# laprade117/interactive-unet

Hardware: AMD Instinct MI355X
Metric: voxels/sec (train step + full-volume predict) on 128^3 chunks (higher is better)
Workload: dtype bf16

## Files before the change

### include/iunet.h

```cpp
#ifndef IUNET_H
#define IUNET_H
#ifdef __cplusplus
extern "C" {
#endif

const char* iunet_last_error(void);
int iunet_abi_version(void);

long long iunet_pack_conv3_elems(int Cout, int Cin, int taps, int mode);
int iunet_pack_conv3(int dtype, const void* w, const void* scale, void* dst, int Cout, int Cin, int taps, int mode,
                     void* stream);
long long iunet_pack_first_conv_elems(int Cout, int Cin, int taps);
int iunet_pack_first_conv(int dtype, const void* w, const void* scale, void* dst, int Cout, int Cin, int taps,
                          void* stream);
int iunet_pack_convT(int dtype, const void* w, void* dst, int Cin, int Cout, int npos, void* stream);

int iunet_pack_desc_bytes(void);
int iunet_pack_batch(const void* descs, int n, int quant_max_cout, void* stream);

int iunet_conv3_fwd(int dtype, int nd, const void* x, long long x_sstride, void* y, long long y_sstride,
                    const void* wpk, const void* bias, void* stats, int N, int D, int H, int W, int Cin, int Cout,
                    int epi, int layout, void* stream);
int iunet_conv3_pick_layout(int nd, int N, int D, int H, int W, int Cin, int Cout);
int iunet_conv3_tile_pairs(int nd, int N, int D, int H, int W, int Cin, int Cout);
// ... 190 lines not shown
int iunet_bn_relu_bwd(int dtype, const void* dz, long long dz_ss, const void* z, long long z_ss, const void* y,
                      long long y_ss, void* dy, long long dy_ss, const void* mean, const void* invstd, const void* gamma,
                      const void* scale, const void* shift, void* dgamma, void* dbeta, void* slab, void* coef, int C, int N,
                      long long vox, void* stream);
int iunet_bn_relu_sum_bwd(int dtype, int nd, int K, const void* const* srcs, const long long* src_ss, const void* dpool,
                          long long dp_ss, const void* y, long long y_ss, void* dy, long long dy_ss, const void* mean,
                          const void* invstd, const void* gamma, const void* scale, const void* shift, void* dgamma, void* dbeta,
                          void* slab, void* coef, int C, int N, int D, int H, int W, void* stream);
int iunet_conv3_dgrad_bnstats(int dtype, int nd, const void* dy, long long dy_sstride, void* dz, long long dz_sstride,
                              const void* wpk, void* stats, const void* yp, long long yp_sstride, const void* mean,
                              const void* invstd, const void* scale, const void* shift, int N, int D, int H, int W, int Cin,
                              int Cout, void* stream);
int iunet_conv3_dgrad_bnstats_lay(int dtype, int nd, const void* dy, long long dy_sstride, void* dz, long long dz_sstride,
                                  const void* wpk, void* stats, const void* yp, long long yp_sstride, const void* mean,
                                  const void* invstd, const void* scale, const void* shift, int N, int D, int H, int W, int Cin,
                                  int Cout, int layout, void* stream);
int iunet_bn_relu_bwd_apply(int dtype, const void* dz, long long dz_ss, const void* y, long long y_ss, void* dy, long long dy_ss,
                            const void* mean, const void* invstd, const void* gamma, const void* scale, const void* shift,
                            void* dgamma, void* dbeta, const void* slab, int nparts, void* coef, int C, int N, long long vox,
                            void* stream);
int iunet_gn_num_parts(int N, long long vox);
int iunet_gn_relu_fwd(int dtype, const void* y, long long y_ss, void* z, long long z_ss, const void* gamma, const void* beta,
                      int groups, float eps, void* slab, void* scale, void* shift, void* mean, void* invstd, int C, int N,
                      long long vox, void* stream);
int iunet_gn_finalize(const void* stats, int nparts, int C, int groups, long long vox, const void* gamma, const void* beta, float eps,
                      void* scale, void* shift, void* mean, void* invstd, void* stream);
int iunet_gn_relu_bwd(int dtype, const void* dz, long long dz_ss, const void* y, long long y_ss, void* dy, long long dy_ss,
                      const void* gamma, int groups, const void* scale, const void* shift, const void* mean, const void* invstd,
                      void* dgamma, void* dbeta, void* slab, void* coef, int C, int N, long long vox, void* stream);
int iunet_gn_relu_pool_fwd(int dtype, int nd, const void* y, long long y_ss, void* z, long long z_ss, void* pooled, long long p_ss,
                           const void* gamma, const void* beta, int groups, float eps, void* slab, void* scale, void* shift, void* mean,
                           void* invstd, int C, int N, int Do, int Ho, int Wo, void* stream);
int iunet_conv3_sample_stats_rows(int dtype, int nd, int N, int D, int H, int W, int Cin, int Cout, int layout);
int iunet_conv3_fwd_sample_stats(int dtype, int nd, const void* x, long long x_sstride, void* y, long long y_sstride, const void* wpk,
                                 void* stats, int N, int D, int H, int W, int Cin, int Cout, int layout, void* stream);
int iunet_gn_relu_fwd_rows(int dtype, const void* y, long long y_ss, void* z, long long z_ss, const void* gamma, const void* beta,
                           int groups, float eps, void* slab, int rows, void* scale, void* shift, void* mean, void* invstd, int C, int N,
                           long long vox, void* stream);
int iunet_gn_relu_pool_fwd_rows(int dtype, int nd, const void* y, long long y_ss, void* z, long long z_ss, void* pooled, long long p_ss,
                                const void* gamma, const void* beta, int groups, float eps, void* slab, int rows, void* scale, void* shift,
                                void* mean, void* invstd, int C, int N, int Do, int Ho, int Wo, void* stream);
int iunet_conv3_dgrad_sample_bnstats(int dtype, int nd, const void* dy, long long dy_sstride, void* dz, long long dz_sstride, const void* wpk,
                                     void* stats, const void* yp, long long yp_sstride, const void* mean, const void* invstd, const void* scale,
                                     const void* shift, int N, int D, int H, int W, int Cin, int Cout, int layout, void* stream);
int iunet_gn_relu_bwd_rows(int dtype, const void* dz, long long dz_ss, const void* y, long long y_ss, void* dy, long long dy_ss,
                           const void* gamma, int groups, const void* scale, const void* shift, const void* mean, const void* invstd,
                           void* dgamma, void* dbeta, void* slab, int rows, void* coef, int C, int N, long long vox, void* stream);
int iunet_gn_relu_pool_bwd(int dtype, int nd, const void* dskip, long long ds_ss, const void* dpool, long long dp_ss, const void* y,
                           long long y_ss, void* dy, long long dy_ss, const void* gamma, int groups, const void* scale, const void* shift,
                           const void* mean, const void* invstd, void* dgamma, void* dbeta, void* slab, void* coef, int C, int N, int Do,
                           int Ho, int Wo, void* stream);
int iunet_bn_relu_pool_bwd(int dtype, int nd, const void* dskip, long long ds_ss, const void* dpool, long long dp_ss,
                           const void* y, long long y_ss, void* dy, long long dy_ss, const void* mean, const void* invstd,
                           const void* gamma, const void* scale, const void* shift, void* dgamma, void* dbeta, void* slab,
                           void* coef, int C, int N, int Do, int Ho, int Wo, void* stream);
int iunet_maxpool_bwd(int dtype, int nd, const void* z, long long z_ss, const void* dpool, long long dp_ss, void* dz,
                      long long dz_ss, int add_skip, int C, int N, int Do, int Ho, int Wo, void* stream);
int iunet_head_loss_num_parts(int N, long long vox);
int iunet_head_loss_fwd(int dtype, const void* x, long long x_ss, int C0, const void* w, const void* bias, int ncls,
                        const void* target, const void* weight, int tdtype, int kind, void* slab, void* out4, void* coef,
                        int N, long long vox, void* stream);
int iunet_head_loss_bwd_num_parts(int N, long long vox, int ncls, int C0);
int iunet_head_loss_bwd(int dtype, const void* x, long long x_ss, int C0, const void* w, const void* bias, int ncls,
                        const void* target, const void* weight, int tdtype, const void* coef, float loss_scale, void* dx,
                        long long dx_ss, void* dwslab, int N, long long vox, void* stream);
int iunet_head_loss_fwd_act(int dtype, const void* x, long long x_ss, int C0, const void* w, const void* bias, int ncls,
                            const void* target, const void* weight, int tdtype, int kind, void* slab, void* out4, void* coef,
                            const void* in_scale, const void* in_shift, int N, long long vox, void* stream);
int iunet_head_loss_bwd_act(int dtype, const void* x, long long x_ss, int C0, const void* w, const void* bias, int ncls,
                            const void* target, const void* weight, int tdtype, const void* coef, float loss_scale, void* dx,
                            long long dx_ss, void* dwslab, const void* in_scale, const void* in_shift, int N, long long vox,
                            void* stream);
int iunet_reduce_slab(void* slab, int nparts, long long n, void* out, float alpha, int accumulate, void* stream);
int iunet_conv3_wgrad_blocks(int nd, int N, int D, int H, int W, int Cin, int Cout);
long long iunet_conv3_wgrad_slab_floats(int nd, int N, int D, int H, int W, int Cin, int Cout);
int iunet_conv3_wgrad(int dtype, int nd, const void* x, long long x_ss, const void* dy, long long dy_ss, void* slab,
                      void* dW, float alpha, int N, int D, int H, int W, int Cin, int Cout, void* stream);
int iunet_conv3_wgrad_act(int dtype, int nd, const void* x, long long x_ss, const void* dy, long long dy_ss, void* slab,
                          void* dW, float alpha, const void* x_scale, const void* x_shift, int N, int D, int H, int W,
                          int Cin, int Cout, void* stream);
int iunet_pack_convT_dgrad(int dtype, const void* w, void* dst, int Cin, int Cout, int npos, void* stream);
int iunet_convT_dgrad(int dtype, int nd, const void* dy, long long dy_ss, void* dx, long long dx_ss, const void* wpk,
                      int N, int D, int H, int W, int Cin, int Cout, void* stream);
int iunet_convT_wgrad_blocks(int nd, int N, int D, int H, int W, int Cin, int Cout);
int iunet_convT_wgrad(int dtype, int nd, const void* x, long long x_ss, const void* dy, long long dy_ss, void* wslab,
                      void* bslab, void* dW, void* db, int N, int D, int H, int W, int Cin, int Cout, void* stream);
int iunet_first_conv_wgrad_blocks(int nd, int N, int D, int H, int W);
int iunet_first_conv_wgrad(int dtype, int nd, const void* x, int in_dtype, const long long* in_strides, const void* dy,
                           long long dy_ss, void* slab, void* dW, int N, int D, int H, int W, int Cin, int Cout,
                           void* stream);
int iunet_first_conv_wgrad_bn(int dtype, int nd, const void* x, int in_dtype, const long long* in_strides, const void* dz,
                              long long dz_ss, const void* y, long long y_ss, const void* mean, const void* invstd,
                              const void* coef, const void* scale, const void* shift, void* slab, void* dW, int N, int D, int H,
                              int W, int Cin, int Cout, void* stream);
int iunet_check_finite(const void* g, long long n, void* flag, void* stream);
int iunet_adamw_step(void* p, const void* g, void* m, void* v, long long n, float lr, float b1, float b2, float eps,
                     float wd, int step, float grad_scale_inv, const void* skip_flag, void* stream);

int iunet_train_state_init(void* state, float loss_scale, int dynamic, void* stream);
int iunet_head_loss_bwd_dev(int dtype, const void* x, long long x_ss, int C0, const void* w, const void* bias, int ncls,
                            const void* target, const void* weight, int tdtype, const void* coef, const void* state, void* dx,
                            long long dx_ss, void* dwslab, const void* in_scale, const void* in_shift, int N, long long vox,
                            void* stream);
int iunet_head_bn_bwd_ok(int C0, int ncls);
int iunet_head_bn_bwd(int dtype, const void* y, long long y_ss, int C0, const void* w, const void* bias, int ncls, const void* target,
                      const void* weight, int tdtype, const void* coef, float loss_scale, const void* state, const void* scale,
                      const void* shift, const void* mean, const void* invstd, const void* gamma, void* dgamma, void* dbeta, void* dy,
                      long long dy_ss, void* dwslab, void* bnslab, void* bncoef, void* dl_scratch, int N, long long vox, void* stream);
int iunet_head_gn_bwd(int dtype, const void* y, long long y_ss, int C0, const void* w, const void* bias, int ncls, const void* target,
                      const void* weight, int tdtype, const void* coef, float loss_scale, const void* state, const void* scale,
                      const void* shift, const void* mean, const void* invstd, const void* gamma, int groups, void* dgamma, void* dbeta, void* dy,
                      long long dy_ss, void* dwslab, void* bnslab, void* bncoef, void* dl_scratch, int N, long long vox, void* stream);
int iunet_head_loss_fwd_act_ps(int dtype, const void* x, long long x_ss, int C0, const void* w, const void* bias, int ncls,
                               const void* target, const void* weight, int tdtype, int kind, void* slab, void* out4, void* coef,
                               const void* in_scale, const void* in_shift, int per_sample, int N, long long vox, void* stream);
int iunet_head_grad_scatter(const void* row, void* dw, void* db, int ncls, int C0, void* stream);
int iunet_adamw_step_dev(void* p, const void* g, void* m, void* v, long long n, float lr, float b1, float b2, float eps, float wd,
                         void* state, int check, float world, void* stream);

typedef struct iunet_train iunet_train;
int iunet_train_create(int dim, int levels, int base, int cin, int ncls, int dtype, int loss_kind, iunet_train** out);
int iunet_train_create_ex(int dim, int levels, int base, int cin, int ncls, int dtype, int loss_kind, int norm, int groups, iunet_train** out);
int iunet_train_create_nested(int dim, int levels, int base, int cin, int ncls, int dtype, int loss_kind, iunet_train** out);
void iunet_train_destroy(iunet_train* t);
long long iunet_train_num_params(const iunet_train* t);
int iunet_train_num_tensors(const iunet_train* t);
int iunet_train_param(const iunet_train* t, int index, char* name, int name_cap, long long* offset, long long* numel);
int iunet_train_num_bn(const iunet_train* t);
long long iunet_train_packed_bytes(const iunet_train* t);
long long iunet_train_workspace_bytes(const iunet_train* t, int N, int D, int H, int W);
int iunet_train_bind(iunet_train* t, void* flat, void* grad, void* m, void* v, void* const* running, void* packed, void* state, void* stream);
int iunet_train_repack(iunet_train* t, void* stream);
int iunet_train_forward_backward(iunet_train* t, const void* x, int in_dtype, const long long* in_strides, const void* target,
                                 const void* weight, int tdtype, int N, int D, int H, int W, void* workspace, void* out4, void* stream);
typedef void (*iunet_train_hook)(void* ctx, int stage);
int iunet_train_forward_backward_hooks(iunet_train* t, const void* x, int in_dtype, const long long* in_strides, const void* target,
                                       const void* weight, int tdtype, int N, int D, int H, int W, void* workspace, void* out4,
                                       iunet_train_hook hook, void* hook_ctx, void* stream);
int iunet_train_update(iunet_train* t, float lr, float b1, float b2, float eps, float wd, float world, void* stream);
int iunet_train_step(iunet_train* t, const void* x, int in_dtype, const long long* in_strides, const void* target, const void* weight,
                     int tdtype, int N, int D, int H, int W, void* workspace, float lr, float b1, float b2, float eps, float wd, void* out4,
                     void* stream);

long long iunet_lk_pack_elems(int nd, int kind, int Cout, int Cin);
int iunet_lk_pack(int dtype, int nd, int kind, const void* w, const void* gamma, const void* beta, const void* mean, const void* var,
                  float eps, void* dst, void* bias_out, int Cout, int Cin, void* stream);
int iunet_lk_stats_parts(int nd, int kind, int N, int D, int H, int W, int Cout);
int iunet_lk_conv_fwd(int dtype, int nd, int kind, const void* x, long long x_ss, void* y, long long y_ss, const void* wpk,
                      const void* in_scale, const void* in_shift, const void* bias, const void* skip, long long skip_ss, void* stats, int epi,
                      int N, int D, int H, int W, int Cin, int Cout, void* stream);
long long iunet_lk_wgrad_slab_floats(int nd, int kind, int N, int D, int H, int W, int Cin, int Cout);
int iunet_lk_wgrad(int dtype, int nd, int kind, const void* x, long long x_ss, const void* dy, long long dy_ss, const void* x_scale,
                   const void* x_shift, void* slab, void* dW, float alpha, int N, int D, int H, int W, int Cin, int Cout, void* stream);
int iunet_lk_bn_relu_add(int dtype, const void* y, long long y_ss, const void* skip, long long skip_ss, void* out, long long out_ss,
                         const void* scale, const void* shift, int C, int N, long long vox, void* stream);
int iunet_lk_f32_conv_fwd(int nd, int kind, const void* x, long long x_ss, void* y, long long y_ss, const void* wpk, const void* bias,
                          const void* skip, long long skip_ss, int N, int D, int H, int W, int Cin, int Cout, void* stream);

int iunet_dl_num_taps(int nd, int rate, int D, int H, int W);
int iunet_dl_pack(int dtype, int nd, int mode, int ksz, const void* w, const void* gamma, const void* beta, const void* mean, const void* var,
                  float eps, void* dst, void* bias_out, int Cout, int Cin, int Cin_tot, int ci_off, int k_off, int ld, void* stream);
int iunet_dl_stats_parts(int N, int D, int H, int W, int Cout);
int iunet_dl_conv_fwd(int dtype, int nd, const void* x, long long x_ss, void* y, long long y_ss, const void* wpk, int Kw, int nbr,
                      const int* rates, const int* cbase, const int* colbase, const void* in_scale, const void* in_shift, const void* bias,
                      const void* psb, float psb_scale, void* stats, int epi, int N, int D, int H, int W, int Cin, int Cout, void* stream);
long long iunet_dl_wgrad_slab_floats(int nd, int rate, int N, int D, int H, int W, int Cin, int Cout);
// ... 45 lines not shown
```

### interactive-unet_amd/csrc/train_misc.hip

```cpp
#include "common.h"

namespace {


struct ConvTDgradParams {
  const void* dy; long long dy_ss;
  void* dx; long long dx_ss;
  const void* wpk;
  int N, D, H, W, Cin, Cout;
};

template <typename T, int ND>
__global__ __launch_bounds__(256) void convT_dgrad_kernel(ConvTDgradParams p) {
  using V8 = V8T<T>;
  constexpr int NPOS = ND == 3 ? 8 : 4;
  const int lane = threadIdx.x & 63, wave = threadIdx.x >> 6;
  const int l15 = lane & 15, q = lane >> 4;
  const int xg = (p.W + 15) / 16;
  const long long rows = (long long)p.D * p.H * xg;
  const long long wid = (long long)blockIdx.x * 4 + wave;
  if (wid >= rows * p.N) return;
  const int n = (int)(wid / rows);
  const long long r = wid - n * rows;
  const int xb = (int)(r % xg), y = (int)((r / xg) % p.H), z = (int)(r / ((long long)xg * p.H));
  const int cib = blockIdx.y;
  const int x = xb * 16 + l15;
  const bool ok = x < p.W;
  const int xc = ok ? x : p.W - 1;
  const int Do = ND == 3 ? p.D * 2 : 1, Ho = p.H * 2, Wo = p.W * 2;
  const long long out_plane = (long long)Do * Ho * Wo * 8;
  const T* dyin = (const T*)p.dy + n * p.dy_ss;
  const int nk = p.Cout >> 5;
  const V8* wp = (const V8*)p.wpk + (long long)cib * NPOS * nk * 2 * 64 + lane;
  f32x4 acc0 = f32x4{0, 0, 0, 0}, acc1 = f32x4{0, 0, 0, 0};
#pragma unroll
  for (int s = 0; s < NPOS; ++s) {
    const int a = ND == 3 ? (s >> 2) : 0, b = (s >> 1) & 1, c = s & 1;
    const int oz = ND == 3 ? z * 2 + a : 0;
    const long long voff = (((long long)oz * Ho + y * 2 + b) * Wo + xc * 2 + c) * 8;
    for (int kc = 0; kc < nk; ++kc) {
      const V8 bf = *(const V8*)(dyin + (long long)(kc * 4 + q) * out_plane + voff);
      const V8 a0 = wp[((s * nk + kc) * 2 + 0) * 64];
      const V8 a1 = wp[((s * nk + kc) * 2 + 1) * 64];
      acc0 = mfma16<T>(a0, bf, acc0);
      acc1 = mfma16<T>(a1, bf, acc1);
    }
  }
  const long long in_plane = (long long)p.D * p.H * p.W * 8;
  V8 o;
#pragma unroll
  for (int j = 0; j < 4; ++j) { o[j] = from_f32<T>(acc0[j]); o[4 + j] = from_f32<T>(acc1[j]); }
  if (ok)
    *(V8*)((T*)p.dx + n * p.dx_ss + (long long)(cib * 4 + q) * in_plane + (((long long)z * p.H + y) * p.W + x) * 8) = o;
}

template <typename T, int ND, int NK, int NCI>
__global__ __launch_bounds__(256, (NCI * NK * (ND == 3 ? 16 : 8) <= 64) ? 2 : 1) void convT_dgrad_lds_kernel(ConvTDgradParams p) {
  using V8 = V8T<T>;
  constexpr int NPOS = ND == 3 ? 8 : 4, G = 2;
  constexpr int WCI = NPOS * NK * 2 * 64;
  extern __shared__ __attribute__((aligned(256))) unsigned char smem[];
  const int lane = threadIdx.x & 63, wave = threadIdx.x >> 6;
  const int l15 = lane & 15, q = lane >> 4;
  const int cib0 = blockIdx.y * NCI;
  {
    const u32x4* wsrc = (const u32x4*)p.wpk + (long long)cib0 * WCI;
    stage_to_lds(smem, wsrc, NCI * WCI, threadIdx.x, 256);
  }
  __syncthreads();
  const int xg = (p.W + 15) / 16;
  const long long rows = (long long)p.D * p.H * xg, ngroups = rows * p.N;
  const int Do = ND == 3 ? p.D * 2 : 1, Ho = p.H * 2, Wo = p.W * 2;
  const long long out_plane = (long long)Do * Ho * Wo * 8, in_plane = (long long)p.D * p.H * p.W * 8;
  for (long long g0 = ((long long)blockIdx.x * 4 + wave) * G; g0 < ngroups; g0 += (long long)gridDim.x * 4 * G) {
    unsigned woff = lane * 16;
    asm volatile("" : "+v"(woff));
    const V8* wl = (const V8*)(smem + woff);
    f32x4 acc[NCI][G][2];
    const T* dyb[G];
    long long xoff[G];
    bool okg[G];
#pragma unroll
    for (int g = 0; g < G; ++g) {
      const long long wid = g0 + g < ngroups ? g0 + g : ngroups - 1;
      const int n = (int)(wid / rows);
      const long long r = wid - n * rows;
      const int xb = (int)(r % xg), y = (int)((r / xg) % p.H), z = (int)(r / ((long long)xg * p.H));
      const int x = xb * 16 + l15, xc = min(x, p.W - 1);
      okg[g] = x < p.W && g0 + g < ngroups;
      const int oz = ND == 3 ? z * 2 : 0;
      dyb[g] = (const T*)p.dy + n * p.dy_ss + (((long long)oz * Ho + y * 2) * Wo + xc * 2) * 8;
      xoff[g] = n * p.dx_ss + (long long)(cib0 * 4 + q) * in_plane + (((long long)z * p.H + y) * p.W + x) * 8;
#pragma unroll
      for (int c = 0; c < NCI; ++c) { acc[c][g][0] = f32x4{0, 0, 0, 0}; acc[c][g][1] = f32x4{0, 0, 0, 0}; }
    }
#pragma unroll
    for (int s = 0; s < NPOS; ++s) {
      const int a = ND == 3 ? (s >> 2) : 0, b = (s >> 1) & 1, c = s & 1;
      const long long voff = (((long long)a * Ho + b) * Wo + c) * 8;
#pragma unroll
      for (int kc = 0; kc < NK; ++kc) {
        V8 bf[G];
#pragma unroll
        for (int g = 0; g < G; ++g) bf[g] = *(const V8*)(dyb[g] + (long long)(kc * 4 + q) * out_plane + voff);
#pragma unroll
        for (int c = 0; c < NCI; ++c) {
          const V8 a0 = wl[c * WCI + ((s * NK + kc) * 2 + 0) * 64];
          const V8 a1 = wl[c * WCI + ((s * NK + kc) * 2 + 1) * 64];
#pragma unroll
          for (int g = 0; g < G; ++g) {
            acc[c][g][0] = mfma16<T>(a0, bf[g], acc[c][g][0]);
            acc[c][g][1] = mfma16<T>(a1, bf[g], acc[c][g][1]);
          }
        }
      }
    }
#pragma unroll
    for (int c = 0; c < NCI; ++c)
#pragma unroll
      for (int g = 0; g < G; ++g) {
        V8 o;
#pragma unroll
        for (int j = 0; j < 4; ++j) { o[j] = from_f32<T>(acc[c][g][0][j]); o[4 + j] = from_f32<T>(acc[c][g][1][j]); }
        if (okg[g]) *(V8*)((T*)p.dx + xoff[g] + (long long)c * 4 * in_plane) = o;
      }
  }
}

template <typename T>
__global__ void pack_convT_dgrad_kernel(const float* __restrict__ w, T* __restrict__ dst, int Cin, int Cout, int npos) {
  const long long total = (long long)Cin * Cout * npos;
  const int nk = Cout >> 5;
  for (long long i = blockIdx.x * (long long)blockDim.x + threadIdx.x; i < total; i += (long long)gridDim.x * blockDim.x) {
    long long r = i;
    const int j = r & 7; r >>= 3;
    const int lane = r & 63; r >>= 6;
    const int t = r & 1; r >>= 1;
    const int kc = r % nk; r /= nk;
    const int s = r % npos;
    const int cib = r / npos;
    const int row = lane & 15, qq = lane >> 4;
    const int ci = cib * 32 + 8 * (row >> 2) + 4 * t + (row & 3);
    const int co = kc * 32 + 8 * qq + j;
    dst[i] = from_f32<T>(w[((long long)ci * Cout + co) * npos + s]);
  }
}

typedef short s16x4w __attribute__((ext_vector_type(4)));
typedef short s16x8w __attribute__((ext_vector_type(8)));
typedef __attribute__((address_space(3))) s16x4w* lds_s4w_ptr;

template <typename T>
__device__ __forceinline__ typename Vec8<T>::type tr_frag2(unsigned addr, unsigned hi_off) {
  const s16x4w lo = __builtin_amdgcn_ds_read_tr16_b64_v4i16((lds_s4w_ptr)addr);
  const s16x4w hi = __builtin_amdgcn_ds_read_tr16_b64_v4i16((lds_s4w_ptr)(addr + hi_off));
  const s16x8w v = __builtin_shufflevector(lo, hi, 0, 1, 2, 3, 4, 5, 6, 7);
  return __builtin_bit_cast(typename Vec8<T>::type, v);
}

struct ConvTWgradParams {
  const void* x; long long x_ss;
  const void* dy; long long dy_ss;
  float* wslab;
  float* bslab;
  int N, D, H, W, Cin, Cout;
  int tilesZ, tilesY, tilesX;
};

template <typename T, int ND, int NCI>
__global__ __launch_bounds__(256, 2) void convT_wgrad_kernel(ConvTWgradParams p) {
  using V8 = V8T<T>;
  constexpr int NPOS = ND == 3 ? 8 : 4;
  constexpr int TZ = ND == 3 ? 2 : 1, TY = ND == 3 ? 4 : 8, TX = 16;
  constexpr int NVI = TZ * TY * TX;
  constexpr int OZ = ND == 3 ? 2 * TZ : 1, OY = 2 * TY, OX = 2 * TX;
  constexpr int NVO = OZ * OY * OX;
  constexpr int PLANE_X = NVI * 16 + 64, PLANE_Y = NVO * 16 + 64;
  constexpr int OFF_Y = 4 * PLANE_X;
  constexpr int NKS = NVI / 32;
  constexpr int PL = NPOS / 4;
  extern __shared__ __attribute__((aligned(256))) unsigned char smem[];
  const unsigned lds0 = (unsigned)(size_t)(__attribute__((address_space(3))) unsigned char*)smem;
  const int tid = threadIdx.x, lane = tid & 63;
  const int wave = __builtin_amdgcn_readfirstlane(tid >> 6);
  const int g = lane >> 4, i16 = lane & 15, q = i16 >> 2, pp = i16 & 3, gh = g >> 1, gl = g & 1;
  const int cib0 = blockIdx.y * NCI, cob = blockIdx.z;
  const unsigned laneX = lds0 + (pp >> 1) * PLANE_X + (pp & 1) * 8 + (gh * 16 + gl * 8 + q) * 16;
  const unsigned laneY = lds0 + OFF_Y + (pp >> 1) * PLANE_Y + (pp & 1) * 8 + (gh * 2 * OX + 2 * (gl * 8 + q)) * 16;
  unsigned pos_off[PL];
#pragma unroll
  for (int i = 0; i < PL; ++i) {
    const int s = wave * PL + i;
    const int a = ND == 3 ? (s >> 2) : 0, b = (s >> 1) & 1, c = s & 1;
    pos_off[i] = (unsigned)(((a * OY + b) * OX + c) * 16);
  }
  f32x4 acc[NCI][PL][2][2];
#pragma unroll
  for (int c = 0; c < NCI; ++c)
#pragma unroll
    for (int i = 0; i < PL; ++i)
#pragma unroll
      for (int t = 0; t < 2; ++t) { acc[c][i][t][0] = f32x4{0, 0, 0, 0}; acc[c][i][t][1] = f32x4{0, 0, 0, 0}; }
  float bacc[8] = {0.f, 0.f, 0.f, 0.f, 0.f, 0.f, 0.f, 0.f};

  const int tps = p.tilesZ * p.tilesY * p.tilesX, ntiles = tps * p.N;
  const int Do = ND == 3 ? p.D * 2 : 1, Ho = p.H * 2, Wo = p.W * 2;
  const long long in_plane = (long long)p.D * p.H * p.W * 8, out_plane = (long long)Do * Ho * Wo * 8;
  constexpr int XIT = NVI * 4 / 256, YIT = NVO * 4 / 256;
  u32x4 xr[NCI * XIT], xkeep[NCI > 1 ? XIT : 1];
  V8 yr[YIT];
  auto load_tile = [&](int tile) {
    const int n = tile / tps;
    int trem = tile - n * tps;
    const int tz_i = trem / (p.tilesY * p.tilesX);
    trem -= tz_i * p.tilesY * p.tilesX;
    const int ty_i = trem / p.tilesX, tx_i = trem - ty_i * p.tilesX;
    const int z0 = tz_i * TZ, y0 = ty_i * TY, x0 = tx_i * TX;
    const T* xin = (const T*)p.x + (long long)n * p.x_ss + (long long)cib0 * 4 * in_plane;
    const T* dyin = (const T*)p.dy + (long long)n * p.dy_ss + (long long)cob * 4 * out_plane;
#pragma unroll
    for (int k = 0; k < NCI * XIT; ++k) {
      const int it = tid + k * 256;
      const int pl = it / NVI, pix = it - pl * NVI;
      const int px = pix % TX, t2 = pix / TX, py = t2 % TY, pz = t2 / TY;
      const int gz = z0 + pz, gy = y0 + py, gx = x0 + px;
      u32x4 v = u32x4{0u, 0u, 0u, 0u};
      if (gz < p.D && gy < p.H && gx < p.W) v = *(const u32x4*)(xin + pl * in_plane + (((long long)gz * p.H + gy) * p.W + gx) * 8);
      xr[k] = v;
    }
#pragma unroll
    for (int k = 0; k < YIT; ++k) {
      const int it = tid + k * 256;
      const int pl = it & 3, pix = it >> 2;
      const int px = pix % OX, t2 = pix / OX, py = t2 % OY, pz = t2 / OY;
      const int gz = 2 * z0 + pz, gy = 2 * y0 + py, gx = 2 * x0 + px;
      V8 v;
#pragma unroll
      for (int j = 0; j < 8; ++j) v[j] = from_f32<T>(0.f);
      if (gz < Do && gy < Ho && gx < Wo) v = *(const V8*)(dyin + pl * out_plane + (((long long)gz * Ho + gy) * Wo + gx) * 8);
      yr[k] = v;
    }
  };
  auto commit_x = [&](const u32x4* src) {
#pragma unroll
    for (int k = 0; k < XIT; ++k) {
      const int it = tid + k * 256;
      const int pl = it / NVI, pix = it - pl * NVI;
      *(u32x4*)(smem + pl * PLANE_X + pix * 16) = src[k];
    }
  };
  auto commit_tile = [&]() {
    commit_x(xr);
    if (NCI > 1) {
#pragma unroll
      for (int k = 0; k < XIT; ++k) xkeep[k] = xr[XIT + k];
    }
#pragma unroll
    for (int k = 0; k < YIT; ++k) {
      const int it = tid + k * 256;
      const int pl = it & 3, pix = it >> 2;
      *(V8*)(smem + OFF_Y + pl * PLANE_Y + pix * 16) = yr[k];
#pragma unroll
      for (int j = 0; j < 8; ++j) bacc[j] += to_f32<T>(yr[k][j]);
    }
  };
  if ((int)blockIdx.x < ntiles) load_tile(blockIdx.x);
  for (int tile = blockIdx.x; tile < ntiles; tile += gridDim.x) {
    __syncthreads();
    commit_tile();
    __syncthreads();
    if (tile + (int)gridDim.x < ntiles) load_tile(tile + gridDim.x);
#pragma unroll
    for (int c = 0; c < NCI; ++c) {
      if (c > 0) {
        __syncthreads();
        commit_x(xkeep);
        __syncthreads();
      }
#pragma unroll
      for (int ks = 0; ks < NKS; ++ks) {
        const int r = 2 * ks, rz = r / TY, ry = r % TY;
        const unsigned offX = (unsigned)(r * TX * 16);
        const unsigned offY = (unsigned)(((2 * rz * OY + 2 * ry) * OX) * 16);
        const V8 a0 = tr_frag2<T>(laneX + offX, 64);
        const V8 a1 = tr_frag2<T>(laneX + offX + 2 * PLANE_X, 64);
#pragma unroll
        for (int i = 0; i < PL; ++i) {
          const V8 b0 = tr_frag2<T>(laneY + offY + pos_off[i], 128);
          const V8 b1 = tr_frag2<T>(laneY + offY + pos_off[i] + 2 * PLANE_Y, 128);
          acc[c][i][0][0] = mfma16<T>(a0, b0, acc[c][i][0][0]);
          acc[c][i][0][1] = mfma16<T>(a0, b1, acc[c][i][0][1]);
          acc[c][i][1][0] = mfma16<T>(a1, b0, acc[c][i][1][0]);
          acc[c][i][1][1] = mfma16<T>(a1, b1, acc[c][i][1][1]);
        }
      }
    }
  }
#pragma unroll
  for (int c = 0; c < NCI; ++c) {
    float* ws = p.wslab + ((((long long)blockIdx.x * (gridDim.y * NCI) + cib0 + c) * gridDim.z + cob) * NPOS) * 1024;
#pragma unroll
    for (int i = 0; i < PL; ++i) {
      const int s = wave * PL + i;
#pragma unroll
      for (int t = 0; t < 2; ++t)
#pragma unroll
        for (int u = 0; u < 2; ++u)
#pragma unroll
          for (int j = 0; j < 4; ++j) ws[s * 1024 + (t * 16 + 4 * g + j) * 32 + u * 16 + i16] = acc[c][i][t][u][j];
    }
  }
  if (blockIdx.y == 0) {
    __syncthreads();
    float* red = (float*)smem;
#pragma unroll
    for (int j = 0; j < 8; ++j) red[tid * 8 + j] = bacc[j];
    __syncthreads();
    if (tid < 32) {
      const int pl = tid >> 3, j = tid & 7;
      float sum = 0.f;
      for (int k = pl; k < 256; k += 4) sum += red[k * 8 + j];
      p.bslab[(long long)blockIdx.x * p.Cout + cob * 32 + pl * 8 + j] = sum;
    }
  }
}

__global__ __launch_bounds__(256) void convT_wgrad_reduce_kernel(const float* __restrict__ slab, int nb, int Cin, int Cout, int npos,
                                                                 float* __restrict__ dW) {
  __shared__ f32x4 red[16][16];
  const long long per_b4 = (long long)Cin * Cout * npos / 4;
  const int col4 = threadIdx.x & 15, grp = threadIdx.x >> 4;
  const long long j4 = (long long)blockIdx.x * 16 + col4;
  const f32x4* slab4 = (const f32x4*)slab;
  f32x4 s = f32x4{0.f, 0.f, 0.f, 0.f};
  for (int b = grp; b < nb; b += 16) s += slab4[b * per_b4 + j4];
  red[grp][col4] = s;
  __syncthreads();
  if (grp != 0) return;
#pragma unroll
  for (int g = 1; g < 16; ++g) s += red[g][col4];
  const int ncob = Cout / 32;
#pragma unroll
  for (int k = 0; k < 4; ++k) {
    const long long j = j4 * 4 + k;
    const int c = (int)(j & 31), r = (int)((j >> 5) & 31);
    long long t = j >> 10;
    const int pos = (int)(t % npos); t /= npos;
    const int cob = (int)(t % ncob), cib = (int)(t / ncob);
    dW[((long long)(cib * 32 + r) * Cout + cob * 32 + c) * npos + pos] = s[k];
  }
}

struct FirstWgradParams {
  const void* x; long long sN, sC, sD, sH, sW; int in_dtype;
  const void* dy; long long dy_ss;
  const void* yraw; long long y_ss;
  const float* mean; const float* invstd; const float* coef; const float* scale; const float* shift;
  float* slab;
  int N, D, H, W, Cin, Cout;
  int tilesZ, tilesY, tilesX;
};

__device__ __forceinline__ float load_in2(const void* p, long long off, int dt) {
  switch (dt) {
    case 0: return ((const float*)p)[off];
    case 1: return (float)((const f16*)p)[off];
    case 2: return (float)((const unsigned char*)p)[off] / 255.0f;
    default: return (float)((const bf16*)p)[off];
  }
}

template <typename T, int ND, int CIN>
__global__ __launch_bounds__(256, 2) void first_wgrad_kernel(FirstWgradParams p) {
  using V8 = V8T<T>;
  constexpr int TZ = ND == 3 ? 4 : 1, TY = ND == 3 ? 8 : 16, TX = ND == 3 ? 16 : 32, PADZ = ND == 3 ? 1 : 0;
  constexpr int PZ = TZ + 2 * PADZ, PY = TY + 2, PX = TX + 2, NPIX = PZ * PY * PX, NVOX = TZ * TY * TX;
  constexpr int TAPS = ND == 3 ? 27 : 9, KK = TAPS * CIN, NT = (KK + 15) / 16, KKP = NT * 16;
  constexpr int FX = TX / 16, NKS = NVOX / 32;
  constexpr int PLANE_Y = NVOX * 16 + 64;
  constexpr int XS_BYTES = ((CIN * NPIX * 2 + 255) / 256) * 256;
  extern __shared__ __attribute__((aligned(256))) unsigned char smem[];
  T* xs = (T*)smem;
  unsigned char* dys = smem + XS_BYTES;
  __shared__ __attribute__((aligned(16))) float par[7 * 32];
  if (p.yraw != nullptr && threadIdx.x < 7 * 32) {
    const int k = threadIdx.x >> 5, c = blockIdx.y * 32 + (threadIdx.x & 31);
    par[threadIdx.x] = k == 0 ? p.scale[c] : k == 1 ? p.shift[c] : k == 2 ? p.mean[c] : k == 3 ? p.invstd[c] : p.coef[c * 3 + (k - 4)];
  }
  const unsigned lds_y = (unsigned)(size_t)(__attribute__((address_space(3))) unsigned char*)dys;
  const int tid = threadIdx.x, lane = tid & 63;
  const int wave = __builtin_amdgcn_readfirstlane(tid >> 6);
  const int g = lane >> 4, i16 = lane & 15, q = i16 >> 2, pp = i16 & 3, gh = g >> 1, gl = g & 1;
  const int cob = blockIdx.y;
  const unsigned laneY = lds_y + (pp >> 1) * PLANE_Y + (pp & 1) * 8 + (gh * 16 + gl * 8 + q) * 16;
  int col_off[NT];
#pragma unroll
  for (int ct = 0; ct < NT; ++ct) {
    const int kk = ct * 16 + i16, kc = kk < KK ? kk : 0;
    const int tap = kc / CIN, c = kc % CIN;
    const int dz = ND == 3 ? tap / 9 : 0, dy_ = (tap / 3) % 3, dx = tap % 3;
    col_off[ct] = c * NPIX + (dz * PY + dy_) * PX + dx;
  }
  f32x4 acc[2][NT];
#pragma unroll
  for (int t = 0; t < 2; ++t)
#pragma unroll
// ... 82 lines not shown
    __syncthreads();
    if (tile + (int)gridDim.x < ntiles) load_tile(tile + gridDim.x);
    for (int ks = wave; ks < NKS; ks += 4) {
      const int f = 2 * ks + gh;
      const int xh = f % FX, row = f / FX, fy = row % TY, fz = row / TY;
      const int vbase = (fz * PY + fy) * PX + xh * 16 + gl * 8;
      const V8 a0 = tr_frag2<T>(laneY + (unsigned)(2 * ks * 256), 64);
      const V8 a1 = tr_frag2<T>(laneY + (unsigned)(2 * ks * 256) + 2 * PLANE_Y, 64);
#pragma unroll
      for (int ct = 0; ct < NT; ++ct) {
        V8 b;
#pragma unroll
        for (int j = 0; j < 8; ++j) b[j] = xs[vbase + j + col_off[ct]];
        acc[0][ct] = mfma16<T>(a0, b, acc[0][ct]);
        acc[1][ct] = mfma16<T>(a1, b, acc[1][ct]);
      }
    }
  }
  __syncthreads();
  float* red = (float*)smem;
#pragma unroll
  for (int t = 0; t < 2; ++t)
#pragma unroll
    for (int ct = 0; ct < NT; ++ct)
#pragma unroll
      for (int j = 0; j < 4; ++j) red[(wave * 32 + t * 16 + 4 * g + j) * KKP + ct * 16 + i16] = acc[t][ct][j];
  __syncthreads();
  float* slab = p.slab + ((long long)blockIdx.x * p.Cout + cob * 32) * KKP;
  for (int i = tid; i < 32 * KKP; i += 256)
    slab[i] = red[i] + red[32 * KKP + i] + red[2 * 32 * KKP + i] + red[3 * 32 * KKP + i];
}

__global__ __launch_bounds__(256) void first_wgrad_reduce_kernel(const float* __restrict__ slab, int nb, int Cout, int Cin, int taps,
                                                                 int KKP, float* __restrict__ dW) {
  __shared__ float red[8][32];
  const int total = Cout * Cin * taps;
  const int o = threadIdx.x & 31, grp = threadIdx.x >> 5;
  const int i = blockIdx.x * 32 + o;
  float s = 0.f;
  if (i < total) {
    const int tap = i % taps, c = (i / taps) % Cin, co = i / (taps * Cin);
    const float* src = slab + (long long)co * KKP + tap * Cin + c;
    const long long st = (long long)Cout * KKP;
    int b = grp;
    float s1 = 0.f, s2 = 0.f, s3 = 0.f;
    for (; b + 24 < nb; b += 32) {
      const float a0 = src[b * st], a1 = src[(b + 8) * st], a2 = src[(b + 16) * st], a3 = src[(b + 24) * st];
      s += a0; s1 += a1; s2 += a2; s3 += a3;
    }
    for (; b < nb; b += 8) s += src[b * st];
    s = (s + s1) + (s2 + s3);
  }
  red[grp][o] = s;
  __syncthreads();
  if (grp == 0 && i < total) {
    float a = red[0][o];
#pragma unroll
    for (int g = 1; g < 8; ++g) a += red[g][o];
    dW[i] = a;
  }
}

}

#define DT_OK(dt) IUNET_REQUIRE((dt) == 0 || (dt) == 1, "dtype must be 0 (f16) or 1 (bf16), got %d", (dt))

extern "C" int iunet_reduce_slab(void* slab, int nparts, long long n, void* out, float alpha, int accumulate, void* stream);

extern "C" {

int iunet_pack_convT_dgrad(int dtype, const void* w, void* dst, int Cin, int Cout, int npos, void* stream) {
  DT_OK(dtype);
  IUNET_REQUIRE(w && dst, "pack_convT_dgrad: null pointer");
  IUNET_REQUIRE(Cin >= 32 && Cout >= 32 && Cin % 32 == 0 && Cout % 32 == 0, "pack_convT_dgrad: channels must be positive multiples of 32");
  IUNET_REQUIRE(npos == 4 || npos == 8, "pack_convT_dgrad: npos must be 4 or 8");
  const long long total = (long long)Cin * Cout * npos;
  const int blocks = (int)((total + 255) / 256 < 4096 ? (total + 255) / 256 : 4096);
  if (dtype == 0) hipLaunchKernelGGL(pack_convT_dgrad_kernel<f16>, dim3(blocks), dim3(256), 0, (hipStream_t)stream, (const float*)w, (f16*)dst, Cin, Cout, npos);
  else hipLaunchKernelGGL(pack_convT_dgrad_kernel<bf16>, dim3(blocks), dim3(256), 0, (hipStream_t)stream, (const float*)w, (bf16*)dst, Cin, Cout, npos);
  IUNET_CHECK_HIP(hipGetLastError());
  return IUNET_OK;
}

int iunet_convT_dgrad(int dtype, int nd, const void* dy, long long dy_ss, void* dx, long long dx_ss, const void* wpk,
                      int N, int D, int H, int W, int Cin, int Cout, void* stream) {
  DT_OK(dtype);
  IUNET_REQUIRE(dy && dx && wpk, "convT_dgrad: null pointer");
  IUNET_REQUIRE(nd == 2 || nd == 3, "convT_dgrad: nd must be 2 or 3");
  IUNET_REQUIRE_GRID("convT_dgrad", N, D, H, W);
  IUNET_REQUIRE(Cin >= 32 && Cout >= 32 && Cin % 32 == 0 && Cout % 32 == 0, "convT_dgrad: channels must be positive multiples of 32 (%d, %d)", Cin, Cout);
  ConvTDgradParams p;
  p.dy = dy; p.dy_ss = dy_ss; p.dx = dx; p.dx_ss = dx_ss; p.wpk = wpk; p.N = N; p.D = D; p.H = H; p.W = W; p.Cin = Cin; p.Cout = Cout;
  const long long waves = (long long)N * D * H * ((W + 15) / 16);
  const int nk = Cout / 32;
  if (nk <= 4 && waves >= 256) {
    const int nci = (nk <= 2 && (Cin / 32) % 2 == 0 && (nd == 3 ? 8 : 4) * nk * 2 * 1024 * 2 <= 32768) ? 2 : 1;
    const int lds = (nd == 3 ? 8 : 4) * nk * 2 * 1024 * nci;
    int gx = (int)((waves + 7) / 8);
    const int cap = 1024 / (Cin / 32 / nci);
    if (gx > cap) gx = cap;
    dim3 g2(gx, Cin / 32 / nci);
#define CDL(TT, NDV, NKV) do { if (nci == 2) { IUNET_SET_MAX_LDS((convT_dgrad_lds_kernel<TT, NDV, NKV, 2>), lds); \
      hipLaunchKernelGGL((convT_dgrad_lds_kernel<TT, NDV, NKV, 2>), g2, dim3(256), lds, (hipStream_t)stream, p); } \
    else { IUNET_SET_MAX_LDS((convT_dgrad_lds_kernel<TT, NDV, NKV, 1>), lds); \
      hipLaunchKernelGGL((convT_dgrad_lds_kernel<TT, NDV, NKV, 1>), g2, dim3(256), lds, (hipStream_t)stream, p); } } while (0)
#define CDL_NK(TT, NDV) switch (nk) { case 1: CDL(TT, NDV, 1); break; case 2: CDL(TT, NDV, 2); break; case 3: CDL(TT, NDV, 3); break; default: CDL(TT, NDV, 4); break; }
    if (dtype == 0) { if (nd == 3) { CDL_NK(f16, 3) } else { CDL_NK(f16, 2) } }
    else            { if (nd == 3) { CDL_NK(bf16, 3) } else { CDL_NK(bf16, 2) } }
#undef CDL_NK
#undef CDL
    IUNET_CHECK_HIP(hipGetLastError());
    return IUNET_OK;
  }
  dim3 grid((unsigned)((waves + 3) / 4), Cin / 32);
  if (dtype == 0) { if (nd == 3) hipLaunchKernelGGL((convT_dgrad_kernel<f16, 3>), grid, dim3(256), 0, (hipStream_t)stream, p);
                    else hipLaunchKernelGGL((convT_dgrad_kernel<f16, 2>), grid, dim3(256), 0, (hipStream_t)stream, p); }
  else { if (nd == 3) hipLaunchKernelGGL((convT_dgrad_kernel<bf16, 3>), grid, dim3(256), 0, (hipStream_t)stream, p);
         else hipLaunchKernelGGL((convT_dgrad_kernel<bf16, 2>), grid, dim3(256), 0, (hipStream_t)stream, p); }
  IUNET_CHECK_HIP(hipGetLastError());
  return IUNET_OK;
}

int iunet_convT_wgrad_blocks(int nd, int N, int D, int H, int W, int Cin, int Cout) {
  if (N < 1 || D < 1 || H < 1 || W < 1 || Cin < 32 || Cout < 32) return 0;
  const int TZ = nd == 3 ? 2 : 1, TY = nd == 3 ? 4 : 8, TX = 16;
  const long long ntiles = (long long)N * ((D + TZ - 1) / TZ) * ((H + TY - 1) / TY) * ((W + TX - 1) / TX);
  const int nci = (Cin / 32) % 2 == 0 ? 2 : 1;
  const int pairs = (Cin / 32 / nci) * (Cout / 32);
  long long nb = (512 + pairs - 1) / pairs;
  if (nb > ntiles) nb = ntiles;
  return (int)(nb < 1 ? 1 : nb);
}

int iunet_convT_wgrad(int dtype, int nd, const void* x, long long x_ss, const void* dy, long long dy_ss, void* wslab,
                      void* bslab, void* dW, void* db, int N, int D, int H, int W, int Cin, int Cout, void* stream) {
  DT_OK(dtype);
  IUNET_REQUIRE(x && dy && wslab && bslab && dW && db, "convT_wgrad: null pointer");
  IUNET_REQUIRE(Cin >= 32 && Cout >= 32 && Cin % 32 == 0 && Cout % 32 == 0, "convT_wgrad: channels must be positive multiples of 32");
  IUNET_REQUIRE(nd == 2 || nd == 3, "convT_wgrad: nd must be 2 or 3");
  IUNET_REQUIRE_GRID("convT_wgrad", N, D, H, W);
  ConvTWgradParams p;
  p.x = x; p.x_ss = x_ss; p.dy = dy; p.dy_ss = dy_ss; p.wslab = (float*)wslab; p.bslab = (float*)bslab;
  p.N = N; p.D = D; p.H = H; p.W = W; p.Cin = Cin; p.Cout = Cout;
  const int TZ = nd == 3 ? 2 : 1, TY = nd == 3 ? 4 : 8, TX = 16;
  p.tilesZ = (D + TZ - 1) / TZ; p.tilesY = (H + TY - 1) / TY; p.tilesX = (W + TX - 1) / TX;
  const int nb = iunet_convT_wgrad_blocks(nd, N, D, H, W, Cin, Cout);
  const int npos = nd == 3 ? 8 : 4;
  const int nvi = 128, nvo = nd == 3 ? 1024 : 512;
  const int lds = 4 * (nvi * 16 + 64) + 4 * (nvo * 16 + 64);
  const int nci = (Cin / 32) % 2 == 0 ? 2 : 1;
  dim3 grid(nb, Cin / 32 / nci, Cout / 32);
#define CTW(TT, NDV) do { if (nci == 2) { IUNET_SET_MAX_LDS((convT_wgrad_kernel<TT, NDV, 2>), lds); \
      hipLaunchKernelGGL((convT_wgrad_kernel<TT, NDV, 2>), grid, dim3(256), lds, (hipStream_t)stream, p); } \
    else { IUNET_SET_MAX_LDS((convT_wgrad_kernel<TT, NDV, 1>), lds); \
      hipLaunchKernelGGL((convT_wgrad_kernel<TT, NDV, 1>), grid, dim3(256), lds, (hipStream_t)stream, p); } } while (0)
  if (dtype == 0) { if (nd == 3) CTW(f16, 3); else CTW(f16, 2); } else { if (nd == 3) CTW(bf16, 3); else CTW(bf16, 2); }
#undef CTW
  const long long total = (long long)Cin * Cout * npos;
  hipLaunchKernelGGL(convT_wgrad_reduce_kernel, dim3((unsigned)(total / 64)), dim3(256), 0, (hipStream_t)stream,
                     (const float*)wslab, nb, Cin, Cout, npos, (float*)dW);
  IUNET_CHECK_HIP(hipGetLastError());
  return iunet_reduce_slab(bslab, nb, Cout, db, 1.0f, 0, stream);
}

int iunet_first_conv_wgrad_blocks(int nd, int N, int D, int H, int W) {
  if (N < 1 || D < 1 || H < 1 || W < 1) return 0;
  const int TZ = nd == 3 ? 4 : 1, TY = nd == 3 ? 8 : 16, TX = nd == 3 ? 16 : 32;
  const long long ntiles = (long long)N * ((D + TZ - 1) / TZ) * ((H + TY - 1) / TY) * ((W + TX - 1) / TX);
  return (int)(ntiles < 512 ? ntiles : 512);
}

static int first_wgrad_impl(int dtype, int nd, const void* x, int in_dtype, const long long* in_strides, const void* dy,
                            long long dy_ss, void* slab, void* dW, int N, int D, int H, int W, int Cin, int Cout,
                            const void* yraw, long long y_ss, const float* mean, const float* invstd, const float* coef,
                            const float* scale, const float* shift, void* stream) {
  DT_OK(dtype);
  IUNET_REQUIRE(x && dy && slab && dW && in_strides, "first_conv_wgrad: null pointer");
  IUNET_REQUIRE(Cin >= 1 && Cin <= 4 && Cout >= 32 && Cout % 32 == 0, "first_conv_wgrad: Cin 1..4, Cout a positive multiple of 32");
  IUNET_REQUIRE(nd == 2 || nd == 3, "first_conv_wgrad: nd must be 2 or 3");
  IUNET_REQUIRE(in_dtype >= 0 && in_dtype <= 3, "first_conv_wgrad: bad input dtype %d", in_dtype);
  IUNET_REQUIRE_GRID("first_conv_wgrad", N, D, H, W);
  FirstWgradParams p;
  p.x = x; p.sN = in_strides[0]; p.sC = in_strides[1]; p.sD = in_strides[2]; p.sH = in_strides[3]; p.sW = in_strides[4];
  p.in_dtype = in_dtype; p.dy = dy; p.dy_ss = dy_ss; p.slab = (float*)slab;
  p.yraw = yraw; p.y_ss = y_ss; p.mean = mean; p.invstd = invstd; p.coef = coef; p.scale = scale; p.shift = shift;
  p.N = N; p.D = D; p.H = H; p.W = W; p.Cin = Cin; p.Cout = Cout;
  const int TZ = nd == 3 ? 4 : 1, TY = nd == 3 ? 8 : 16, TX = nd == 3 ? 16 : 32;
  p.tilesZ = (D + TZ - 1) / TZ; p.tilesY = (H + TY - 1) / TY; p.tilesX = (W + TX - 1) / TX;
  const int nb = iunet_first_conv_wgrad_blocks(nd, N, D, H, W);
  const int taps = nd == 3 ? 27 : 9, KKP = ((taps * Cin + 15) / 16) * 16;
  const int npix = (nd == 3 ? 6 : 1) * (TY + 2) * (TX + 2);
  const int xs_bytes = ((Cin * npix * 2 + 255) / 256) * 256;
  int lds = xs_bytes + 4 * (512 * 16 + 64);
  if (lds < 4 * 32 * KKP * 4) lds = 4 * 32 * KKP * 4;
  dim3 grid(nb, Cout / 32);
#define FW(TT, NDV, CI) do { IUNET_SET_MAX_LDS((first_wgrad_kernel<TT, NDV, CI>), lds); \
    hipLaunchKernelGGL((first_wgrad_kernel<TT, NDV, CI>), grid, dim3(256), lds, (hipStream_t)stream, p); } while (0)
#define FW_CIN(TT, NDV) switch (Cin) { case 1: FW(TT, NDV, 1); break; case 2: FW(TT, NDV, 2); break; case 3: FW(TT, NDV, 3); break; default: FW(TT, NDV, 4); break; }
  if (dtype == 0) { if (nd == 3) { FW_CIN(f16, 3) } else { FW_CIN(f16, 2) } }
  else            { if (nd == 3) { FW_CIN(bf16, 3) } else { FW_CIN(bf16, 2) } }
#undef FW_CIN
#undef FW
  const int total = Cout * Cin * taps;
  hipLaunchKernelGGL(first_wgrad_reduce_kernel, dim3((total + 31) / 32), dim3(256), 0, (hipStream_t)stream,
                     (const float*)slab, nb, Cout, Cin, taps, KKP, (float*)dW);
  IUNET_CHECK_HIP(hipGetLastError());
  return IUNET_OK;
}

int iunet_first_conv_wgrad(int dtype, int nd, const void* x, int in_dtype, const long long* in_strides, const void* dy,
                           long long dy_ss, void* slab, void* dW, int N, int D, int H, int W, int Cin, int Cout,
                           void* stream) {
  return first_wgrad_impl(dtype, nd, x, in_dtype, in_strides, dy, dy_ss, slab, dW, N, D, H, W, Cin, Cout, nullptr, 0, nullptr,
                          nullptr, nullptr, nullptr, nullptr, stream);
}

int iunet_first_conv_wgrad_bn(int dtype, int nd, const void* x, int in_dtype, const long long* in_strides, const void* dz,
                              long long dz_ss, const void* y, long long y_ss, const void* mean, const void* invstd,
                              const void* coef, const void* scale, const void* shift, void* slab, void* dW, int N, int D, int H,
                              int W, int Cin, int Cout, void* stream) {
  IUNET_REQUIRE(y && mean && invstd && coef && scale && shift, "first_conv_wgrad_bn: null pointer");
  return first_wgrad_impl(dtype, nd, x, in_dtype, in_strides, dz, dz_ss, slab, dW, N, D, H, W, Cin, Cout, y, y_ss,
                          (const float*)mean, (const float*)invstd, (const float*)coef, (const float*)scale,
                          (const float*)shift, stream);
}

}
```

### interactive-unet_amd/csrc/train_net.hip

```cpp
#include "common.h"
#include "pack_desc.h"
#include <algorithm>
#include <cstdio>
#include <cstdlib>
#include <string>
#include <vector>

extern "C" {
int iunet_pack_batch(const void*, int, int, void*);
int iunet_pack_desc_bytes(void);
long long iunet_pack_conv3_elems(int, int, int, int);
long long iunet_pack_first_conv_elems(int, int, int);
int iunet_conv3_packs_compact(int, int);
int iunet_conv3_plan(int, int, int, int, int, int, int, int, int, int, int*);
int iunet_conv3_num_tiles(int, int, int, int, int);
int iunet_conv3_stats_parts(int, int, int, int, int, int, int);
int iunet_first_conv_fwd(int, int, const void*, int, const long long*, void*, long long, const void*, const void*, void*, int, int, int,
                         int, int, int, int, void*);
int iunet_conv3_fwd(int, int, const void*, long long, void*, long long, const void*, const void*, void*, int, int, int, int, int, int,
                    int, int, void*);
int iunet_conv3_fwd_act(int, int, const void*, long long, void*, long long, const void*, const void*, void*, const void*, const void*,
                        int, int, int, int, int, int, int, int, void*);
int iunet_convT_fwd(int, int, const void*, long long, void*, long long, const void*, const void*, int, int, int, int, int, int, void*);
int iunet_bn_finalize(const void*, int, int, double, const void*, const void*, void*, void*, float, float, void*, void*, void*, void*, void*);
int iunet_bn_relu_fwd(int, const void*, long long, void*, long long, const void*, const void*, int, int, long long, void*);
int iunet_bn_relu_pool_fwd(int, int, const void*, long long, void*, long long, void*, long long, const void*, const void*, int, int, int,
                           int, int, void*);
int iunet_bn_bwd_num_parts(int, long long);
int iunet_bn_relu_bwd(int, const void*, long long, const void*, long long, const void*, long long, void*, long long, const void*,
                      const void*, const void*, const void*, const void*, void*, void*, void*, void*, int, int, long long, void*);
int iunet_conv3_dgrad_bnstats_lay(int, int, const void*, long long, void*, long long, const void*, void*, const void*, long long, const void*,
                                  const void*, const void*, const void*, int, int, int, int, int, int, int, void*);
int iunet_bn_relu_bwd_apply(int, const void*, long long, const void*, long long, void*, long long, const void*, const void*, const void*,
                            const void*, const void*, void*, void*, const void*, int, void*, int, int, long long, void*);
int iunet_bn_relu_pool_bwd(int, int, const void*, long long, const void*, long long, const void*, long long, void*, long long, const void*,
                           const void*, const void*, const void*, const void*, void*, void*, void*, void*, int, int, int, int, int, void*);
int iunet_head_loss_num_parts(int, long long);
int iunet_head_loss_fwd(int, const void*, long long, int, const void*, const void*, int, const void*, const void*, int, int, void*, void*,
                        void*, int, long long, void*);
int iunet_head_loss_fwd_act(int, const void*, long long, int, const void*, const void*, int, const void*, const void*, int, int, void*,
                            void*, void*, const void*, const void*, int, long long, void*);
int iunet_head_loss_bwd_num_parts(int, long long, int, int);
int iunet_head_loss_bwd_dev(int, const void*, long long, int, const void*, const void*, int, const void*, const void*, int, const void*,
                            const void*, void*, long long, void*, const void*, const void*, int, long long, void*);
int iunet_head_grad_scatter(const void*, void*, void*, int, int, void*);
int iunet_head_bn_bwd_ok(int, int);
int iunet_head_gn_bwd(int, const void*, long long, int, const void*, const void*, int, const void*, const void*, int, const void*, float, const void*, const void*,
                      const void*, const void*, const void*, const void*, int, void*, void*, void*, long long, void*, void*, void*, void*, int, long long, void*);
int iunet_head_loss_fwd_act_ps(int, const void*, long long, int, const void*, const void*, int, const void*, const void*, int, int, void*, void*, void*,
                               const void*, const void*, int, int, long long, void*);
int iunet_head_bn_bwd(int, const void*, long long, int, const void*, const void*, int, const void*, const void*, int, const void*, float, const void*, const void*,
                      const void*, const void*, const void*, const void*, void*, void*, void*, long long, void*, void*, void*, void*, int, long long, void*);
int iunet_reduce_slab(void*, int, long long, void*, float, int, void*);
long long iunet_conv3_wgrad_slab_floats(int, int, int, int, int, int, int);
int iunet_conv3_wgrad(int, int, const void*, long long, const void*, long long, void*, void*, float, int, int, int, int, int, int, void*);
int iunet_conv3_wgrad_act(int, int, const void*, long long, const void*, long long, void*, void*, float, const void*, const void*, int,
                          int, int, int, int, int, void*);
int iunet_convT_dgrad(int, int, const void*, long long, void*, long long, const void*, int, int, int, int, int, int, void*);
int iunet_convT_wgrad_blocks(int, int, int, int, int, int, int);
int iunet_convT_wgrad(int, int, const void*, long long, const void*, long long, void*, void*, void*, void*, int, int, int, int, int, int,
                      void*);
int iunet_first_conv_wgrad_blocks(int, int, int, int, int);
int iunet_first_conv_wgrad_bn(int, int, const void*, int, const long long*, const void*, long long, const void*, long long, const void*,
                              const void*, const void*, const void*, const void*, void*, void*, int, int, int, int, int, int, void*);
int iunet_adamw_step_dev(void*, const void*, void*, void*, long long, float, float, float, float, float, void*, int, float, void*);
int iunet_conv3_sample_stats_rows(int, int, int, int, int, int, int, int, int);
int iunet_conv3_fwd_sample_stats(int, int, const void*, long long, void*, long long, const void*, void*, int, int, int, int, int, int, int, void*);
int iunet_conv3_dgrad_sample_bnstats(int, int, const void*, long long, void*, long long, const void*, void*, const void*, long long, const void*, const void*,
                                     const void*, const void*, int, int, int, int, int, int, int, void*);
int iunet_gn_relu_bwd_rows(int, const void*, long long, const void*, long long, void*, long long, const void*, int, const void*, const void*, const void*,
                           const void*, void*, void*, void*, int, void*, int, int, long long, void*);
int iunet_gn_relu_fwd_rows(int, const void*, long long, void*, long long, const void*, const void*, int, float, void*, int, void*, void*, void*, void*, int, int,
                           long long, void*);
int iunet_gn_relu_pool_fwd_rows(int, int, const void*, long long, void*, long long, void*, long long, const void*, const void*, int, float, void*, int, void*,
                                void*, void*, void*, int, int, int, int, int, void*);
int iunet_gn_relu_fwd(int, const void*, long long, void*, long long, const void*, const void*, int, float, void*, void*, void*, void*, void*, int, int,
                      long long, void*);
int iunet_gn_relu_pool_fwd(int, int, const void*, long long, void*, long long, void*, long long, const void*, const void*, int, float, void*, void*,
                           void*, void*, void*, int, int, int, int, int, void*);
int iunet_gn_relu_bwd(int, const void*, long long, const void*, long long, void*, long long, const void*, int, const void*, const void*, const void*,
                      const void*, void*, void*, void*, void*, int, int, long long, void*);
int iunet_gn_relu_pool_bwd(int, int, const void*, long long, const void*, long long, const void*, long long, void*, long long, const void*, int,
                           const void*, const void*, const void*, const void*, void*, void*, void*, void*, int, int, int, int, int, void*);
int iunet_first_conv_wgrad(int, int, const void*, int, const long long*, const void*, long long, void*, void*, int, int, int, int, int, int, void*);
int iunet_bn_relu_sum_bwd(int, int, int, const void* const*, const long long*, const void*, long long, const void*, long long, void*, long long,
                          const void*, const void*, const void*, const void*, const void*, void*, void*, void*, void*, int, int, int, int, int, void*);
}

namespace {

long long align256(long long v) { return (v + 255) & ~255ll; }
bool env_on(const char* name) { const char* e = getenv(name); return e != nullptr && e[0] != 0; }

struct TParam { std::string name; long long off, numel; };

struct TPack {
  int cout = 0, cin = 0, dg = 0;
  long long buf[2] = {-1, -1};
  long long elems[2] = {0, 0};
};

struct TConv {
  std::string name;
  int ci, co, l, first;
  long long w, gamma, beta;
  int bn;
  TPack fwd, dgr;
  long long first_pk = -1, first_elems = 0;
};
struct TUp { int ci, co, l; long long w, b, fwd, dgr; };

struct TWs {
  std::vector<long long> y, z, dz, scale, shift, mean, invstd;
  std::vector<long long> cat, dcat, bslab, pin, dpin;
  std::vector<long long> up, ndcat, dT;
  long long dy, stats, wslab, bnslab, bncoef, lslab, hslab, htmp, out4, coef, bytes;
};

}

struct iunet_train {
  int norm = 0, groups = 8;
  int dim, levels, base, cin, ncls, dtype, kind;
  int taps, npos;
  bool fuse_act, fuse_bw, head_act, gn_conv_stats, gn_bw, head_bn, gn_head;
  std::vector<int> ch;
  std::vector<TParam> params;
  long long nparams = 0;
  std::vector<TConv> conv;
  std::vector<TUp> up;
  bool nested = false;
  std::vector<std::pair<int, int>> nodes;
  std::vector<int> node_at;
  long long head_w = 0, head_b = 0;
  long long packed_bytes = 0, table_off = 0;
  int ndesc = 0;
  float *flat = nullptr, *grad = nullptr, *m = nullptr, *v = nullptr, *state = nullptr;
  std::vector<float*> running;
  unsigned char* packed = nullptr;
};

namespace {

int stage_index(const iunet_train* n, bool dec, int l) { return dec ? n->levels + (n->levels - 2 - l) : l; }
const TConv& conv_of(const iunet_train* n, bool dec, int l, int j) { return n->conv[2 * stage_index(n, dec, l) + (j - 1)]; }

void pack_alloc(TPack& p, int cout, int cin, int taps, int dg, long long& pk) {
  p.cout = cout; p.cin = cin; p.dg = dg;
  auto take = [&](int k, int mode) { p.elems[k] = iunet_pack_conv3_elems(cout, cin, taps, mode | dg); p.buf[k] = pk; pk = align256(pk + p.elems[k] * 2); };
  take(0, 2);
  if (iunet_conv3_packs_compact(taps, dg ? cout : cin) > 0) take(1, 6);
}

int pack_pick(const TPack& p, int nd, int N, int D, int H, int W, bool act, bool bw, long long* off, int* fused = nullptr) {
  const int in_ch = p.dg ? p.cout : p.cin, out_ch = p.dg ? p.cin : p.cout;
  const int lay = iunet_conv3_plan(nd, N, D, H, W, in_ch, out_ch, act, bw, p.buf[1] >= 0, fused);
  *off = p.buf[lay == 3];
  return lay;
}

TWs ws_layout_nested(const iunet_train* n, int N, int D, int H, int W);

TWs ws_layout(const iunet_train* n, int N, int D, int H, int W) {
  if (n->nested) return ws_layout_nested(n, N, D, H, W);
  TWs L;
  const int lv = n->levels, dim = n->dim;
  long long off = 0;
  auto act = [&](long long elems) { const long long o = off; off = align256(off + elems * 2); return o; };
  auto f32 = [&](long long nfl) { const long long o = off; off = align256(off + nfl * 4); return o; };
  auto dims = [&](int l, int& d, int& h, int& w) { d = dim == 3 ? D >> l : 1; h = H >> l; w = W >> l; };
  auto vox = [&](int l) { int d, h, w; dims(l, d, h, w); return (long long)d * h * w; };
  const size_t nc = n->conv.size();
  L.y.assign(nc, -1); L.z.assign(nc, -1); L.dz.assign(nc, -1);
  L.scale.assign(nc, -1); L.shift.assign(nc, -1); L.mean.assign(nc, -1); L.invstd.assign(nc, -1);
  long long max_stats = 0, max_wslab = 0, max_bn = 0, max_dy = 0;
  for (size_t k = 0; k < nc; ++k) {
    const TConv& c = n->conv[k];
    int d, h, w;
    dims(c.l, d, h, w);
    const long long v = vox(c.l);
    L.y[k] = act((long long)N * c.co * v);
    const bool enc = c.name[0] == 'e', skip = enc && c.name.back() == '2' && c.l < lv - 1;
    if (!skip) { L.z[k] = act((long long)N * c.co * v); L.dz[k] = act((long long)N * c.co * v); }
    const long long rows = n->norm == 1 ? N : 1;
    L.scale[k] = f32(rows * c.co); L.shift[k] = f32(rows * c.co); L.mean[k] = f32(rows * c.co); L.invstd[k] = f32(rows * c.co);
    if (c.first) {
      max_stats = std::max(max_stats, (long long)iunet_conv3_num_tiles(dim, N, d, h, w) * c.co * 2);
      max_wslab = std::max(max_wslab, (long long)iunet_first_conv_wgrad_blocks(dim, N, d, h, w) * c.co * 112);
    } else {
      const long long p0 = iunet_conv3_num_tiles(dim, N, d, h, w), p2 = iunet_conv3_stats_parts(dim, N, d, h, w, c.co, 2);
      max_stats = std::max(max_stats, std::max(p0, p2) * c.co * 2);
      if (n->norm == 1)
        for (int lay = 2; lay <= 3; ++lay)
          max_stats = std::max(max_stats, (long long)N * iunet_conv3_sample_stats_rows(n->dtype, dim, N, d, h, w, c.ci, c.co, lay) * c.co * 2);
      max_wslab = std::max(max_wslab, iunet_conv3_wgrad_slab_floats(dim, N, d, h, w, c.ci, c.co));
    }
    max_bn = std::max(max_bn, (long long)iunet_bn_bwd_num_parts(N, v) * c.co * 2);
    max_dy = std::max(max_dy, (long long)n->ch[c.l] * v);
  }
  L.cat.assign(lv, -1); L.dcat.assign(lv, -1); L.bslab.assign(lv, -1); L.pin.assign(lv, -1); L.dpin.assign(lv, -1);
  for (int l = 0; l < lv; ++l) {
    const long long v = vox(l);
    if (l < lv - 1) {
      L.cat[l] = act((long long)N * 2 * n->ch[l] * v);
      L.dcat[l] = act((long long)N * 2 * n->ch[l] * v);
      int d, h, w;
      dims(l + 1, d, h, w);
      const long long nb = iunet_convT_wgrad_blocks(dim, N, d, h, w, n->ch[l + 1], n->ch[l]);
      max_wslab = std::max(max_wslab, nb * n->ch[l + 1] * n->ch[l] * n->npos);
      L.bslab[l] = f32(nb * n->ch[l]);
    }
    if (l > 0) { L.pin[l] = act((long long)N * n->ch[l - 1] * v); L.dpin[l] = act((long long)N * n->ch[l - 1] * v); }
  }
  const long long v0 = vox(0);
  L.dy = act((long long)N * max_dy);
  L.stats = f32(max_stats); L.wslab = f32(max_wslab); L.bnslab = f32(max_bn);
  L.bncoef = f32(3ll * n->ch[lv - 1] * (n->norm == 1 ? N : 1));
  L.lslab = f32((long long)iunet_head_loss_num_parts(N, v0) * n->ncls * 8);
  L.hslab = f32((long long)iunet_head_loss_bwd_num_parts(N, v0, n->ncls, n->ch[0]) * n->ncls * (n->ch[0] + 1));
  L.htmp = f32((long long)n->ncls * (n->ch[0] + 1));
  L.out4 = f32(4);
  L.coef = f32((long long)n->ncls * 3);
  L.bytes = off;
  return L;
}

TWs ws_layout_nested(const iunet_train* n, int N, int D, int H, int W) {
  TWs L;
  const int lv = n->levels, dim = n->dim;
  long long off = 0;
  auto act = [&](long long elems) { const long long o = off; off = align256(off + elems * 2); return o; };
  auto f32 = [&](long long nfl) { const long long o = off; off = align256(off + nfl * 4); return o; };
  auto dims = [&](int l, int& d, int& h, int& w) { d = dim == 3 ? D >> l : 1; h = H >> l; w = W >> l; };
  auto vox = [&](int l) { int d, h, w; dims(l, d, h, w); return (long long)d * h * w; };
  const size_t nc = n->conv.size();
  L.y.assign(nc, -1); L.z.assign(nc, -1); L.dz.assign(nc, -1);
  L.scale.assign(nc, -1); L.shift.assign(nc, -1); L.mean.assign(nc, -1); L.invstd.assign(nc, -1);
  long long max_stats = 0, max_wslab = 0, max_bn = 0, max_dy = 0;
  for (size_t k = 0; k < nc; ++k) {
    const TConv& c = n->conv[k];
    int d, h, w;
    dims(c.l, d, h, w);
    const long long v = vox(c.l);
    L.y[k] = act((long long)N * c.co * v);
    if (k % 2 == 0 || k == nc - 1) { L.z[k] = act((long long)N * c.co * v); L.dz[k] = act((long long)N * c.co * v); }
    L.scale[k] = f32(c.co); L.shift[k] = f32(c.co); L.mean[k] = f32(c.co); L.invstd[k] = f32(c.co);
    if (c.first) {
      max_stats = std::max(max_stats, (long long)iunet_conv3_num_tiles(dim, N, d, h, w) * c.co * 2);
      max_wslab = std::max(max_wslab, (long long)iunet_first_conv_wgrad_blocks(dim, N, d, h, w) * c.co * 112);
    } else {
      const long long p0 = iunet_conv3_num_tiles(dim, N, d, h, w), p2 = iunet_conv3_stats_parts(dim, N, d, h, w, c.co, 2);
      max_stats = std::max(max_stats, std::max(p0, p2) * c.co * 2);
      max_wslab = std::max(max_wslab, iunet_conv3_wgrad_slab_floats(dim, N, d, h, w, c.ci, c.co));
    }
    max_bn = std::max(max_bn, (long long)iunet_bn_bwd_num_parts(N, v) * c.co * 2);
    max_dy = std::max(max_dy, (long long)n->ch[c.l] * v);
  }
  L.cat.assign(lv, -1); L.pin.assign(lv, -1); L.dpin.assign(lv, -1);
  for (int l = 0; l < lv; ++l) {
    const long long v = vox(l);
    L.cat[l] = act((long long)N * (lv - l) * n->ch[l] * v);
    if (l > 0) { L.pin[l] = act((long long)N * n->ch[l - 1] * v); L.dpin[l] = act((long long)N * n->ch[l - 1] * v); }
  }
  const size_t nn = n->nodes.size();
  L.up.assign(nn, -1); L.ndcat.assign(nn, -1); L.dT.assign(nn, -1); L.bslab.assign(nn, -1);
  for (size_t k = 0; k < nn; ++k) {
    const int i = n->nodes[k].first, j = n->nodes[k].second;
    const long long v = vox(i), vi = vox(i + 1);
    L.up[k] = act((long long)N * n->ch[i] * v);
    L.ndcat[k] = act((long long)N * (j + 1) * n->ch[i] * v);
    L.dT[k] = act((long long)N * n->ch[i + 1] * vi);
    int d, h, w;
    dims(i + 1, d, h, w);
    const long long nb = iunet_convT_wgrad_blocks(dim, N, d, h, w, n->ch[i + 1], n->ch[i]);
    max_wslab = std::max(max_wslab, nb * n->ch[i + 1] * n->ch[i] * n->npos);
    L.bslab[k] = f32(nb * n->ch[i]);
  }
  const long long v0 = vox(0);
  L.dy = act((long long)N * max_dy);
  L.stats = f32(max_stats); L.wslab = f32(max_wslab); L.bnslab = f32(max_bn);
  L.bncoef = f32(3ll * n->ch[lv - 1]);
  L.lslab = f32((long long)iunet_head_loss_num_parts(N, v0) * n->ncls * 8);
  L.hslab = f32((long long)iunet_head_loss_bwd_num_parts(N, v0, n->ncls, n->ch[0]) * n->ncls * (n->ch[0] + 1));
  L.htmp = f32((long long)n->ncls * (n->ch[0] + 1));
  L.out4 = f32(4);
  L.coef = f32((long long)n->ncls * 3);
  L.bytes = off;
  return L;
}

int copy_slot(void* dst, long long dst_ss, const void* src, long long src_ss, long long elems, int N, void* stream) {
  IUNET_CHECK_HIP(hipMemcpy2DAsync(dst, (size_t)dst_ss * 2, src, (size_t)src_ss * 2, (size_t)elems * 2, (size_t)N, hipMemcpyDeviceToDevice,
                                   (hipStream_t)stream));
  return IUNET_OK;
}

}

extern "C" {

int iunet_train_create_ex(int dim, int levels, int base, int cin, int ncls, int dtype, int loss_kind, int norm, int groups, iunet_train** out);
int iunet_train_create(int dim, int levels, int base, int cin, int ncls, int dtype, int loss_kind, iunet_train** out) {
  return iunet_train_create_ex(dim, levels, base, cin, ncls, dtype, loss_kind, 0, 8, out);
}
static int train_create(int dim, int levels, int base, int cin, int ncls, int dtype, int loss_kind, int norm, int groups, bool nested, iunet_train** out);
int iunet_train_create_ex(int dim, int levels, int base, int cin, int ncls, int dtype, int loss_kind, int norm, int groups, iunet_train** out) {
  return train_create(dim, levels, base, cin, ncls, dtype, loss_kind, norm, groups, false, out);
}
int iunet_train_create_nested(int dim, int levels, int base, int cin, int ncls, int dtype, int loss_kind, iunet_train** out) {
  return train_create(dim, levels, base, cin, ncls, dtype, loss_kind, 0, 8, true, out);
}
static int train_create(int dim, int levels, int base, int cin, int ncls, int dtype, int loss_kind, int norm, int groups, bool nested, iunet_train** out) {
  IUNET_REQUIRE(out != nullptr, "train_create: null handle pointer");
  IUNET_REQUIRE(norm == 0 || (norm == 1 && groups > 0 && base % groups == 0), "train_create: norm must be 0 (batch) or 1 (group, groups dividing base): %d, %d groups", norm, groups);
  IUNET_REQUIRE(dim == 2 || dim == 3, "train_create: dim must be 2 or 3 (got %d)", dim);
  if (nested) IUNET_REQUIRE(levels >= 2 && levels <= 9, "train_create_nested: levels must be 2..9 (got %d)", levels);
  else IUNET_REQUIRE(levels >= 2 && levels <= 6, "train_create: levels must be 2..6 (got %d)", levels);
  IUNET_REQUIRE(base > 0 && base % 32 == 0, "train_create: base channels must be a positive multiple of 32 (got %d)", base);
  IUNET_REQUIRE(base == 32 || base == 64, "train_create: the fused head + loss kernels take 32 or 64 head input channels (base %d)", base);
  IUNET_REQUIRE(cin >= 1 && cin <= 4, "train_create: 1..4 input channels (got %d)", cin);
  IUNET_REQUIRE(ncls >= 2 && ncls <= 10, "train_create: 2..10 classes (app.py:162; got %d)", ncls);
  IUNET_REQUIRE(dtype == 0 || dtype == 1, "train_create: dtype must be 0 (fp16) or 1 (bf16), got %d", dtype);
  IUNET_REQUIRE(loss_kind >= 0 && loss_kind <= 6, "train_create: loss kind must be 0..6 (got %d)", loss_kind);
  IUNET_REQUIRE(iunet_pack_desc_bytes() == (int)sizeof(PackDesc), "train_create: PackDesc layout mismatch");
  iunet_train* n = new iunet_train();
  n->dim = dim; n->levels = levels; n->base = base; n->cin = cin; n->ncls = ncls; n->dtype = dtype; n->kind = loss_kind;
  n->taps = dim == 3 ? 27 : 9; n->npos = dim == 3 ? 8 : 4;
  n->norm = norm; n->groups = groups;
  n->fuse_act = norm == 0 && !env_on("IUNET_NO_ACT_FUSION");
  n->fuse_bw = norm == 0 && !env_on("IUNET_NO_BW_FUSION");
  n->head_act = norm == 0 && !env_on("IUNET_NO_HEAD_ACT");
  n->gn_head = norm == 1 && !env_on("IUNET_NO_HEAD_ACT") && !env_on("IUNET_NO_HEAD_BN_FUSION") && iunet_head_bn_bwd_ok(base, ncls);
  n->head_bn = n->head_act && !env_on("IUNET_NO_HEAD_BN_FUSION");
  n->gn_conv_stats = norm == 1 && !env_on("IUNET_NO_GN_CONV_STATS");
  n->gn_bw = n->gn_conv_stats && !env_on("IUNET_NO_GN_BW_FUSION");
  for (int l = 0; l < levels; ++l) n->ch.push_back(base << l);
  long long off = 0, pk = 0;
  int nbn = 0;
  auto add = [&](const std::string& name, long long numel) { n->params.push_back({name, off, numel}); const long long o = off; off += numel; return o; };
  auto stage = [&](const std::string& prefix, int ci, int co, int l) {
    for (int j = 1; j <= 2; ++j) {
      TConv c;
      c.ci = j == 1 ? ci : co; c.co = co; c.l = l; c.first = (prefix == "enc0" && j == 1);
      c.name = prefix + ".conv" + std::to_string(j);
      const std::string b = prefix + ".bn" + std::to_string(j);
      c.w = add(c.name + ".weight", (long long)co * c.ci * n->taps);
      c.gamma = add(b + ".weight", co);
      c.beta = add(b + ".bias", co);
      c.bn = nbn++;
      if (c.first) {
        c.first_elems = iunet_pack_first_conv_elems(co, c.ci, n->taps);
        c.first_pk = pk; pk = align256(pk + c.first_elems * 2);
        n->ndesc += 1;
      } else {
        pack_alloc(c.fwd, co, c.ci, n->taps, 0, pk);
        pack_alloc(c.dgr, co, c.ci, n->taps, 1, pk);
        for (int k = 0; k < 2; ++k) n->ndesc += (c.fwd.buf[k] >= 0) + (c.dgr.buf[k] >= 0);
      }
      n->conv.push_back(c);
    }
  };
  for (int l = 0; l < levels; ++l) stage("enc" + std::to_string(l), l == 0 ? cin : n->ch[l - 1], n->ch[l], l);
  auto up_op = [&](const std::string& p, int l) {
    TUp u;
    u.ci = n->ch[l + 1]; u.co = n->ch[l]; u.l = l;
    u.w = add(p + ".up.weight", (long long)u.ci * u.co * n->npos);
    u.b = add(p + ".up.bias", u.co);
    const long long ne = (long long)u.ci * u.co * n->npos;
    u.fwd = pk; pk = align256(pk + ne * 2);
    u.dgr = pk; pk = align256(pk + ne * 2);
    n->ndesc += 2;
    n->up.push_back(u);
  };
  n->nested = nested;
  n->node_at.assign((size_t)levels * levels, -1);
  for (int j = 1; j < levels && nested; ++j)
    for (int i = 0; i + j < levels; ++i) {
      n->node_at[i * levels + j] = (int)n->nodes.size();
      n->nodes.push_back({i, j});
      const std::string p = "dec" + std::to_string(i) + "_" + std::to_string(j);
      up_op(p, i);
      stage(p, (j + 1) * n->ch[i], n->ch[i], i);
    }
  for (int l = levels - 2; l >= 0 && !nested; --l) {
    TUp u;
    u.ci = n->ch[l + 1]; u.co = n->ch[l]; u.l = l;
    const std::string p = "dec" + std::to_string(l);
    u.w = add(p + ".up.weight", (long long)u.ci * u.co * n->npos);
    u.b = add(p + ".up.bias", u.co);
    const long long ne = (long long)u.ci * u.co * n->npos;
    u.fwd = pk; pk = align256(pk + ne * 2);
    u.dgr = pk; pk = align256(pk + ne * 2);
    n->ndesc += 2;
    n->up.push_back(u);
    stage(p, 2 * n->ch[l], n->ch[l], l);
  }
  n->head_w = add("head.weight", (long long)ncls * n->ch[0]);
  n->head_b = add("head.bias", ncls);
  n->nparams = off;
  n->table_off = pk;
  n->packed_bytes = pk + align256((long long)n->ndesc * sizeof(PackDesc));
  n->running.assign(2 * nbn, nullptr);
  *out = n;
  return IUNET_OK;
}

void iunet_train_destroy(iunet_train* n) { delete n; }

long long iunet_train_num_params(const iunet_train* n) { return n ? n->nparams : 0; }
int iunet_train_num_tensors(const iunet_train* n) { return n ? (int)n->params.size() : 0; }
int iunet_train_param(const iunet_train* n, int index, char* name, int name_cap, long long* offset, long long* numel) {
  IUNET_REQUIRE(n != nullptr, "train_param: null handle");
  IUNET_REQUIRE(index >= 0 && index < (int)n->params.size(), "train_param: index %d out of range", index);
  const TParam& p = n->params[index];
  if (name && name_cap > 0) snprintf(name, name_cap, "%s", p.name.c_str());
  if (offset) *offset = p.off;
// ... 328 lines not shown
      if (k2 != dy_ready) {
        const void* sp[8];
        long long ss[8];
        int K_ = 0;
        for (int jj = m + 1; jj < lv - i; ++jj) {
          const int q = n->node_at[i * lv + jj];
          sp[K_] = WS + L.ndcat[q] + (long long)m * c * v * 2; ss[K_++] = (long long)(jj + 1) * c * v;
        }
        if (i >= 1) { sp[K_] = WS + L.dT[n->node_at[(i - 1) * lv + m + 1]]; ss[K_++] = (long long)c * v; }
        if (K_ + (dpool != nullptr) == 1) {
          dzp = sp[0]; dz_ss = ss[0];
        } else {
          const TConv& cc = n->conv[k2];
          int d, h, w;
          dims(i, d, h, w);
          rc = iunet_bn_relu_sum_bwd(dt, dim, K_, sp, ss, dpool, dpool_ss, WS + L.y[k2], (long long)c * v, WS + L.dy, (long long)c * v, F(L.mean[k2]),
                                     F(L.invstd[k2]), P + cc.gamma, F(L.scale[k2]), F(L.shift[k2]), G + cc.gamma, G + cc.beta, F(L.bnslab), F(L.bncoef),
                                     c, N, d, h, w, stream);
          if (rc) return rc;
          dy_ready = k2;
        }
      }
      return conv_bwd(k2, dzp, dz_ss, x2, (long long)c * v, WS + L.dz[k1], (long long)c * v, fused ? k1 : -1, nullptr, 0, k1);
    };
    for (int k = (int)n->nodes.size() - 1; k >= 0; --k) {
      const int i = n->nodes[k].first, j = n->nodes[k].second, s = lv + k;
      int di, hi, wi;
      dims(i + 1, di, hi, wi);
      const long long v = vox(i), vi = vox(i + 1);
      const int c = n->ch[i], cn = n->ch[i + 1], k1 = 2 * s;
      if (k + 1 == (int)n->nodes.size() && dy_ready != kl) {
        const bool fused = conv2_fused(i);
        const void* x2 = fused ? (const void*)(WS + L.y[k1]) : (const void*)(WS + L.z[k1]);
        rc = conv_bwd(kl, WS + L.dz[kl], (long long)c * v, x2, (long long)c * v, WS + L.dz[k1], (long long)c * v, fused ? k1 : -1, nullptr, 0, k1);
      } else {
        rc = node_conv2_bwd(s, i, j, nullptr, 0);
      }
      if (rc) return rc;
      const long long cat_ss = (long long)(lv - i) * c * v, dcat_ss = (long long)(j + 1) * c * v;
      rc = copy_slot(WS + L.cat[i] + (long long)j * c * v * 2, cat_ss, WS + L.up[k], (long long)c * v, (long long)c * v, N, stream);
      if (rc) return rc;
      rc = conv_bwd(k1, WS + L.dz[k1], (long long)c * v, WS + L.cat[i], cat_ss, WS + L.ndcat[k], dcat_ss, -1, nullptr, 0, -1);
      if (rc) return rc;
      const TUp& u = n->up[k];
      const void* src = WS + L.cat[i + 1] + (long long)(j - 1) * cn * vi * 2;
      void* dup = WS + L.ndcat[k] + (long long)j * c * v * 2;
      rc = iunet_convT_wgrad(dt, dim, src, (long long)(lv - i - 1) * cn * vi, dup, dcat_ss, F(L.wslab), F(L.bslab[k]), G + u.w, G + u.b, N, di, hi, wi, cn,
                             c, stream);
      if (rc) return rc;
      rc = iunet_convT_dgrad(dt, dim, dup, dcat_ss, WS + L.dT[k], (long long)cn * vi, K + u.dgr, N, di, hi, wi, cn, c, stream);
      if (rc) return rc;
    }
    if (hook) hook(hook_ctx, 0);
    for (int l = lv - 1; l >= 0; --l) {
      const long long v = vox(l);
      const int c = n->ch[l], k1 = 2 * l;
      rc = l < lv - 1 ? node_conv2_bwd(l, l, 0, WS + L.dpin[l + 1], (long long)c * vox(l + 1)) : node_conv2_bwd(l, l, 0, nullptr, 0);
      if (rc) return rc;
      if (l == 0) rc = conv_bwd(k1, WS + L.dz[k1], (long long)c * v, nullptr, 0, nullptr, 0, -1, nullptr, 0, -1);
      else {
        const int cp = n->ch[l - 1];
        rc = conv_bwd(k1, WS + L.dz[k1], (long long)c * v, WS + L.pin[l], (long long)cp * v, WS + L.dpin[l], (long long)cp * v, -1, nullptr, 0, -1);
      }
      if (rc) return rc;
      if (hook && l == lv - 1) hook(hook_ctx, 1);
    }
    return IUNET_OK;
  }
  for (int l = 0; l < lv - 1; ++l) {
    int di, hi, wi;
    dims(l + 1, di, hi, wi);
    const long long v = vox(l), vi = vox(l + 1);
    const int c = n->ch[l], cn = n->ch[l + 1];
    const int k1 = idx(true, l, 1), k2 = idx(true, l, 2);
    const bool fused = conv2_fused(l);
    const void* x2 = fused ? (const void*)(WS + L.y[k1]) : (const void*)(WS + L.z[k1]);
    rc = conv_bwd(k2, WS + L.dz[k2], (long long)c * v, x2, (long long)c * v, WS + L.dz[k1], (long long)c * v, fused ? k1 : -1, nullptr, 0, k1);
    if (rc) return rc;
    rc = conv_bwd(k1, WS + L.dz[k1], (long long)c * v, WS + L.cat[l], 2ll * c * v, WS + L.dcat[l], 2ll * c * v, -1, nullptr, 0, -1);
    if (rc) return rc;
    const int ksrc = l == lv - 2 ? idx(false, l + 1, 2) : idx(true, l + 1, 2);
    const TUp& u = n->up[lv - 2 - l];
    void* dup = WS + L.dcat[l] + (long long)c * v * 2;
    rc = iunet_convT_wgrad(dt, dim, WS + L.z[ksrc], (long long)cn * vi, dup, 2ll * c * v, F(L.wslab), F(L.bslab[l]), G + u.w, G + u.b, N, di, hi, wi, cn,
                           c, stream);
    if (rc) return rc;
    rc = iunet_convT_dgrad(dt, dim, dup, 2ll * c * v, WS + L.dz[ksrc], (long long)cn * vi, K + u.dgr, N, di, hi, wi, cn, c, stream);
    if (rc) return rc;
  }
  if (hook) hook(hook_ctx, 0);
  for (int l = lv - 1; l >= 0; --l) {
    const long long v = vox(l);
    const int c = n->ch[l];
    const int k1 = idx(false, l, 1), k2 = idx(false, l, 2);
    const bool fused = conv2_fused(l);
    const void* x2 = fused ? (const void*)(WS + L.y[k1]) : (const void*)(WS + L.z[k1]);
    if (l == lv - 1)
      rc = conv_bwd(k2, WS + L.dz[k2], (long long)c * v, x2, (long long)c * v, WS + L.dz[k1], (long long)c * v, fused ? k1 : -1, nullptr, 0, k1);
    else
      rc = conv_bwd(k2, WS + L.dcat[l], 2ll * c * v, x2, (long long)c * v, WS + L.dz[k1], (long long)c * v, fused ? k1 : -1, WS + L.dpin[l + 1],
                    (long long)c * vox(l + 1), k1);
    if (rc) return rc;
    if (l == 0) rc = conv_bwd(k1, WS + L.dz[k1], (long long)c * v, nullptr, 0, nullptr, 0, -1, nullptr, 0, -1);
    else {
      const int cp = n->ch[l - 1];
      rc = conv_bwd(k1, WS + L.dz[k1], (long long)c * v, WS + L.pin[l], (long long)cp * v, WS + L.dpin[l], (long long)cp * v, -1, nullptr, 0, -1);
    }
    if (rc) return rc;
    if (hook && l == lv - 1 && lv > 1) hook(hook_ctx, 1);
  }
  return IUNET_OK;
}

int iunet_train_update(iunet_train* n, float lr, float b1, float b2, float eps, float wd, float world, void* stream) {
  IUNET_REQUIRE(n && n->packed, "train_update: iunet_train_bind has not been called");
  const int rc = iunet_adamw_step_dev(n->flat, n->grad, n->m, n->v, n->nparams, lr, b1, b2, eps, wd, n->state, n->dtype == 0 ? 1 : 0, world, stream);
  if (rc) return rc;
  return iunet_pack_batch(n->packed + n->table_off, n->ndesc, 0, stream);
}

int iunet_train_step(iunet_train* n, const void* x, int in_dtype, const long long* in_strides, const void* target, const void* weight,
                     int tdtype, int N, int D, int H, int W, void* workspace, float lr, float b1, float b2, float eps, float wd, void* out4,
                     void* stream) {
  const int rc = iunet_train_forward_backward(n, x, in_dtype, in_strides, target, weight, tdtype, N, D, H, W, workspace, out4, stream);
  if (rc) return rc;
  return iunet_train_update(n, lr, b1, b2, eps, wd, 1.0f, stream);
}

}
```

### interactive-unet_amd/interactive_unet/_native.py

```python
import ctypes
import os

import torch

_HERE = os.path.dirname(os.path.abspath(__file__))
LIB_PATH = os.environ.get('IUNET_LIB') or os.path.join(os.path.dirname(_HERE), 'lib', 'libiunet.so')

_lib = None

c_void_p, c_int, c_ll, c_float = ctypes.c_void_p, ctypes.c_int, ctypes.c_longlong, ctypes.c_float
_IP = ctypes.POINTER(c_int)
_LP = ctypes.POINTER(c_ll)
_VP = ctypes.POINTER(c_void_p)

_SIGS = {
    'iunet_abi_version': [],
    'iunet_conv3_num_tiles': [c_int] * 5,
    'iunet_conv3_stats_parts': [c_int] * 7,
    'iunet_pack_conv3': [c_int, c_void_p, c_void_p, c_void_p, c_int, c_int, c_int, c_int, c_void_p],
    'iunet_pack_first_conv': [c_int, c_void_p, c_void_p, c_void_p, c_int, c_int, c_int, c_void_p],
    'iunet_pack_convT': [c_int, c_void_p, c_void_p, c_int, c_int, c_int, c_void_p],
    'iunet_pack_batch': [c_void_p, c_int, c_int, c_void_p],
    'iunet_conv3_fwd': [c_int, c_int, c_void_p, c_ll, c_void_p, c_ll, c_void_p, c_void_p, c_void_p,
                        c_int, c_int, c_int, c_int, c_int, c_int, c_int, c_int, c_void_p],
# ... 115 lines not shown
    'iunet_normalize_quantize': [c_void_p, c_void_p, c_void_p, c_ll, c_int, c_float, c_void_p],
    'iunet_div_f32': [c_void_p, c_ll, c_float, c_void_p],
    'iunet_colorize': [c_void_p, c_ll, c_void_p, c_int, c_void_p, c_void_p],
    'iunet_slice_gather': [c_void_p, c_int, c_int, c_int, ctypes.POINTER(ctypes.c_double), ctypes.POINTER(c_int),
                           ctypes.POINTER(c_int), c_int, c_int, c_int, c_void_p, c_void_p],
    'iunet_slice_scatter': [c_void_p, c_int, c_int, c_int, c_int, ctypes.POINTER(ctypes.c_double), c_int, c_int, c_void_p, c_void_p,
                            c_void_p],
    'iunet_augment_batch': [c_void_p, c_int, c_int, c_int, c_int, c_int, c_void_p, c_void_p, c_void_p, c_void_p, c_void_p],
    'iunet_zoom_nearest_table': [c_int, ctypes.c_double, ctypes.POINTER(c_int), c_int],
    'iunet_zoom_nearest_u8': [c_void_p, ctypes.POINTER(c_int), ctypes.POINTER(c_ll), c_void_p, ctypes.POINTER(c_ll),
                              ctypes.POINTER(c_int), c_void_p, c_void_p],
    'iunet_bn_finalize': [c_void_p, c_int, c_int, ctypes.c_double, c_void_p, c_void_p, c_void_p, c_void_p, c_float,
                          c_float, c_void_p, c_void_p, c_void_p, c_void_p, c_void_p],
    'iunet_bn_relu_fwd': [c_int, c_void_p, c_ll, c_void_p, c_ll, c_void_p, c_void_p, c_int, c_int, c_ll, c_void_p],
    'iunet_bn_relu_pool_fwd': [c_int, c_int, c_void_p, c_ll, c_void_p, c_ll, c_void_p, c_ll, c_void_p, c_void_p,
                               c_int, c_int, c_int, c_int, c_int, c_void_p],
    'iunet_bn_bwd_num_parts': [c_int, c_ll],
    'iunet_conv3_dgrad_bnstats': [c_int, c_int, c_void_p, c_ll, c_void_p, c_ll, c_void_p, c_void_p, c_void_p, c_ll, c_void_p, c_void_p,
                                  c_void_p, c_void_p, c_int, c_int, c_int, c_int, c_int, c_int, c_void_p],
    'iunet_conv3_dgrad_bnstats_lay': [c_int, c_int, c_void_p, c_ll, c_void_p, c_ll, c_void_p, c_void_p, c_void_p, c_ll, c_void_p, c_void_p,
                                      c_void_p, c_void_p, c_int, c_int, c_int, c_int, c_int, c_int, c_int, c_void_p],
    'iunet_head_bn_bwd_ok': [c_int, c_int],
    'iunet_head_bn_bwd': [c_int, c_void_p, c_ll, c_int, c_void_p, c_void_p, c_int, c_void_p, c_void_p, c_int, c_void_p, c_float, c_void_p, c_void_p,
                          c_void_p, c_void_p, c_void_p, c_void_p, c_void_p, c_void_p, c_void_p, c_ll, c_void_p, c_void_p, c_void_p, c_void_p, c_int, c_ll, c_void_p],
    'iunet_bn_relu_bwd_apply': [c_int, c_void_p, c_ll, c_void_p, c_ll, c_void_p, c_ll, c_void_p, c_void_p, c_void_p, c_void_p, c_void_p,
                                c_void_p, c_void_p, c_void_p, c_int, c_void_p, c_int, c_int, c_ll, c_void_p],
    'iunet_gn_num_parts': [c_int, c_ll],
    'iunet_gn_finalize': [c_void_p, c_int, c_int, c_int, c_ll, c_void_p, c_void_p, c_float, c_void_p, c_void_p, c_void_p, c_void_p, c_void_p],
    'iunet_gn_relu_fwd': [c_int, c_void_p, c_ll, c_void_p, c_ll, c_void_p, c_void_p, c_int, c_float, c_void_p, c_void_p, c_void_p,
                          c_void_p, c_void_p, c_int, c_int, c_ll, c_void_p],
    'iunet_gn_relu_fwd_rows': [c_int, c_void_p, c_ll, c_void_p, c_ll, c_void_p, c_void_p, c_int, c_float, c_void_p, c_int, c_void_p, c_void_p,
                               c_void_p, c_void_p, c_int, c_int, c_ll, c_void_p],
    'iunet_gn_relu_pool_fwd_rows': [c_int, c_int, c_void_p, c_ll, c_void_p, c_ll, c_void_p, c_ll, c_void_p, c_void_p, c_int, c_float, c_void_p,
                                    c_int, c_void_p, c_void_p, c_void_p, c_void_p, c_int, c_int, c_int, c_int, c_int, c_void_p],
    'iunet_conv3_sample_stats_rows': [c_int] * 9,
    'iunet_conv3_fwd_sample_stats': [c_int, c_int, c_void_p, c_ll, c_void_p, c_ll, c_void_p, c_void_p, c_int, c_int, c_int, c_int,
                                     c_int, c_int, c_int, c_void_p],
    'iunet_conv3_dgrad_sample_bnstats': [c_int, c_int, c_void_p, c_ll, c_void_p, c_ll, c_void_p, c_void_p, c_void_p, c_ll, c_void_p, c_void_p,
                                         c_void_p, c_void_p, c_int, c_int, c_int, c_int, c_int, c_int, c_int, c_void_p],
    'iunet_gn_relu_bwd_rows': [c_int, c_void_p, c_ll, c_void_p, c_ll, c_void_p, c_ll, c_void_p, c_int, c_void_p, c_void_p, c_void_p,
                               c_void_p, c_void_p, c_void_p, c_void_p, c_int, c_void_p, c_int, c_int, c_ll, c_void_p],
    'iunet_gn_relu_bwd': [c_int, c_void_p, c_ll, c_void_p, c_ll, c_void_p, c_ll, c_void_p, c_int, c_void_p, c_void_p, c_void_p,
                          c_void_p, c_void_p, c_void_p, c_void_p, c_void_p, c_int, c_int, c_ll, c_void_p],
    'iunet_gn_relu_pool_fwd': [c_int, c_int, c_void_p, c_ll, c_void_p, c_ll, c_void_p, c_ll, c_void_p, c_void_p, c_int, c_float, c_void_p,
                               c_void_p, c_void_p, c_void_p, c_void_p, c_int, c_int, c_int, c_int, c_int, c_void_p],
    'iunet_gn_relu_pool_bwd': [c_int, c_int, c_void_p, c_ll, c_void_p, c_ll, c_void_p, c_ll, c_void_p, c_ll, c_void_p, c_int, c_void_p, c_void_p,
                               c_void_p, c_void_p, c_void_p, c_void_p, c_void_p, c_void_p, c_int, c_int, c_int, c_int, c_int, c_void_p],
    'iunet_bn_relu_bwd': [c_int, c_void_p, c_ll, c_void_p, c_ll, c_void_p, c_ll, c_void_p, c_ll, c_void_p, c_void_p,
                          c_void_p, c_void_p, c_void_p, c_void_p, c_void_p, c_void_p, c_void_p, c_int, c_int, c_ll, c_void_p],
    'iunet_bn_relu_pool_bwd': [c_int, c_int, c_void_p, c_ll, c_void_p, c_ll, c_void_p, c_ll, c_void_p, c_ll, c_void_p, c_void_p,
                               c_void_p, c_void_p, c_void_p, c_void_p, c_void_p, c_void_p, c_void_p, c_int, c_int, c_int,
                               c_int, c_int, c_void_p],
    'iunet_bn_relu_sum_bwd': [c_int, c_int, c_int, ctypes.POINTER(c_void_p), ctypes.POINTER(c_ll), c_void_p, c_ll, c_void_p, c_ll,
                              c_void_p, c_ll, c_void_p, c_void_p, c_void_p, c_void_p, c_void_p, c_void_p, c_void_p, c_void_p,
                              c_void_p, c_int, c_int, c_int, c_int, c_int, c_void_p],
    'iunet_maxpool_bwd': [c_int, c_int, c_void_p, c_ll, c_void_p, c_ll, c_void_p, c_ll, c_int, c_int, c_int, c_int,
                          c_int, c_int, c_void_p],
    'iunet_head_loss_num_parts': [c_int, c_ll],
    'iunet_head_loss_bwd_num_parts': [c_int, c_ll, c_int, c_int],
    'iunet_head_loss_fwd': [c_int, c_void_p, c_ll, c_int, c_void_p, c_void_p, c_int, c_void_p, c_void_p, c_int, c_int,
                            c_void_p, c_void_p, c_void_p, c_int, c_ll, c_void_p],
    'iunet_head_loss_bwd': [c_int, c_void_p, c_ll, c_int, c_void_p, c_void_p, c_int, c_void_p, c_void_p, c_int,
                            c_void_p, c_float, c_void_p, c_ll, c_void_p, c_int, c_ll, c_void_p],
    'iunet_head_loss_fwd_act': [c_int, c_void_p, c_ll, c_int, c_void_p, c_void_p, c_int, c_void_p, c_void_p, c_int, c_int,
                                c_void_p, c_void_p, c_void_p, c_void_p, c_void_p, c_int, c_ll, c_void_p],
    'iunet_head_loss_fwd_act_ps': [c_int, c_void_p, c_ll, c_int, c_void_p, c_void_p, c_int, c_void_p, c_void_p, c_int, c_int,
                                   c_void_p, c_void_p, c_void_p, c_void_p, c_void_p, c_int, c_int, c_ll, c_void_p],
    'iunet_head_gn_bwd': [c_int, c_void_p, c_ll, c_int, c_void_p, c_void_p, c_int, c_void_p, c_void_p, c_int, c_void_p, c_float, c_void_p, c_void_p,
                          c_void_p, c_void_p, c_void_p, c_void_p, c_int, c_void_p, c_void_p, c_void_p, c_ll, c_void_p, c_void_p, c_void_p, c_void_p, c_int, c_ll, c_void_p],
    'iunet_head_loss_bwd_act': [c_int, c_void_p, c_ll, c_int, c_void_p, c_void_p, c_int, c_void_p, c_void_p, c_int,
                                c_void_p, c_float, c_void_p, c_ll, c_void_p, c_void_p, c_void_p, c_int, c_ll, c_void_p],
    'iunet_reduce_slab': [c_void_p, c_int, c_ll, c_void_p, c_float, c_int, c_void_p],
    'iunet_check_finite': [c_void_p, c_ll, c_void_p, c_void_p],
    'iunet_adamw_step': [c_void_p, c_void_p, c_void_p, c_void_p, c_ll, c_float, c_float, c_float, c_float, c_float,
                         c_int, c_float, c_void_p, c_void_p],
    'iunet_conv3_wgrad_blocks': [c_int] * 7,
    'iunet_conv3_wgrad': [c_int, c_int, c_void_p, c_ll, c_void_p, c_ll, c_void_p, c_void_p, c_float,
                          c_int, c_int, c_int, c_int, c_int, c_int, c_void_p],
    'iunet_conv3_wgrad_act': [c_int, c_int, c_void_p, c_ll, c_void_p, c_ll, c_void_p, c_void_p, c_float, c_void_p, c_void_p,
                              c_int, c_int, c_int, c_int, c_int, c_int, c_void_p],
    'iunet_pack_convT_dgrad': [c_int, c_void_p, c_void_p, c_int, c_int, c_int, c_void_p],
    'iunet_convT_dgrad': [c_int, c_int, c_void_p, c_ll, c_void_p, c_ll, c_void_p, c_int, c_int, c_int, c_int, c_int,
                          c_int, c_void_p],
    'iunet_convT_wgrad_blocks': [c_int] * 7,
    'iunet_convT_wgrad': [c_int, c_int, c_void_p, c_ll, c_void_p, c_ll, c_void_p, c_void_p, c_void_p, c_void_p,
                          c_int, c_int, c_int, c_int, c_int, c_int, c_void_p],
    'iunet_first_conv_wgrad_blocks': [c_int] * 5,
    'iunet_first_conv_wgrad_bn': [c_int, c_int, c_void_p, c_int, ctypes.POINTER(c_ll), c_void_p, c_ll, c_void_p, c_ll, c_void_p,
                                  c_void_p, c_void_p, c_void_p, c_void_p, c_void_p, c_void_p, c_int, c_int, c_int, c_int, c_int,
                                  c_int, c_void_p],
    'iunet_first_conv_wgrad': [c_int, c_int, c_void_p, c_int, ctypes.POINTER(c_ll), c_void_p, c_ll, c_void_p, c_void_p,
                               c_int, c_int, c_int, c_int, c_int, c_int, c_void_p],
    'iunet_lk_pack': [c_int, c_int, c_int] + [c_void_p] * 5 + [c_float, c_void_p, c_void_p, c_int, c_int, c_void_p],
    'iunet_lk_stats_parts': [c_int] * 7,
    'iunet_lk_conv_fwd': [c_int, c_int, c_int, c_void_p, c_ll, c_void_p, c_ll, c_void_p, c_void_p, c_void_p, c_void_p, c_void_p, c_ll,
                          c_void_p, c_int, c_int, c_int, c_int, c_int, c_int, c_int, c_void_p],
    'iunet_lk_wgrad': [c_int, c_int, c_int, c_void_p, c_ll, c_void_p, c_ll, c_void_p, c_void_p, c_void_p, c_void_p, c_float,
                       c_int, c_int, c_int, c_int, c_int, c_int, c_void_p],
    'iunet_lk_bn_relu_add': [c_int, c_void_p, c_ll, c_void_p, c_ll, c_void_p, c_ll, c_void_p, c_void_p, c_int, c_int, c_ll, c_void_p],
    'iunet_lk_f32_conv_fwd': [c_int, c_int, c_void_p, c_ll, c_void_p, c_ll, c_void_p, c_void_p, c_void_p, c_ll,
                              c_int, c_int, c_int, c_int, c_int, c_int, c_void_p],
    'iunet_dl_pack': [c_int, c_int, c_int, c_int] + [c_void_p] * 5 + [c_float, c_void_p, c_void_p] + [c_int] * 6 + [c_void_p],
    'iunet_dl_stats_parts': [c_int] * 5,
    'iunet_dl_conv_fwd': [c_int, c_int, c_void_p, c_ll, c_void_p, c_ll, c_void_p, c_int, c_int, _IP, _IP, _IP, c_void_p, c_void_p, c_void_p,
                          c_void_p, c_float, c_void_p, c_int, c_int, c_int, c_int, c_int, c_int, c_int, c_void_p],
    'iunet_dl_wgrad': [c_int, c_int, c_int, c_void_p, c_ll, c_int, c_void_p, c_ll, c_void_p, c_void_p, c_void_p, c_void_p, c_int, c_int,
                       c_float, c_int, c_int, c_int, c_int, c_int, c_int, c_void_p],
    'iunet_dl_f32_conv_fwd': [c_int, c_int, c_void_p, c_ll, c_void_p, c_ll, c_void_p, c_int, c_void_p, c_void_p,
                              c_int, c_int, c_int, c_int, c_int, c_int, c_void_p],
    'iunet_dl_chansum': [c_int, c_void_p, c_ll, c_void_p, c_float, c_int, c_int, c_ll, c_void_p],
    'iunet_dl_pool_gemv': [c_void_p] * 4 + [c_int] * 3 + [c_void_p],
    'iunet_dl_pool_psb': [c_void_p] * 7 + [c_float] + [c_void_p] * 5 + [c_int, c_int, c_void_p],
    'iunet_dl_pool_bwd': [c_void_p] * 15 + [c_int] * 3 + [c_void_p],
    'iunet_dl_dropout': [c_int, c_int, c_void_p, c_ll, c_void_p, c_ll, c_void_p, c_void_p, c_void_p, c_float, c_int, c_int, c_ll, c_void_p],
    'iunet_dl_up_head': [c_int, c_void_p] + [c_int] * 5 + [c_void_p] * 3 + [ctypes.POINTER(c_ll), c_float, c_int, c_int, c_void_p],
    'iunet_dl_up_loss_fwd': [c_int, c_void_p] + [c_int] * 5 + [c_void_p, c_void_p, c_int, c_int, c_void_p, c_void_p, c_void_p, c_int, c_void_p],
    'iunet_dl_up_loss_bwd': [c_int, c_void_p] + [c_int] * 5 + [c_void_p, c_void_p, c_int] + [c_void_p] * 5 + [c_int, c_void_p],
    'iunet_dl_head_bwd': [c_int, c_void_p, c_ll, c_int, c_void_p, c_void_p, c_int, c_void_p, c_ll] + [c_void_p] * 3 + [c_int, c_ll, c_void_p],
    'iunet_sf_pack': [c_int, c_int, c_int, _IP, c_void_p, _VP, _VP] + [c_void_p] * 4 + [c_float] + [c_void_p] * 4,
    'iunet_sf_gemm': [c_int, c_int, c_int, _VP, _LP, _IP, _IP, _VP, _VP, c_void_p, c_void_p, c_void_p, c_ll, c_void_p] + [c_int] * 6 + [c_void_p],
    'iunet_sf_wgrad': [c_int, c_int, c_int, _VP, _LP, _IP, _IP, _VP, _VP, c_void_p, c_ll, c_void_p, c_void_p] + [c_int] * 5 + [c_void_p],
    'iunet_sf_adjoint': [c_int, c_int, c_void_p, c_ll, c_int, c_int, c_int, c_void_p, c_ll] + [c_int] * 5 + [c_void_p],
    'iunet_sf_param_grads': [c_int, c_int, _IP, c_void_p, _VP, _VP, c_void_p, c_void_p, c_int, _VP, _VP, c_void_p, c_void_p],
}
_INT_RETURN = ['iunet_pack_desc_bytes', 'iunet_augment_desc_bytes', 'iunet_x2_prep_desc_bytes']
_INT_RETURN_ARGS = {'iunet_sf_stats_parts': [c_int] * 4, 'iunet_dl_num_taps': [c_int] * 5, 'iunet_dl_up_loss_num_parts': [c_int, c_ll], 'iunet_dl_head_bwd_parts': [c_int, c_ll], 'iunet_zoom_nearest_len': [c_int, ctypes.c_double], 'iunet_x2_convT_kc': [c_int], 'iunet_x2m_head_fusable': [c_int, c_int], 'iunet_x2m_pool_fusable': [c_int, c_int], 'iunet_x2m_first_stage_fusable': [c_int] * 6, 'iunet_x2_pack_mode': [c_int], 'iunet_f8_pack_order': [c_int, c_int]}
_LL_RETURN = {'iunet_gn_precise_slab_bytes': [c_int, c_int, c_ll], 'iunet_net_eval_scratch_bytes': [c_void_p, c_int, c_int, c_int, c_int], 'iunet_x2m_w8_bytes': [c_int] * 2, 'iunet_x2m_w8_bytes_nd': [c_int] * 3, 'iunet_train_num_params': [c_void_p], 'iunet_train_packed_bytes': [c_void_p], 'iunet_train_workspace_bytes': [c_void_p, c_int, c_int, c_int, c_int], 'iunet_conv3_wgrad_slab_floats': [c_int] * 7, 'iunet_f32_pack_conv_elems': [c_int] * 3, 'iunet_f8_pack_conv3_bytes': [c_int] * 3, 'iunet_conv3_f8_workspace_elems': [c_int] * 7, 'iunet_pack_conv3_elems': [c_int] * 4,
              'iunet_pack_first_conv_elems': [c_int] * 3, 'iunet_slice_scatter_workspace_bytes': [c_int],
              'iunet_lk_pack_elems': [c_int] * 4, 'iunet_lk_wgrad_slab_floats': [c_int] * 8, 'iunet_dl_wgrad_slab_floats': [c_int] * 8,
              'iunet_sf_wgrad_slab_floats': [c_int] * 6,
              'iunet_net_num_params': [c_void_p], 'iunet_net_packed_bytes': [c_void_p], 'iunet_net_workspace_bytes': [c_void_p] + [c_int] * 4}


class NativeError(RuntimeError):
    pass


def lib():
    global _lib
    if _lib is None:
        if not os.path.isfile(LIB_PATH):
            raise NativeError(f'{LIB_PATH} is missing: build it with __graft_entry__.build() '
                              f'(interactive-unet_amd/csrc/build.sh); there is no CPU fallback')
        l = ctypes.CDLL(LIB_PATH)
        l.iunet_last_error.restype = ctypes.c_char_p
        l.iunet_last_error.argtypes = []
        for name, args in _SIGS.items():
            fn = getattr(l, name)
            fn.argtypes = args
            fn.restype = c_int
        for name in _INT_RETURN:
            getattr(l, name).restype = c_int
            getattr(l, name).argtypes = []
        for name, args in _INT_RETURN_ARGS.items():
            getattr(l, name).restype = c_int
            getattr(l, name).argtypes = args
        for name, args in _LL_RETURN.items():
            fn = getattr(l, name)
            fn.argtypes = args
            fn.restype = c_ll
        l.iunet_net_destroy.argtypes, l.iunet_net_destroy.restype = [c_void_p], None
        l.iunet_train_destroy.argtypes, l.iunet_train_destroy.restype = [c_void_p], None
        _lib = l
    return _lib


# ... 146 lines not shown
```

### interactive-unet_amd/interactive_unet/train_engine.py

```python
import ctypes
import math

import os

import torch

from . import _native as nv
from .engine import BN_EPS, check_spatial

LOSS_KINDS = {'ce': 0, 'dice': 1, 'iou': 2, 'mcc': 3, 'dice_ce': 4, 'iou_ce': 5, 'mcc_ce': 6}
BN_MOMENTUM = 0.1


def _vox(d):
    return d[0] * d[1] * d[2]


class TrainEngine:
    def __init__(self, model, lr=None, loss_kind='mcc_ce', betas=(0.9, 0.999), eps=1e-8, weight_decay=1e-2,
                 loss_scale=None, process_group=None):
        self.model = model
        self.dev = model.device
        if self.dev.type != 'cuda':
            raise RuntimeError('native training runs on the GPU only (no CPU fallback)')
        nv.lib()
        self.dim, self.levels, self.ch = model.dim, model.levels, [model.base * 2 ** l for l in range(model.levels)]
        self.cin, self.ncls = model.num_channels, model.num_classes
        self.T = model.act_dtype
        if self.T not in nv.DTYPE_CODE:
            raise NotImplementedError("native training runs with 16-bit activations (act_dtype 'fp16' / 'bf16'); "
                                      "act_dtype='fp32' is the inference parity mode")
        self.dt = nv.DTYPE_CODE[self.T]
        self.es = 2
        self.taps, self.npos = 3 ** self.dim, 2 ** self.dim
        self.lr = model.lr if lr is None else lr
        self.kind = LOSS_KINDS[loss_kind] if isinstance(loss_kind, str) else int(loss_kind)
        self.betas, self.eps, self.wd = betas, eps, weight_decay
        self.dynamic_scale = self.T == torch.float16 and loss_scale is None
        self.state = torch.zeros(8, dtype=torch.float32, device=self.dev)
        nv.call('iunet_train_state_init', nv.ptr(self.state), float(loss_scale) if loss_scale is not None else (1024.0 if self.T == torch.float16 else 1.0),
                int(self.dynamic_scale), nv.stream())
        self.pg = process_group
        self.fuse_act = not os.environ.get('IUNET_NO_ACT_FUSION')
        self.norm, self.groups = getattr(model, 'norm', 'batch'), getattr(model, 'groups', 8)
        self.gn = self.norm == 'group'
        if self.gn:
            self.fuse_act = False
        self.fuse_bw = not self.gn and not os.environ.get('IUNET_NO_BW_FUSION')
        self.gn_conv_stats = self.gn and not os.environ.get('IUNET_NO_GN_CONV_STATS')
        self.gn_bw = self.gn_conv_stats and not os.environ.get('IUNET_NO_GN_BW_FUSION')
        self.head_act = not self.gn and not os.environ.get('IUNET_NO_HEAD_ACT')
        self.head_bn = self.head_act and not os.environ.get('IUNET_NO_HEAD_BN_FUSION')
        self.gn_head = (self.gn and not os.environ.get('IUNET_NO_HEAD_ACT') and not os.environ.get('IUNET_NO_HEAD_BN_FUSION')
                        and bool(nv.lib().iunet_head_bn_bwd_ok(self.ch[0], self.ncls)))
        self._bw_ready = {}
        self._flatten()
        if self.pg is not None:
            from . import dp
            dp.broadcast_state(self.flat, [model.tensor(n) for n in model._names
                                           if n.endswith('running_mean') or n.endswith('running_var')], self.pg)
            self.buckets = dp.GradBuckets(self.grad, self._dec_start, self.pg)
        self._alloc_packed()
        self._ws = {}
        self.probe = None
        self.use_handle = True
        self.repack()
        model._packed_sig = None

    @property
    def loss_scale(self):
        return float(self.state[0].item())

    @loss_scale.setter
    def loss_scale(self, value):
        self.state[0:1].fill_(float(value))
        self._fixed_scale = None

    @property
    def step_count(self):
        return int(self.state.view(torch.int32)[1].item())

    @property
    def good_steps(self):
        return int(self.state.view(torch.int32)[2].item())

    @property
    def last_step_ok(self):
        return int(self.state.view(torch.int32)[3].item()) == 0

    def _flatten(self):
        m = self.model
        names = [n for n in m._names if not (n.endswith('running_mean') or n.endswith('running_var'))]
        sizes = [m.tensor(n).numel() for n in names]
        total = sum(sizes)
        flat = torch.empty(total, dtype=torch.float32, device=self.dev)
        off = 0
        self.offsets = {}
        for n, s in zip(names, sizes):
            t = m.tensor(n)
            flat[off:off + s].copy_(t.detach().reshape(-1))
            t.data = flat[off:off + s].view(t.shape)
            self.offsets[n] = (off, s)
            off += s
        self.flat = flat
        self.grad = torch.zeros_like(flat)
        self.m = torch.zeros_like(flat)
        self.v = torch.zeros_like(flat)
        self.names = names
        first_dec = f'dec{self.levels - 2}.up.weight'
        self._dec_start = self.offsets[first_dec][0] if first_dec in self.offsets else 0
        bottom = [self.offsets[n] for n in names if n.startswith(f'enc{self.levels - 1}.')]
        lo = min((o for o, _ in bottom), default=0)
        self._bottom_start = lo if bottom and lo + sum(s for _, s in bottom) == self._dec_start else None

    def p(self, name):
        return self.model.tensor(name)

    def g(self, name):
        off, s = self.offsets[name]
        return self.grad[off:off + s]

    def stage_names(self):
        return [f'enc{l}' for l in range(self.levels)] + [f'dec{l}' for l in range(self.levels - 2, -1, -1)]

    def stage_io(self, prefix):
        l = int(prefix[3:])
        ci = (self.cin if l == 0 else self.ch[l - 1]) if prefix.startswith('enc') else 2 * self.ch[l]
        return ci, self.ch[l], l

    def up_convs(self):
        return [(f'dec{l}', l) for l in range(self.levels - 2, -1, -1)]

    def _alloc_packed(self):
        self.pk = {}
        for prefix in self.stage_names():
            ci, co, _ = self.stage_io(prefix)
            for j, (a, b) in enumerate(((ci, co), (co, co)), 1):
# ... 1 lines not shown
                if name == 'enc0.conv1':
                    self.pk[name] = (torch.empty(nv.lib().iunet_pack_first_conv_elems(b, a, self.taps), dtype=self.T,
                                                 device=self.dev), None)
                else:
                    self.pk[name] = (nv.PackedConv(b, a, self.taps, self.T, self.dev),
                                     nv.PackedConv(b, a, self.taps, self.T, self.dev, dgrad=True))
        for prefix, l in self.up_convs():
            n = self.ch[l + 1] * self.ch[l] * self.npos
            self.pk[f'{prefix}.up'] = (torch.empty(n, dtype=self.T, device=self.dev),
                                       torch.empty(n, dtype=self.T, device=self.dev))
        self._alloc_decoder()

    def _alloc_decoder(self):
        """The packed operators of a decoder that is not made of stages and transposed convs (EncoderTrainEngine's subclasses)."""

    def repack(self):
        if getattr(self, '_pack_table', None) is None:
            descs = []
            for prefix in self.stage_names():
                ci, co, _ = self.stage_io(prefix)
                for j, (a, b) in enumerate(((ci, co), (co, co)), 1):
                    name = f'{prefix}.conv{j}'
                    w = self.p(name + '.weight')
                    fwd, dg = self.pk[name]
                    if name == 'enc0.conv1':
                        descs.append(nv.make_desc(w, fwd, b, a, self.taps, 2, self.T))
                    else:
                        descs += fwd.descs(w) + dg.descs(w)
            for prefix, l in self.up_convs():
                w = self.p(f'{prefix}.up.weight')
                fwd, dg = self.pk[f'{prefix}.up']
                descs.append(nv.make_desc(w, fwd, self.ch[l], self.ch[l + 1], self.npos, 3, self.T))
                descs.append(nv.make_desc(w, dg, self.ch[l], self.ch[l + 1], self.npos, 4, self.T))
            self._pack_table = nv.PackTable(descs, self.dev, sources=[self.flat])
        self._pack_table.run()
        self._pack_decoder()

    def _pack_decoder(self):
        """Launches that pack the operators _alloc_decoder allocated (after the table's)."""

    def workspace(self, N, D, H, W):
        key = (N, D, H, W)
        ws = self._ws.get(key)
        if ws is not None:
            return ws
        check_spatial(self.dim, self.levels, D, H, W)
        L, ch = self.levels, self.ch
        dims = [((D >> l) if self.dim == 3 else 1, H >> l, W >> l) for l in range(L)]
        act = lambda c, v: torch.empty(N * c * v, dtype=self.T, device=self.dev)
        f32 = lambda n: torch.empty(n, dtype=torch.float32, device=self.dev)
        lib = nv.lib()
        ws = {'dims': dims}
        max_stats, max_wslab, max_bn = 0, 0, 0
        for prefix in self.stage_names():
            ci, co, l = self.stage_io(prefix)
            v = _vox(dims[l])
            d = dims[l]
            for j, (a, b) in enumerate(((ci, co), (co, co)), 1):
                name = f'{prefix}.conv{j}'
                ws['y.' + name] = act(b, v)
                skip = prefix.startswith('enc') and j == 2 and l < L - 1
                if not skip:
                    ws['z.' + name] = act(b, v)
                    ws['dz.' + name] = act(b, v)
                for k in ('scale', 'shift', 'mean', 'invstd'):
                    ws[f'{k}.{name}'] = f32(b * (N if self.gn else 1))
                if name == 'enc0.conv1':
                    max_stats = max(max_stats, lib.iunet_conv3_num_tiles(self.dim, N, *d) * b * 2)
                    max_wslab = max(max_wslab, lib.iunet_first_conv_wgrad_blocks(self.dim, N, *d) * b * 112)
                else:
                    max_stats = max(max_stats, max(lib.iunet_conv3_num_tiles(self.dim, N, *d), lib.iunet_conv3_stats_parts(self.dim, N, *d, b, 2)) * b * 2)
                    if self.gn:
                        max_stats = max(max_stats, max(lib.iunet_conv3_sample_stats_rows(self.dt, self.dim, N, *d, a, b, lay) for lay in (2, 3)) * N * b * 2)
                    max_wslab = max(max_wslab, lib.iunet_conv3_wgrad_slab_floats(self.dim, N, *d, a, b))
                max_bn = max(max_bn, lib.iunet_bn_bwd_num_parts(N, v) * b * 2)
        for l in range(L):
            v = _vox(dims[l])
            if l < L - 1:
                ws[f'cat{l}'] = act(2 * ch[l], v)
                ws[f'dcat{l}'] = act(2 * ch[l], v)
                nb = lib.iunet_convT_wgrad_blocks(self.dim, N, *dims[l + 1], ch[l + 1], ch[l])
                max_wslab = max(max_wslab, nb * ch[l + 1] * ch[l] * self.npos)
                ws[f'bslab{l}'] = f32(nb * ch[l])
            if l > 0:
                ws[f'pin{l}'] = act(ch[l - 1], v)
                ws[f'dpin{l}'] = act(ch[l - 1], v)
        ws['dy'] = act(max(ch[l] * _vox(dims[l]) for l in range(L)), 1)
        ws['stats'] = f32(max_stats)
        ws['wslab'] = f32(max_wslab)
        ws['bnslab'] = f32(max_bn)
        ws['bncoef'] = f32(3 * max(ch) * (N if self.gn else 1))
        for k, n in self._loss_slabs(N, D, H, W, dims).items():
            ws[k] = f32(n)
        ws['out4'] = f32(4)
        ws['coef'] = f32(self.ncls * 3)
        self._ws = {key: ws}
        return ws

    def _loss_slabs(self, N, D, H, W, dims):
        lib, v0, c0 = nv.lib(), _vox(dims[0]), self.ch[0]
        return {'lslab': lib.iunet_head_loss_num_parts(N, v0) * self.ncls * 8,
                'hslab': lib.iunet_head_loss_bwd_num_parts(N, v0, self.ncls, c0) * self.ncls * (c0 + 1),
                'htmp': self.ncls * (c0 + 1)}

    def _P(self, t, off_elems=0):
        return ctypes.c_void_p(t.data_ptr() + off_elems * self.es)

    def _stage_conv_fwd(self, ws, name, x_ptr, x_ss, ci, co, l, z_ptr, z_ss, N, x_raw=None, training=True, x_act=None,
                        pool=None):
        d = ws['dims'][l]
        v = _vox(d)
        s = nv.stream()
        y = ws['y.' + name]
        stats = ws['stats']
        gn_rows = 0
        if name == 'enc0.conv1':
            x, xs = x_raw
            w, _ = self.pk[name]
            nparts = nv.lib().iunet_conv3_num_tiles(self.dim, N, *d)
            if self.gn and self.gn_conv_stats:
                gn_rows = nparts // N
            nv.call('iunet_first_conv_fwd', self.dt, self.dim, nv.ptr(x), nv.IN_DTYPE_CODE[x.dtype], nv.ll_array(xs),
                    self._P(y), co * v, nv.ptr(w), None, None if (self.gn and not gn_rows) else nv.ptr(stats), N, d[0], d[1], d[2], ci, co, 0, s)
        else:
            pk, _ = self.pk[name]
            lay, w, _ = pk.pick(self.dim, N, *d, act=x_act is not None)
            nparts = nv.lib().iunet_conv3_stats_parts(self.dim, N, *d, co, lay)
            probe = self.probe if (self.probe is not None and self.probe['name'] == name) else None
            if probe is not None:
                e0 = torch.cuda.Event(enable_timing=True)
                e0.record()
            if self.gn and x_act is None and self.gn_conv_stats:
                gn_rows = nv.lib().iunet_conv3_sample_stats_rows(self.dt, self.dim, N, d[0], d[1], d[2], ci, co, lay)
            if gn_rows > 0:
                nv.call('iunet_conv3_fwd_sample_stats', self.dt, self.dim, x_ptr, x_ss, self._P(y), co * v, nv.ptr(w), nv.ptr(stats),
                        N, d[0], d[1], d[2], ci, co, lay, s)
            elif x_act is None:
                nv.call('iunet_conv3_fwd', self.dt, self.dim, x_ptr, x_ss, self._P(y), co * v, nv.ptr(w), None,
                        None if self.gn else nv.ptr(stats), N, d[0], d[1], d[2], ci, co, 0, lay, s)
            else:
                nv.call('iunet_conv3_fwd_act', self.dt, self.dim, x_ptr, x_ss, self._P(y), co * v, nv.ptr(w), None,
                        nv.ptr(stats), nv.ptr(ws['scale.' + x_act]), nv.ptr(ws['shift.' + x_act]),
                        N, d[0], d[1], d[2], ci, co, 0, lay, s)
            if probe is not None:
                e1 = torch.cuda.Event(enable_timing=True)
                e1.record()
                probe['events'].append((e0, e1, N))
        bn = name.replace('conv', 'bn')
        if self.gn:
            if pool is not None:
                p_ptr, p_ss, do = pool
                nv.call('iunet_gn_relu_pool_fwd_rows', self.dt, self.dim, self._P(y), co * v, z_ptr, z_ss, p_ptr, p_ss, nv.ptr(self.p(bn + '.weight')),
                        nv.ptr(self.p(bn + '.bias')), self.groups, BN_EPS, nv.ptr(stats if gn_rows > 0 else ws['bnslab']), gn_rows, nv.ptr(ws['scale.' + name]),
                        nv.ptr(ws['shift.' + name]), nv.ptr(ws['mean.' + name]), nv.ptr(ws['invstd.' + name]), co, N, do[0], do[1], do[2], s)
            else:
                nv.call('iunet_gn_relu_fwd_rows', self.dt, self._P(y), co * v, z_ptr, z_ss, nv.ptr(self.p(bn + '.weight')),
                        nv.ptr(self.p(bn + '.bias')), self.groups, BN_EPS, nv.ptr(stats if gn_rows > 0 else ws['bnslab']), gn_rows, nv.ptr(ws['scale.' + name]),
                        nv.ptr(ws['shift.' + name]), nv.ptr(ws['mean.' + name]), nv.ptr(ws['invstd.' + name]), co, N, v, s)
            return
        nv.call('iunet_bn_finalize', nv.ptr(stats), nparts, co, float(N) * v,
                nv.ptr(self.p(bn + '.weight')), nv.ptr(self.p(bn + '.bias')),
                nv.ptr(self.p(bn + '.running_mean')), nv.ptr(self.p(bn + '.running_var')), BN_MOMENTUM, BN_EPS,
                nv.ptr(ws['scale.' + name]), nv.ptr(ws['shift.' + name]), nv.ptr(ws['mean.' + name]),
                nv.ptr(ws['invstd.' + name]), s)
        if z_ptr is not None and pool is not None:
            p_ptr, p_ss, do = pool
# ... 114 lines not shown
        elif first:
            x, xs = x_raw
            nv.call('iunet_first_conv_wgrad_bn', self.dt, self.dim, nv.ptr(x), nv.IN_DTYPE_CODE[x.dtype], nv.ll_array(xs),
                    dz_ptr, dz_ss, self._P(ws['y.' + name]), co * v, nv.ptr(ws['mean.' + name]), nv.ptr(ws['invstd.' + name]),
                    nv.ptr(ws['bncoef']), nv.ptr(ws['scale.' + name]), nv.ptr(ws['shift.' + name]),
                    nv.ptr(ws['wslab']), nv.ptr(gw), N, d[0], d[1], d[2], ci, co, s)
        else:
            if x_act is None:
                nv.call('iunet_conv3_wgrad', self.dt, self.dim, x_ptr, x_ss, self._P(dy), co * v, nv.ptr(ws['wslab']),
                        nv.ptr(gw), 1.0, N, d[0], d[1], d[2], ci, co, s)
            else:
                nv.call('iunet_conv3_wgrad_act', self.dt, self.dim, x_ptr, x_ss, self._P(dy), co * v, nv.ptr(ws['wslab']),
                        nv.ptr(gw), 1.0, nv.ptr(ws['scale.' + x_act]), nv.ptr(ws['shift.' + x_act]),
                        N, d[0], d[1], d[2], ci, co, s)
            _, pkd = self.pk[name]
            lay, wd, fused = pkd.pick(self.dim, N, *d, bw=feeds is not None and (self.fuse_bw or self.gn_bw))
            gn_rows = 0
            if self.gn and fused and self.gn_bw:
                gn_rows = nv.lib().iunet_conv3_sample_stats_rows(self.dt, self.dim, N, d[0], d[1], d[2], co, ci, lay)
            if fused and self.fuse_bw:
                nv.call('iunet_conv3_dgrad_bnstats_lay', self.dt, self.dim, self._P(dy), co * v, dx_ptr, dx_ss, nv.ptr(wd),
                        nv.ptr(ws['stats']), self._P(ws['y.' + feeds]), ci * v, nv.ptr(ws['mean.' + feeds]),
                        nv.ptr(ws['invstd.' + feeds]), nv.ptr(ws['scale.' + feeds]), nv.ptr(ws['shift.' + feeds]),
                        N, d[0], d[1], d[2], co, ci, lay, s)
                self._bw_ready[feeds] = nv.lib().iunet_conv3_stats_parts(self.dim, N, d[0], d[1], d[2], ci, 2)
            elif gn_rows > 0:
                nv.call('iunet_conv3_dgrad_sample_bnstats', self.dt, self.dim, self._P(dy), co * v, dx_ptr, dx_ss, nv.ptr(wd),
                        nv.ptr(ws['stats']), self._P(ws['y.' + feeds]), ci * v, nv.ptr(ws['mean.' + feeds]),
                        nv.ptr(ws['invstd.' + feeds]), nv.ptr(ws['scale.' + feeds]), nv.ptr(ws['shift.' + feeds]),
                        N, d[0], d[1], d[2], co, ci, lay, s)
                self._bw_ready[feeds] = gn_rows
            else:
                nv.call('iunet_conv3_fwd', self.dt, self.dim, self._P(dy), co * v, dx_ptr, dx_ss, nv.ptr(wd), None, None,
                        N, d[0], d[1], d[2], co, ci, 0, lay, s)

    def backward(self, ws, x, x_strides, y, w, tdt, N):
        L, ch, dims = self.levels, self.ch, ws['dims']
        s = nv.stream()
        v0 = _vox(dims[0])
        dfeat = ws['dz.dec0.conv2']
        nparts = nv.lib().iunet_head_loss_bwd_num_parts(N, v0, self.ncls, ch[0])
        dy_ready = None
        if self.gn_head:
            bn = 'dec0.bn2'
            nv.call('iunet_head_gn_bwd', self.dt, self._P(ws['y.dec0.conv2']), ch[0] * v0, ch[0], nv.ptr(self.p('head.weight')),
                    nv.ptr(self.p('head.bias')), self.ncls, nv.ptr(y), nv.ptr(w), tdt, nv.ptr(ws['coef']), 0.0, nv.ptr(self.state),
                    nv.ptr(ws['scale.dec0.conv2']), nv.ptr(ws['shift.dec0.conv2']), nv.ptr(ws['mean.dec0.conv2']), nv.ptr(ws['invstd.dec0.conv2']),
                    nv.ptr(self.p(bn + '.weight')), self.groups, nv.ptr(self.g(bn + '.weight')), nv.ptr(self.g(bn + '.bias')), self._P(ws['dy']), ch[0] * v0,
                    nv.ptr(ws['hslab']), nv.ptr(ws['bnslab']), nv.ptr(ws['bncoef']), self._P(dfeat), N, v0, s)
            dy_ready = 'dec0.conv2'
        elif self.head_bn and nv.lib().iunet_head_bn_bwd_ok(ch[0], self.ncls):
            bn = 'dec0.bn2'
            nv.call('iunet_head_bn_bwd', self.dt, self._P(ws['y.dec0.conv2']), ch[0] * v0, ch[0], nv.ptr(self.p('head.weight')),
                    nv.ptr(self.p('head.bias')), self.ncls, nv.ptr(y), nv.ptr(w), tdt, nv.ptr(ws['coef']), 0.0, nv.ptr(self.state),
                    nv.ptr(ws['scale.dec0.conv2']), nv.ptr(ws['shift.dec0.conv2']), nv.ptr(ws['mean.dec0.conv2']), nv.ptr(ws['invstd.dec0.conv2']),
                    nv.ptr(self.p(bn + '.weight')), nv.ptr(self.g(bn + '.weight')), nv.ptr(self.g(bn + '.bias')), self._P(ws['dy']), ch[0] * v0,
                    nv.ptr(ws['hslab']), nv.ptr(ws['bnslab']), nv.ptr(ws['bncoef']), self._P(dfeat), N, v0, s)
            dy_ready = 'dec0.conv2'
        elif self.head_act:
            nv.call('iunet_head_loss_bwd_dev', self.dt, self._P(ws['y.dec0.conv2']), ch[0] * v0, ch[0], nv.ptr(self.p('head.weight')),
                    nv.ptr(self.p('head.bias')), self.ncls, nv.ptr(y), nv.ptr(w), tdt, nv.ptr(ws['coef']),
                    nv.ptr(self.state), self._P(dfeat), ch[0] * v0, nv.ptr(ws['hslab']), nv.ptr(ws['scale.dec0.conv2']),
                    nv.ptr(ws['shift.dec0.conv2']), N, v0, s)
        else:
            nv.call('iunet_head_loss_bwd_dev', self.dt, self._P(ws['z.dec0.conv2']), ch[0] * v0, ch[0], nv.ptr(self.p('head.weight')),
                    nv.ptr(self.p('head.bias')), self.ncls, nv.ptr(y), nv.ptr(w), tdt, nv.ptr(ws['coef']),
                    nv.ptr(self.state), self._P(dfeat), ch[0] * v0, nv.ptr(ws['hslab']), None, None, N, v0, s)
        nv.call('iunet_reduce_slab', nv.ptr(ws['hslab']), nparts, self.ncls * (ch[0] + 1), nv.ptr(ws['htmp']), 1.0, 0, s)
        nv.call('iunet_head_grad_scatter', nv.ptr(ws['htmp']), nv.ptr(self.g('head.weight')), nv.ptr(self.g('head.bias')), self.ncls, ch[0], s)
        for l in range(0, L - 1):
            v, vi, di = _vox(dims[l]), _vox(dims[l + 1]), dims[l + 1]
            z1, z2 = ws[f'z.dec{l}.conv1'], ws[f'z.dec{l}.conv2']
            dz1, dz2 = ws[f'dz.dec{l}.conv1'], ws[f'dz.dec{l}.conv2']
            x2, act, _ = self._conv2_input(ws, f'dec{l}', l, N)
            self._stage_conv_bwd(ws, f'dec{l}.conv2', self._P(dz2), ch[l] * v, self._P(z2), ch[l] * v, x2,
                                 ch[l] * v, ch[l], ch[l], l, self._P(dz1), ch[l] * v, N, x_act=act, feeds=f'dec{l}.conv1',
                                 dy_ready=dy_ready == f'dec{l}.conv2')
            self._stage_conv_bwd(ws, f'dec{l}.conv1', self._P(dz1), ch[l] * v, self._P(z1), ch[l] * v,
                                 self._P(ws[f'cat{l}']), 2 * ch[l] * v, 2 * ch[l], ch[l], l, self._P(ws[f'dcat{l}']),
                                 2 * ch[l] * v, N)
            src_name = f'enc{l + 1}.conv2' if l == L - 2 else f'dec{l + 1}.conv2'
            src, dsrc = ws['z.' + src_name], ws['dz.' + src_name]
            dup = self._P(ws[f'dcat{l}'], ch[l] * v)
            nv.call('iunet_convT_wgrad', self.dt, self.dim, self._P(src), ch[l + 1] * vi, dup, 2 * ch[l] * v,
                    nv.ptr(ws['wslab']), nv.ptr(ws[f'bslab{l}']), nv.ptr(self.g(f'dec{l}.up.weight')),
                    nv.ptr(self.g(f'dec{l}.up.bias')), N, di[0], di[1], di[2], ch[l + 1], ch[l], s)
            _, wd = self.pk[f'dec{l}.up']
            nv.call('iunet_convT_dgrad', self.dt, self.dim, dup, 2 * ch[l] * v, self._P(dsrc), ch[l + 1] * vi,
                    nv.ptr(wd), N, di[0], di[1], di[2], ch[l + 1], ch[l], s)
        if self.pg is not None:
            self.buckets.start_tail()
        for l in range(L - 1, -1, -1):
            v = _vox(dims[l])
            z1, dz1 = ws[f'z.enc{l}.conv1'], ws[f'dz.enc{l}.conv1']
            pool_bwd = None
            if l == L - 1:
                dz2_ptr, dz2_ss = self._P(ws[f'dz.enc{l}.conv2']), ch[l] * v
                z2_ptr, z2_ss = self._P(ws[f'z.enc{l}.conv2']), ch[l] * v
            else:
                do = dims[l + 1]
                pool_bwd = (self._P(ws[f'dpin{l + 1}']), ch[l] * _vox(do), do)
                dz2_ptr, dz2_ss = self._P(ws[f'dcat{l}']), 2 * ch[l] * v
                z2_ptr, z2_ss = self._P(ws[f'cat{l}']), 2 * ch[l] * v
            x2, act, _ = self._conv2_input(ws, f'enc{l}', l, N)
            self._stage_conv_bwd(ws, f'enc{l}.conv2', dz2_ptr, dz2_ss, z2_ptr, z2_ss, x2, ch[l] * v, ch[l],
                                 ch[l], l, self._P(dz1), ch[l] * v, N, x_act=act, pool_bwd=pool_bwd, feeds=f'enc{l}.conv1')
            if l == 0:
                self._stage_conv_bwd(ws, 'enc0.conv1', self._P(dz1), ch[0] * v, self._P(z1), ch[0] * v, None, 0,
                                     self.cin, ch[0], 0, None, 0, N, x_raw=(x, x_strides))
            else:
                self._stage_conv_bwd(ws, f'enc{l}.conv1', self._P(dz1), ch[l] * v, self._P(z1), ch[l] * v,
                                     self._P(ws[f'pin{l}']), ch[l - 1] * v, ch[l - 1], ch[l], l,
                                     self._P(ws[f'dpin{l}']), ch[l - 1] * v, N)
            if l == L - 1 and L > 1 and self.pg is not None and self._bottom_start is not None:
                self.buckets.start(self._bottom_start, self._dec_start)

    def optimizer_step(self):
        s = nv.stream()
        n = self.flat.numel()
        world = self.buckets.finish() if self.pg is not None else 1
        nv.call('iunet_adamw_step_dev', nv.ptr(self.flat), nv.ptr(self.grad), nv.ptr(self.m), nv.ptr(self.v), n,
                float(self.lr), self.betas[0], self.betas[1], self.eps, self.wd, nv.ptr(self.state),
                int(self.T == torch.float16), float(world), s)
        self.repack()
        self.model._packed_sig = None

    def _prep(self, X, y, w):
        X = X.to(self.dev).contiguous()
        y = y.to(self.dev).contiguous()
        w = None if w is None else w.to(self.dev).contiguous()
        if y.dtype not in (torch.float16, torch.float32):
            y = y.float()
        N = X.shape[0]
        sp = tuple(X.shape[2:])
        D, H, W = sp if self.dim == 3 else (1,) + sp
        vox = D * H * W
        if X.dtype not in nv.IN_DTYPE_CODE:
            X = X.float()
        return X, y, w, N, D, H, W, vox, (self.cin * vox, vox, H * W, W, 1)

    def train_step(self, X, y, w=None, sync=True):
        self.sync_weights()
        X, y, w, N, D, H, W, vox, xs = self._prep(X, y, w)
        h = self._handle()
        if h is not None and self.pg is not None:
            out4 = h.forward_backward(X, xs, y, w, N, D, H, W, buckets=self.buckets, bottom=(self._bottom_start, self._dec_start))
            world = self.buckets.finish()
            h.update(float(self.lr), self.betas, self.eps, self.wd, float(world))
            self._py_stale = True
            self.model._packed_sig = None
        elif h is not None:
            out4 = h.step(X, xs, y, w, N, D, H, W, float(self.lr), self.betas, self.eps, self.wd)
            self._py_stale = True
            self.model._packed_sig = None
        else:
            self._refresh()
            ws = self.forward_train(X, xs, N, D, H, W)
            tdt, w = self.train_loss_forward(ws, y, w, N, vox)
            self.backward(ws, X, xs, y, w, tdt, N)
            self.optimizer_step()
            out4 = ws['out4']
        if sync:
            o = out4.tolist()
            return {'Loss': o[0], 'Dice': o[1], 'IoU': o[2], 'MCC': o[3]}
        return out4

    def _handle(self):
        self._steps_seen = getattr(self, '_steps_seen', 0) + 1
        if (self.pg is not None and os.environ.get('IUNET_PY_DP')) or self.probe is not None or os.environ.get('IUNET_PY_TRAIN') \
                or not self.use_handle or self._steps_seen < 2:
            return None
        if getattr(self, '_h', None) is None:
# ... 363 lines not shown
```

Baseline: 737.0 million.

## Fuse batchnorm backward stats into convT dgrad and merge convT wgrad+dgrad

Adds a BN-backward statistics epilogue to the transposed-conv data-gradient kernels, so the per-channel sums the following norm backward needs are computed while dx is written instead of in a separate pass over dx. Also adds a one-pass convT backward kernel that computes dgrad (with the same stats) inside the wgrad kernel, reusing the dy tile already staged in LDS. This aims to cut a full extra read of dy and of the pre-norm activations per decoder level. In exchange the wgrad kernel's occupancy bound drops from 2 to 1 when the dgrad work is fused in, it uses more LDS, and the dgrad kernels now use a grid-stride loop.

```diff
diff --git a/include/iunet.h b/include/iunet.h
--- a/include/iunet.h
+++ b/include/iunet.h
@@ -296,6 +296,15 @@
 int iunet_pack_convT_dgrad(int dtype, const void* w, void* dst, int Cin, int Cout, int npos, void* stream);
 int iunet_convT_dgrad(int dtype, int nd, const void* dy, long long dy_ss, void* dx, long long dx_ss, const void* wpk,
                       int N, int D, int H, int W, int Cin, int Cout, void* stream);
+int iunet_convT_bwd_parts(int nd, int N, int D, int H, int W, int Cin, int Cout);
+int iunet_convT_dgrad_bnstats(int dtype, int nd, const void* dy, long long dy_ss, void* dx, long long dx_ss, const void* wpk,
+                              const void* bw_y, long long bw_y_ss, const void* mean, const void* invstd, const void* scale,
+                              const void* shift, void* stats, int N, int D, int H, int W, int Cin, int Cout, void* stream);
+int iunet_convT_bwd_ok(int nd, int Cin, int Cout);
+int iunet_convT_bwd(int dtype, int nd, const void* x, long long x_ss, const void* dy, long long dy_ss, void* wslab, void* bslab,
+                    void* dW, void* db, void* dx, long long dx_ss, const void* wpk, const void* bw_y, long long bw_y_ss,
+                    const void* mean, const void* invstd, const void* scale, const void* shift, void* stats, int N, int D, int H,
+                    int W, int Cin, int Cout, void* stream);
 int iunet_convT_wgrad_blocks(int nd, int N, int D, int H, int W, int Cin, int Cout);
 int iunet_convT_wgrad(int dtype, int nd, const void* x, long long x_ss, const void* dy, long long dy_ss, void* wslab,
                       void* bslab, void* dW, void* db, int N, int D, int H, int W, int Cin, int Cout, void* stream);
diff --git a/interactive-unet_amd/csrc/train_misc.hip b/interactive-unet_amd/csrc/train_misc.hip
--- a/interactive-unet_amd/csrc/train_misc.hip
+++ b/interactive-unet_amd/csrc/train_misc.hip
@@ -8,9 +8,34 @@
   void* dx; long long dx_ss;
   const void* wpk;
   int N, D, H, W, Cin, Cout;
+  const void* bw_y; long long bw_y_ss;
+  const float *bw_mean, *bw_invstd, *bw_scale, *bw_shift;
+  float* stats;
 };
 
-template <typename T, int ND>
+template <int NC>
+__device__ __forceinline__ void convT_bw_row(float (&s1)[NC][8], float (&s2)[NC][8], float* red, float* __restrict__ stats, int Cin, int cib0) {
+  const int lane = threadIdx.x & 63, wave = threadIdx.x >> 6, l15 = lane & 15, q = lane >> 4;
+#pragma unroll
+  for (int c = 0; c < NC; ++c)
+#pragma unroll
+    for (int j = 0; j < 8; ++j) {
+      float a = s1[c][j], b = s2[c][j];
+#pragma unroll
+      for (int h = 1; h < 16; h <<= 1) { a += __shfl_xor(a, h); b += __shfl_xor(b, h); }
+      if (l15 == 0) { red[((wave * 4 + q) * NC + c) * 16 + j] = a; red[((wave * 4 + q) * NC + c) * 16 + 8 + j] = b; }
+    }
+  __syncthreads();
+  if ((int)threadIdx.x < NC * 64) {
+    const int c = threadIdx.x >> 6, ch = (threadIdx.x >> 1) & 31, which = threadIdx.x & 1;
+    float sum = 0.f;
+#pragma unroll
+    for (int w = 0; w < 4; ++w) sum += red[((w * 4 + (ch >> 3)) * NC + c) * 16 + which * 8 + (ch & 7)];
+    stats[((long long)blockIdx.x * Cin + (cib0 + c) * 32 + ch) * 2 + which] = sum;
+  }
+}
+
+template <typename T, int ND, bool BW = false>
 __global__ __launch_bounds__(256) void convT_dgrad_kernel(ConvTDgradParams p) {
   using V8 = V8T<T>;
   constexpr int NPOS = ND == 3 ? 8 : 4;
@@ -18,43 +43,66 @@
   const int l15 = lane & 15, q = lane >> 4;
   const int xg = (p.W + 15) / 16;
   const long long rows = (long long)p.D * p.H * xg;
-  const long long wid = (long long)blockIdx.x * 4 + wave;
-  if (wid >= rows * p.N) return;
-  const int n = (int)(wid / rows);
-  const long long r = wid - n * rows;
-  const int xb = (int)(r % xg), y = (int)((r / xg) % p.H), z = (int)(r / ((long long)xg * p.H));
   const int cib = blockIdx.y;
-  const int x = xb * 16 + l15;
-  const bool ok = x < p.W;
-  const int xc = ok ? x : p.W - 1;
   const int Do = ND == 3 ? p.D * 2 : 1, Ho = p.H * 2, Wo = p.W * 2;
   const long long out_plane = (long long)Do * Ho * Wo * 8;
-  const T* dyin = (const T*)p.dy + n * p.dy_ss;
+  const long long in_plane = (long long)p.D * p.H * p.W * 8;
   const int nk = p.Cout >> 5;
   const V8* wp = (const V8*)p.wpk + (long long)cib * NPOS * nk * 2 * 64 + lane;
-  f32x4 acc0 = f32x4{0, 0, 0, 0}, acc1 = f32x4{0, 0, 0, 0};
-#pragma unroll
-  for (int s = 0; s < NPOS; ++s) {
-    const int a = ND == 3 ? (s >> 2) : 0, b = (s >> 1) & 1, c = s & 1;
-    const int oz = ND == 3 ? z * 2 + a : 0;
-    const long long voff = (((long long)oz * Ho + y * 2 + b) * Wo + xc * 2 + c) * 8;
-    for (int kc = 0; kc < nk; ++kc) {
-      const V8 bf = *(const V8*)(dyin + (long long)(kc * 4 + q) * out_plane + voff);
-      const V8 a0 = wp[((s * nk + kc) * 2 + 0) * 64];
-      const V8 a1 = wp[((s * nk + kc) * 2 + 1) * 64];
-      acc0 = mfma16<T>(a0, bf, acc0);
-      acc1 = mfma16<T>(a1, bf, acc1);
-    }
-  }
-  const long long in_plane = (long long)p.D * p.H * p.W * 8;
-  V8 o;
-#pragma unroll
-  for (int j = 0; j < 4; ++j) { o[j] = from_f32<T>(acc0[j]); o[4 + j] = from_f32<T>(acc1[j]); }
-  if (ok)
-    *(V8*)((T*)p.dx + n * p.dx_ss + (long long)(cib * 4 + q) * in_plane + (((long long)z * p.H + y) * p.W + x) * 8) = o;
-}
-
-template <typename T, int ND, int NK, int NCI>
+  [[maybe_unused]] float s1[1][8], s2[1][8], mu[8], is[8], sc[8], sh[8];
+  if constexpr (BW) {
+#pragma unroll
+    for (int j = 0; j < 8; ++j) {
+      const int ch = cib * 32 + q * 8 + j;
+      s1[0][j] = 0.f; s2[0][j] = 0.f;
+      mu[j] = p.bw_mean[ch]; is[j] = p.bw_invstd[ch]; sc[j] = p.bw_scale[ch]; sh[j] = p.bw_shift[ch];
+    }
+  }
+  for (long long wid = (long long)blockIdx.x * 4 + wave; wid < rows * p.N; wid += (long long)gridDim.x * 4) {
+    const int n = (int)(wid / rows);
+    const long long r = wid - n * rows;
+    const int xb = (int)(r % xg), y = (int)((r / xg) % p.H), z = (int)(r / ((long long)xg * p.H));
+    const int x = xb * 16 + l15;
+    const bool ok = x < p.W;
+    const int xc = ok ? x : p.W - 1;
+    const T* dyin = (const T*)p.dy + n * p.dy_ss;
+    f32x4 acc0 = f32x4{0, 0, 0, 0}, acc1 = f32x4{0, 0, 0, 0};
+#pragma unroll
+    for (int s = 0; s < NPOS; ++s) {
+      const int a = ND == 3 ? (s >> 2) : 0, b = (s >> 1) & 1, c = s & 1;
+      const int oz = ND == 3 ? z * 2 + a : 0;
+      const long long voff = (((long long)oz * Ho + y * 2 + b) * Wo + xc * 2 + c) * 8;
+      for (int kc = 0; kc < nk; ++kc) {
+        const V8 bf = *(const V8*)(dyin + (long long)(kc * 4 + q) * out_plane + voff);
+        const V8 a0 = wp[((s * nk + kc) * 2 + 0) * 64];
+        const V8 a1 = wp[((s * nk + kc) * 2 + 1) * 64];
+        acc0 = mfma16<T>(a0, bf, acc0);
+        acc1 = mfma16<T>(a1, bf, acc1);
+      }
+    }
+    V8 o;
+#pragma unroll
+    for (int j = 0; j < 4; ++j) { o[j] = from_f32<T>(acc0[j]); o[4 + j] = from_f32<T>(acc1[j]); }
+    const long long voxoff = (long long)(cib * 4 + q) * in_plane + (((long long)z * p.H + y) * p.W + x) * 8;
+    if (ok) {
+      if constexpr (BW) {
+        const V8 yv = *(const V8*)((const T*)p.bw_y + n * p.bw_y_ss + voxoff);
+#pragma unroll
+        for (int j = 0; j < 8; ++j) {
+          const float yy = to_f32<T>(yv[j]);
+          norm_bwd_sums(norm_masked(norm_z<T>(sc[j], yy, sh[j]), to_f32<T>(o[j])), yy, mu[j], is[j], s1[0][j], s2[0][j]);
+        }
+      }
+      *(V8*)((T*)p.dx + n * p.dx_ss + voxoff) = o;
+    }
+  }
+  if constexpr (BW) {
+    __shared__ float red[4 * 4 * 16];
+    convT_bw_row<1>(s1, s2, red, p.stats, p.Cin, cib);
+  }
+}
+
+template <typename T, int ND, int NK, int NCI, bool BW = false>
 __global__ __launch_bounds__(256, (NCI * NK * (ND == 3 ? 16 : 8) <= 64) ? 2 : 1) void convT_dgrad_lds_kernel(ConvTDgradParams p) {
   using V8 = V8T<T>;
   constexpr int NPOS = ND == 3 ? 8 : 4, G = 2;
@@ -66,6 +114,18 @@
   {
     const u32x4* wsrc = (const u32x4*)p.wpk + (long long)cib0 * WCI;
     stage_to_lds(smem, wsrc, NCI * WCI, threadIdx.x, 256);
+  }
+  [[maybe_unused]] float s1[NCI][8], s2[NCI][8];
+  if constexpr (BW) {
+    float* par = (float*)(smem + NCI * WCI * 16);
+    for (int i = threadIdx.x; i < NCI * 128; i += 256) {
+      const int c = i >> 7, which = (i >> 5) & 3, ch = (cib0 + c) * 32 + (i & 31);
+      par[i] = (which == 0 ? p.bw_mean : which == 1 ? p.bw_invstd : which == 2 ? p.bw_scale : p.bw_shift)[ch];
+    }
+#pragma unroll
+    for (int c = 0; c < NCI; ++c)
+#pragma unroll
+      for (int j = 0; j < 8; ++j) { s1[c][j] = 0.f; s2[c][j] = 0.f; }
   }
   __syncthreads();
   const int xg = (p.W + 15) / 16;
@@ -80,6 +140,7 @@
     const T* dyb[G];
     long long xoff[G];
     bool okg[G];
+    [[maybe_unused]] V8 bw_yv[BW ? NCI : 1][G];
 #pragma unroll
     for (int g = 0; g < G; ++g) {
       const long long wid = g0 + g < ngroups ? g0 + g : ngroups - 1;
@@ -93,6 +154,11 @@
       xoff[g] = n * p.dx_ss + (long long)(cib0 * 4 + q) * in_plane + (((long long)z * p.H + y) * p.W + x) * 8;
 #pragma unroll
       for (int c = 0; c < NCI; ++c) { acc[c][g][0] = f32x4{0, 0, 0, 0}; acc[c][g][1] = f32x4{0, 0, 0, 0}; }
+      if constexpr (BW) {
+        const T* yp = (const T*)p.bw_y + n * p.bw_y_ss + (long long)(cib0 * 4 + q) * in_plane + (((long long)z * p.H + y) * p.W + xc) * 8;
+#pragma unroll
+        for (int c = 0; c < NCI; ++c) bw_yv[c][g] = *(const V8*)(yp + (long long)c * 4 * in_plane);
+      }
     }
 #pragma unroll
     for (int s = 0; s < NPOS; ++s) {
@@ -122,8 +188,23 @@
         V8 o;
 #pragma unroll
         for (int j = 0; j < 4; ++j) { o[j] = from_f32<T>(acc[c][g][0][j]); o[4 + j] = from_f32<T>(acc[c][g][1][j]); }
+        if constexpr (BW) if (okg[g]) {
+          const f32x4* bp = (const f32x4*)(smem + NCI * WCI * 16) + c * 32 + 2 * q;
+          const f32x4 m0 = bp[0], m1 = bp[1], i0 = bp[8], i1 = bp[9], c0 = bp[16], c1 = bp[17], h0 = bp[24], h1 = bp[25];
+#pragma unroll
+          for (int j = 0; j < 8; ++j) {
+            const float mu = j < 4 ? m0[j & 3] : m1[j & 3], is = j < 4 ? i0[j & 3] : i1[j & 3];
+            const float sc = j < 4 ? c0[j & 3] : c1[j & 3], sh = j < 4 ? h0[j & 3] : h1[j & 3];
+            const float yy = to_f32<T>(bw_yv[c][g][j]);
+            norm_bwd_sums(norm_masked(norm_z<T>(sc, yy, sh), to_f32<T>(o[j])), yy, mu, is, s1[c][j], s2[c][j]);
+          }
+        }
         if (okg[g]) *(V8*)((T*)p.dx + xoff[g] + (long long)c * 4 * in_plane) = o;
       }
+  }
+  if constexpr (BW) {
+    __syncthreads();
+    convT_bw_row<NCI>(s1, s2, (float*)smem, p.stats, p.Cin, cib0);
   }
 }
 
@@ -165,10 +246,11 @@
   float* bslab;
   int N, D, H, W, Cin, Cout;
   int tilesZ, tilesY, tilesX;
+  ConvTDgradParams dg;
 };
 
-template <typename T, int ND, int NCI>
-__global__ __launch_bounds__(256, 2) void convT_wgrad_kernel(ConvTWgradParams p) {
+template <typename T, int ND, int NCI, bool DG = false>
+__global__ __launch_bounds__(256, DG ? 1 : 2) void convT_wgrad_kernel(ConvTWgradParams p) {
   using V8 = V8T<T>;
   constexpr int NPOS = ND == 3 ? 8 : 4;
   constexpr int TZ = ND == 3 ? 2 : 1, TY = ND == 3 ? 4 : 8, TX = 16;
@@ -179,6 +261,8 @@
   constexpr int OFF_Y = 4 * PLANE_X;
   constexpr int NKS = NVI / 32;
   constexpr int PL = NPOS / 4;
+  constexpr int OFF_W = OFF_Y + 4 * PLANE_Y, WCI = NPOS * 2 * 64;
+  constexpr int OFF_P = OFF_W + NCI * WCI * 16;
   extern __shared__ __attribute__((aligned(256))) unsigned char smem[];
   const unsigned lds0 = (unsigned)(size_t)(__attribute__((address_space(3))) unsigned char*)smem;
   const int tid = threadIdx.x, lane = tid & 63;
@@ -209,13 +293,41 @@
   constexpr int XIT = NVI * 4 / 256, YIT = NVO * 4 / 256;
   u32x4 xr[NCI * XIT], xkeep[NCI > 1 ? XIT : 1];
   V8 yr[YIT];
-  auto load_tile = [&](int tile) {
-    const int n = tile / tps;
+  [[maybe_unused]] V8 bw_yr[DG ? NCI * 2 : 1], bw_yc[DG ? NCI * 2 : 1];
+  [[maybe_unused]] float s1[NCI][8], s2[NCI][8];
+  if constexpr (DG) {
+    stage_to_lds(smem + OFF_W, (const u32x4*)p.dg.wpk, NCI * WCI, tid, 256);
+    float* par = (float*)(smem + OFF_P);
+    for (int i = tid; i < NCI * 128; i += 256) {
+      const int which = (i >> 5) & 3, ch = (i >> 7) * 32 + (i & 31);
+      par[i] = (which == 0 ? p.dg.bw_mean : which == 1 ? p.dg.bw_invstd : which == 2 ? p.dg.bw_scale : p.dg.bw_shift)[ch];
+    }
+#pragma unroll
+    for (int c = 0; c < NCI; ++c)
+#pragma unroll
+      for (int j = 0; j < 8; ++j) { s1[c][j] = 0.f; s2[c][j] = 0.f; }
+  }
+  auto tile_origin = [&](int tile, int& n, int& z0, int& y0, int& x0) {
+    n = tile / tps;
     int trem = tile - n * tps;
     const int tz_i = trem / (p.tilesY * p.tilesX);
     trem -= tz_i * p.tilesY * p.tilesX;
     const int ty_i = trem / p.tilesX, tx_i = trem - ty_i * p.tilesX;
-    const int z0 = tz_i * TZ, y0 = ty_i * TY, x0 = tx_i * TX;
+    z0 = tz_i * TZ; y0 = ty_i * TY; x0 = tx_i * TX;
+  };
+  auto load_tile = [&](int tile) {
+    int n, z0, y0, x0;
+    tile_origin(tile, n, z0, y0, x0);
+    if constexpr (DG) {
+#pragma unroll
+      for (int gi = 0; gi < 2; ++gi) {
+        const int r = wave * 2 + gi;
+        const int gz = min(z0 + r / TY, p.D - 1), gy = min(y0 + r % TY, p.H - 1), gx = min(x0 + i16, p.W - 1);
+        const T* yp = (const T*)p.dg.bw_y + (long long)n * p.dg.bw_y_ss + (long long)g * in_plane + (((long long)gz * p.H + gy) * p.W + gx) * 8;
+#pragma unroll
+        for (int c = 0; c < NCI; ++c) bw_yr[c * 2 + gi] = *(const V8*)(yp + (long long)c * 4 * in_plane);
+      }
+    }
     const T* xin = (const T*)p.x + (long long)n * p.x_ss + (long long)cib0 * 4 * in_plane;
     const T* dyin = (const T*)p.dy + (long long)n * p.dy_ss + (long long)cob * 4 * out_plane;
 #pragma unroll
@@ -255,6 +367,10 @@
 #pragma unroll
       for (int k = 0; k < XIT; ++k) xkeep[k] = xr[XIT + k];
     }
+    if constexpr (DG) {
+#pragma unroll
+      for (int k = 0; k < NCI * 2; ++k) bw_yc[k] = bw_yr[k];
+    }
 #pragma unroll
     for (int k = 0; k < YIT; ++k) {
       const int it = tid + k * 256;
@@ -295,6 +411,61 @@
         }
       }
     }
+    if constexpr (DG) {
+      int n, z0, y0, x0;
+      tile_origin(tile, n, z0, y0, x0);
+      unsigned woff = OFF_W + lane * 16;
+      asm volatile("" : "+v"(woff));
+      const V8* wl = (const V8*)(smem + woff);
+      f32x4 dacc[NCI][2][2];
+#pragma unroll
+      for (int c = 0; c < NCI; ++c)
+#pragma unroll
+        for (int gi = 0; gi < 2; ++gi) { dacc[c][gi][0] = f32x4{0, 0, 0, 0}; dacc[c][gi][1] = f32x4{0, 0, 0, 0}; }
+#pragma unroll
+      for (int s = 0; s < NPOS; ++s) {
+        const int a = ND == 3 ? (s >> 2) : 0, b = (s >> 1) & 1, c2 = s & 1;
+        V8 bf[2];
+#pragma unroll
+        for (int gi = 0; gi < 2; ++gi) {
+          const int r = wave * 2 + gi, pz = r / TY, py = r % TY;
+          bf[gi] = *(const V8*)(smem + OFF_Y + g * PLANE_Y + ((((2 * pz + a) * OY + 2 * py + b) * OX) + 2 * i16 + c2) * 16);
+        }
+#pragma unroll
+        for (int c = 0; c < NCI; ++c) {
+          const V8 a0 = wl[c * WCI + (s * 2 + 0) * 64];
+          const V8 a1 = wl[c * WCI + (s * 2 + 1) * 64];
+#pragma unroll
+          for (int gi = 0; gi < 2; ++gi) {
+            dacc[c][gi][0] = mfma16<T>(a0, bf[gi], dacc[c][gi][0]);
+            dacc[c][gi][1] = mfma16<T>(a1, bf[gi], dacc[c][gi][1]);
+          }
+        }
+      }
+#pragma unroll
+      for (int c = 0; c < NCI; ++c) {
+        const f32x4* bp = (const f32x4*)(smem + OFF_P) + c * 32 + 2 * g;
+        const f32x4 m0 = bp[0], m1 = bp[1], i0 = bp[8], i1 = bp[9], c0 = bp[16], c1 = bp[17], h0 = bp[24], h1 = bp[25];
+#pragma unroll
+        for (int gi = 0; gi < 2; ++gi) {
+          const int r = wave * 2 + gi;
+          const int gz = z0 + r / TY, gy = y0 + r % TY, gx = x0 + i16;
+          V8 o;
+#pragma unroll
+          for (int j = 0; j < 4; ++j) { o[j] = from_f32<T>(dacc[c][gi][0][j]); o[4 + j] = from_f32<T>(dacc[c][gi][1][j]); }
+          if (gz < p.D && gy < p.H && gx < p.W) {
+#pragma unroll
+            for (int j = 0; j < 8; ++j) {
+              const float mu = j < 4 ? m0[j & 3] : m1[j & 3], is = j < 4 ? i0[j & 3] : i1[j & 3];
+              const float sc = j < 4 ? c0[j & 3] : c1[j & 3], sh = j < 4 ? h0[j & 3] : h1[j & 3];
+              const float yy = to_f32<T>(bw_yc[c * 2 + gi][j]);
+              norm_bwd_sums(norm_masked(norm_z<T>(sc, yy, sh), to_f32<T>(o[j])), yy, mu, is, s1[c][j], s2[c][j]);
+            }
+            *(V8*)((T*)p.dg.dx + (long long)n * p.dg.dx_ss + (long long)(c * 4 + g) * in_plane + (((long long)gz * p.H + gy) * p.W + gx) * 8) = o;
+          }
+        }
+      }
+    }
   }
 #pragma unroll
   for (int c = 0; c < NCI; ++c) {
@@ -322,6 +493,10 @@
       for (int k = pl; k < 256; k += 4) sum += red[k * 8 + j];
       p.bslab[(long long)blockIdx.x * p.Cout + cob * 32 + pl * 8 + j] = sum;
     }
+  }
+  if constexpr (DG) {
+    __syncthreads();
+    convT_bw_row<NCI>(s1, s2, (float*)(smem + OFF_Y), p.dg.stats, p.Cin, 0);
   }
 }
 
@@ -570,43 +745,84 @@
   return IUNET_OK;
 }
 
-int iunet_convT_dgrad(int dtype, int nd, const void* dy, long long dy_ss, void* dx, long long dx_ss, const void* wpk,
-                      int N, int D, int H, int W, int Cin, int Cout, void* stream) {
+struct ConvTDgradLaunch { int nci, gx, lds; };
+static ConvTDgradLaunch convT_dgrad_launch(int nd, int N, int D, int H, int W, int Cin, int Cout, bool bw) {
+  const long long waves = (long long)N * D * H * ((W + 15) / 16);
+  const int nk = Cout / 32;
+  ConvTDgradLaunch l;
+  if (nk <= 4 && waves >= 256) {
+    l.nci = (nk <= 2 && (Cin / 32) % 2 == 0 && (nd == 3 ? 8 : 4) * nk * 2 * 1024 * 2 <= 32768) ? 2 : 1;
+    l.lds = (nd == 3 ? 8 : 4) * nk * 2 * 1024 * l.nci + (bw ? l.nci * 512 : 0);
+    const long long gx = (waves + 7) / 8;
+    const int cap = 1024 / (Cin / 32 / l.nci);
+    l.gx = (int)(gx > cap ? cap : gx);
+    return l;
+  }
+  const long long gx = (waves + 3) / 4;
+  l.nci = 0; l.lds = 0;
+  l.gx = (int)(bw && gx > 1024 ? 1024 : gx);
+  return l;
+}
+
+static int convT_dgrad_impl(const char* what, int dtype, int nd, const void* dy, long long dy_ss, void* dx, long long dx_ss, const void* wpk,
+                            const void* bw_y, long long bw_y_ss, const void* mean, const void* invstd, const void* scale, const void* shift,
+                            void* stats, int N, int D, int H, int W, int Cin, int Cout, void* stream) {
   DT_OK(dtype);
-  IUNET_REQUIRE(dy && dx && wpk, "convT_dgrad: null pointer");
-  IUNET_REQUIRE(nd == 2 || nd == 3, "convT_dgrad: nd must be 2 or 3");
-  IUNET_REQUIRE_GRID("convT_dgrad", N, D, H, W);
-  IUNET_REQUIRE(Cin >= 32 && Cout >= 32 && Cin % 32 == 0 && Cout % 32 == 0, "convT_dgrad: channels must be positive multiples of 32 (%d, %d)", Cin, Cout);
+  IUNET_REQUIRE(dy && dx && wpk, "%s: null pointer", what);
+  IUNET_REQUIRE(nd == 2 || nd == 3, "%s: nd must be 2 or 3", what);
+  IUNET_REQUIRE(N > 0 && D > 0 && H > 0 && W > 0, "%s: bad shape N %d, %d x %d x %d", what, N, D, H, W);
+  IUNET_REQUIRE(Cin >= 32 && Cout >= 32 && Cin % 32 == 0 && Cout % 32 == 0, "%s: channels must be positive multiples of 32 (%d, %d)", what, Cin, Cout);
+  const bool bw = bw_y != nullptr;
   ConvTDgradParams p;
   p.dy = dy; p.dy_ss = dy_ss; p.dx = dx; p.dx_ss = dx_ss; p.wpk = wpk; p.N = N; p.D = D; p.H = H; p.W = W; p.Cin = Cin; p.Cout = Cout;
-  const long long waves = (long long)N * D * H * ((W + 15) / 16);
+  p.bw_y = bw_y; p.bw_y_ss = bw_y_ss; p.bw_mean = (const float*)mean; p.bw_invstd = (const float*)invstd;
+  p.bw_scale = (const float*)scale; p.bw_shift = (const float*)shift; p.stats = (float*)stats;
+  const ConvTDgradLaunch l = convT_dgrad_launch(nd, N, D, H, W, Cin, Cout, bw);
   const int nk = Cout / 32;
-  if (nk <= 4 && waves >= 256) {
-    const int nci = (nk <= 2 && (Cin / 32) % 2 == 0 && (nd == 3 ? 8 : 4) * nk * 2 * 1024 * 2 <= 32768) ? 2 : 1;
-    const int lds = (nd == 3 ? 8 : 4) * nk * 2 * 1024 * nci;
-    int gx = (int)((waves + 7) / 8);
-    const int cap = 1024 / (Cin / 32 / nci);
-    if (gx > cap) gx = cap;
-    dim3 g2(gx, Cin / 32 / nci);
-#define CDL(TT, NDV, NKV) do { if (nci == 2) { IUNET_SET_MAX_LDS((convT_dgrad_lds_kernel<TT, NDV, NKV, 2>), lds); \
-      hipLaunchKernelGGL((convT_dgrad_lds_kernel<TT, NDV, NKV, 2>), g2, dim3(256), lds, (hipStream_t)stream, p); } \
-    else { IUNET_SET_MAX_LDS((convT_dgrad_lds_kernel<TT, NDV, NKV, 1>), lds); \
-      hipLaunchKernelGGL((convT_dgrad_lds_kernel<TT, NDV, NKV, 1>), g2, dim3(256), lds, (hipStream_t)stream, p); } } while (0)
+  if (l.nci > 0) {
+    const int nci = l.nci, lds = l.lds;
+    dim3 g2(l.gx, Cin / 32 / nci);
+#define CDL2(TT, NDV, NKV, NCIV, BWV) do { IUNET_SET_MAX_LDS((convT_dgrad_lds_kernel<TT, NDV, NKV, NCIV, BWV>), lds); \
+      hipLaunchKernelGGL((convT_dgrad_lds_kernel<TT, NDV, NKV, NCIV, BWV>), g2, dim3(256), lds, (hipStream_t)stream, p); } while (0)
+#define CDL(TT, NDV, NKV) do { if (nci == 2) { if (bw) CDL2(TT, NDV, NKV, 2, true); else CDL2(TT, NDV, NKV, 2, false); } \
+    else { if (bw) CDL2(TT, NDV, NKV, 1, true); else CDL2(TT, NDV, NKV, 1, false); } } while (0)
 #define CDL_NK(TT, NDV) switch (nk) { case 1: CDL(TT, NDV, 1); break; case 2: CDL(TT, NDV, 2); break; case 3: CDL(TT, NDV, 3); break; default: CDL(TT, NDV, 4); break; }
     if (dtype == 0) { if (nd == 3) { CDL_NK(f16, 3) } else { CDL_NK(f16, 2) } }
     else            { if (nd == 3) { CDL_NK(bf16, 3) } else { CDL_NK(bf16, 2) } }
 #undef CDL_NK
 #undef CDL
+#undef CDL2
     IUNET_CHECK_HIP(hipGetLastError());
     return IUNET_OK;
   }
-  dim3 grid((unsigned)((waves + 3) / 4), Cin / 32);
-  if (dtype == 0) { if (nd == 3) hipLaunchKernelGGL((convT_dgrad_kernel<f16, 3>), grid, dim3(256), 0, (hipStream_t)stream, p);
-                    else hipLaunchKernelGGL((convT_dgrad_kernel<f16, 2>), grid, dim3(256), 0, (hipStream_t)stream, p); }
-  else { if (nd == 3) hipLaunchKernelGGL((convT_dgrad_kernel<bf16, 3>), grid, dim3(256), 0, (hipStream_t)stream, p);
-         else hipLaunchKernelGGL((convT_dgrad_kernel<bf16, 2>), grid, dim3(256), 0, (hipStream_t)stream, p); }
+  dim3 grid((unsigned)l.gx, Cin / 32);
+  iunet_dispatch(dtype, nd, bw, [&](auto t, auto ndc, auto bwc) {
+    hipLaunchKernelGGL((convT_dgrad_kernel<decltype(t), decltype(ndc)::value, decltype(bwc)::value>), grid, dim3(256), 0, (hipStream_t)stream, p);
+    return 0;
+  });
   IUNET_CHECK_HIP(hipGetLastError());
   return IUNET_OK;
+}
+
+int iunet_convT_dgrad(int dtype, int nd, const void* dy, long long dy_ss, void* dx, long long dx_ss, const void* wpk,
+                      int N, int D, int H, int W, int Cin, int Cout, void* stream) {
+  return convT_dgrad_impl("convT_dgrad", dtype, nd, dy, dy_ss, dx, dx_ss, wpk, nullptr, 0, nullptr, nullptr, nullptr, nullptr, nullptr, N, D, H, W,
+                          Cin, Cout, stream);
+}
+
+int iunet_convT_bwd_parts(int nd, int N, int D, int H, int W, int Cin, int Cout) {
+  IUNET_REQUIRE(nd == 2 || nd == 3, "convT_bwd_parts: nd must be 2 or 3");
+  IUNET_REQUIRE_GRID("convT_bwd_parts", N, D, H, W);
+  IUNET_REQUIRE(Cin >= 32 && Cout >= 32 && Cin % 32 == 0 && Cout % 32 == 0, "convT_bwd_parts: channels must be positive multiples of 32 (%d, %d)", Cin, Cout);
+  return convT_dgrad_launch(nd, N, D, H, W, Cin, Cout, true).gx;
+}
+
+int iunet_convT_dgrad_bnstats(int dtype, int nd, const void* dy, long long dy_ss, void* dx, long long dx_ss, const void* wpk, const void* bw_y,
+                              long long bw_y_ss, const void* mean, const void* invstd, const void* scale, const void* shift, void* stats,
+                              int N, int D, int H, int W, int Cin, int Cout, void* stream) {
+  IUNET_REQUIRE(bw_y && mean && invstd && scale && shift && stats, "convT_dgrad_bnstats: null pointer");
+  return convT_dgrad_impl("convT_dgrad_bnstats", dtype, nd, dy, dy_ss, dx, dx_ss, wpk, bw_y, bw_y_ss, mean, invstd, scale, shift, stats, N, D, H, W,
+                          Cin, Cout, stream);
 }
 
 int iunet_convT_wgrad_blocks(int nd, int N, int D, int H, int W, int Cin, int Cout) {
@@ -620,35 +836,62 @@
   return (int)(nb < 1 ? 1 : nb);
 }
 
-int iunet_convT_wgrad(int dtype, int nd, const void* x, long long x_ss, const void* dy, long long dy_ss, void* wslab,
-                      void* bslab, void* dW, void* db, int N, int D, int H, int W, int Cin, int Cout, void* stream) {
+static int convT_wgrad_impl(const char* what, int dtype, int nd, const void* x, long long x_ss, const void* dy, long long dy_ss, void* wslab,
+                            void* bslab, void* dW, void* db, const ConvTDgradParams* dg, int N, int D, int H, int W, int Cin, int Cout,
+                            void* stream) {
   DT_OK(dtype);
-  IUNET_REQUIRE(x && dy && wslab && bslab && dW && db, "convT_wgrad: null pointer");
-  IUNET_REQUIRE(Cin >= 32 && Cout >= 32 && Cin % 32 == 0 && Cout % 32 == 0, "convT_wgrad: channels must be positive multiples of 32");
-  IUNET_REQUIRE(nd == 2 || nd == 3, "convT_wgrad: nd must be 2 or 3");
-  IUNET_REQUIRE_GRID("convT_wgrad", N, D, H, W);
+  IUNET_REQUIRE(x && dy && wslab && bslab && dW && db, "%s: null pointer", what);
+  IUNET_REQUIRE(Cin >= 32 && Cout >= 32 && Cin % 32 == 0 && Cout % 32 == 0, "%s: channels must be positive multiples of 32", what);
+  IUNET_REQUIRE(nd == 2 || nd == 3, "%s: nd must be 2 or 3", what);
+  IUNET_REQUIRE(N > 0 && D > 0 && H > 0 && W > 0, "%s: bad shape N %d, %d x %d x %d", what, N, D, H, W);
   ConvTWgradParams p;
   p.x = x; p.x_ss = x_ss; p.dy = dy; p.dy_ss = dy_ss; p.wslab = (float*)wslab; p.bslab = (float*)bslab;
   p.N = N; p.D = D; p.H = H; p.W = W; p.Cin = Cin; p.Cout = Cout;
+  p.dg = dg ? *dg : ConvTDgradParams{};
   const int TZ = nd == 3 ? 2 : 1, TY = nd == 3 ? 4 : 8, TX = 16;
   p.tilesZ = (D + TZ - 1) / TZ; p.tilesY = (H + TY - 1) / TY; p.tilesX = (W + TX - 1) / TX;
   const int nb = iunet_convT_wgrad_blocks(nd, N, D, H, W, Cin, Cout);
   const int npos = nd == 3 ? 8 : 4;
   const int nvi = 128, nvo = nd == 3 ? 1024 : 512;
-  const int lds = 4 * (nvi * 16 + 64) + 4 * (nvo * 16 + 64);
   const int nci = (Cin / 32) % 2 == 0 ? 2 : 1;
+  const int lds = 4 * (nvi * 16 + 64) + 4 * (nvo * 16 + 64) + (dg ? nci * (npos * 2 * 1024 + 512) : 0);
   dim3 grid(nb, Cin / 32 / nci, Cout / 32);
-#define CTW(TT, NDV) do { if (nci == 2) { IUNET_SET_MAX_LDS((convT_wgrad_kernel<TT, NDV, 2>), lds); \
-      hipLaunchKernelGGL((convT_wgrad_kernel<TT, NDV, 2>), grid, dim3(256), lds, (hipStream_t)stream, p); } \
-    else { IUNET_SET_MAX_LDS((convT_wgrad_kernel<TT, NDV, 1>), lds); \
-      hipLaunchKernelGGL((convT_wgrad_kernel<TT, NDV, 1>), grid, dim3(256), lds, (hipStream_t)stream, p); } } while (0)
+#define CTW2(TT, NDV, NCIV, DGV) do { IUNET_SET_MAX_LDS((convT_wgrad_kernel<TT, NDV, NCIV, DGV>), lds); \
+      hipLaunchKernelGGL((convT_wgrad_kernel<TT, NDV, NCIV, DGV>), grid, dim3(256), lds, (hipStream_t)stream, p); } while (0)
+#define CTW(TT, NDV) do { if (nci == 2) { if (dg) CTW2(TT, NDV, 2, true); else CTW2(TT, NDV, 2, false); } \
+    else { if (dg) CTW2(TT, NDV, 1, true); else CTW2(TT, NDV, 1, false); } } while (0)
   if (dtype == 0) { if (nd == 3) CTW(f16, 3); else CTW(f16, 2); } else { if (nd == 3) CTW(bf16, 3); else CTW(bf16, 2); }
 #undef CTW
+#undef CTW2
   const long long total = (long long)Cin * Cout * npos;
   hipLaunchKernelGGL(convT_wgrad_reduce_kernel, dim3((unsigned)(total / 64)), dim3(256), 0, (hipStream_t)stream,
                      (const float*)wslab, nb, Cin, Cout, npos, (float*)dW);
   IUNET_CHECK_HIP(hipGetLastError());
   return iunet_reduce_slab(bslab, nb, Cout, db, 1.0f, 0, stream);
+}
+
+int iunet_convT_wgrad(int dtype, int nd, const void* x, long long x_ss, const void* dy, long long dy_ss, void* wslab,
+                      void* bslab, void* dW, void* db, int N, int D, int H, int W, int Cin, int Cout, void* stream) {
+  return convT_wgrad_impl("convT_wgrad", dtype, nd, x, x_ss, dy, dy_ss, wslab, bslab, dW, db, nullptr, N, D, H, W, Cin, Cout, stream);
+}
+
+int iunet_convT_bwd_ok(int nd, int Cin, int Cout) {
+  IUNET_REQUIRE(nd == 2 || nd == 3, "convT_bwd_ok: nd must be 2 or 3");
+  IUNET_REQUIRE(Cin >= 32 && Cout >= 32 && Cin % 32 == 0 && Cout % 32 == 0, "convT_bwd_ok: channels must be positive multiples of 32 (%d, %d)", Cin, Cout);
+  return Cout == 32 && (Cin == 32 || Cin == 64) ? 1 : 0;
+}
+
+int iunet_convT_bwd(int dtype, int nd, const void* x, long long x_ss, const void* dy, long long dy_ss, void* wslab, void* bslab, void* dW,
+                    void* db, void* dx, long long dx_ss, const void* wpk, const void* bw_y, long long bw_y_ss, const void* mean,
+                    const void* invstd, const void* scale, const void* shift, void* stats, int N, int D, int H, int W, int Cin, int Cout,
+                    void* stream) {
+  IUNET_REQUIRE(dx && wpk && bw_y && mean && invstd && scale && shift && stats, "convT_bwd: null pointer");
+  IUNET_REQUIRE((nd == 2 || nd == 3) && Cin >= 32 && Cout >= 32 && Cin % 32 == 0 && Cout % 32 == 0 && iunet_convT_bwd_ok(nd, Cin, Cout) == 1,
+                "convT_bwd: no one-pass form for %d -> %d channels in %d-D (iunet_convT_bwd_ok)", Cin, Cout, nd);
+  ConvTDgradParams dg{};
+  dg.dx = dx; dg.dx_ss = dx_ss; dg.wpk = wpk; dg.bw_y = bw_y; dg.bw_y_ss = bw_y_ss; dg.bw_mean = (const float*)mean;
+  dg.bw_invstd = (const float*)invstd; dg.bw_scale = (const float*)scale; dg.bw_shift = (const float*)shift; dg.stats = (float*)stats;
+  return convT_wgrad_impl("convT_bwd", dtype, nd, x, x_ss, dy, dy_ss, wslab, bslab, dW, db, &dg, N, D, H, W, Cin, Cout, stream);
 }
 
 int iunet_first_conv_wgrad_blocks(int nd, int N, int D, int H, int W) {
diff --git a/interactive-unet_amd/csrc/train_net.hip b/interactive-unet_amd/csrc/train_net.hip
--- a/interactive-unet_amd/csrc/train_net.hip
+++ b/interactive-unet_amd/csrc/train_net.hip
@@ -57,6 +57,12 @@
 int iunet_conv3_wgrad_act(int, int, const void*, long long, const void*, long long, void*, void*, float, const void*, const void*, int,
                           int, int, int, int, int, void*);
 int iunet_convT_dgrad(int, int, const void*, long long, void*, long long, const void*, int, int, int, int, int, int, void*);
+int iunet_convT_bwd_parts(int, int, int, int, int, int, int);
+int iunet_convT_dgrad_bnstats(int, int, const void*, long long, void*, long long, const void*, const void*, long long, const void*, const void*,
+                              const void*, const void*, void*, int, int, int, int, int, int, void*);
+int iunet_convT_bwd_ok(int, int, int);
+int iunet_convT_bwd(int, int, const void*, long long, const void*, long long, void*, void*, void*, void*, void*, long long, const void*, const void*,
+                    long long, const void*, const void*, const void*, const void*, void*, int, int, int, int, int, int, void*);
 int iunet_convT_wgrad_blocks(int, int, int, int, int, int, int);
 int iunet_convT_wgrad(int, int, const void*, long long, const void*, long long, void*, void*, void*, void*, int, int, int, int, int, int,
                       void*);
@@ -123,7 +129,7 @@
   int norm = 0, groups = 8;
   int dim, levels, base, cin, ncls, dtype, kind;
   int taps, npos;
-  bool fuse_act, fuse_bw, head_act, gn_conv_stats, gn_bw, head_bn, gn_head;
+  bool fuse_act, fuse_bw, head_act, gn_conv_stats, gn_bw, head_bn, gn_head, convT_bw, convT_one;
   std::vector<int> ch;
   std::vector<TParam> params;
   long long nparams = 0;
@@ -209,6 +215,7 @@
       const long long nb = iunet_convT_wgrad_blocks(dim, N, d, h, w, n->ch[l + 1], n->ch[l]);
       max_wslab = std::max(max_wslab, nb * n->ch[l + 1] * n->ch[l] * n->npos);
       L.bslab[l] = f32(nb * n->ch[l]);
+      max_stats = std::max(max_stats, std::max<long long>(iunet_convT_bwd_parts(dim, N, d, h, w, n->ch[l + 1], n->ch[l]), nb) * n->ch[l + 1] * 2);
     }
     if (l > 0) { L.pin[l] = act((long long)N * n->ch[l - 1] * v); L.dpin[l] = act((long long)N * n->ch[l - 1] * v); }
   }
@@ -332,6 +339,8 @@
   n->head_act = norm == 0 && !env_on("IUNET_NO_HEAD_ACT");
   n->gn_head = norm == 1 && !env_on("IUNET_NO_HEAD_ACT") && !env_on("IUNET_NO_HEAD_BN_FUSION") && iunet_head_bn_bwd_ok(base, ncls);
   n->head_bn = n->head_act && !env_on("IUNET_NO_HEAD_BN_FUSION");
+  n->convT_bw = norm == 0 && !env_on("IUNET_NO_CONVT_FUSION");
+  n->convT_one = n->convT_bw && !env_on("IUNET_NO_CONVT_ONE_PASS");
   n->gn_conv_stats = norm == 1 && !env_on("IUNET_NO_GN_CONV_STATS");
   n->gn_bw = n->gn_conv_stats && !env_on("IUNET_NO_GN_BW_FUSION");
   for (int l = 0; l < levels; ++l) n->ch.push_back(base << l);
@@ -826,10 +835,23 @@
     const int ksrc = l == lv - 2 ? idx(false, l + 1, 2) : idx(true, l + 1, 2);
     const TUp& u = n->up[lv - 2 - l];
     void* dup = WS + L.dcat[l] + (long long)c * v * 2;
+    if (n->convT_one && iunet_convT_bwd_ok(dim, cn, c) == 1) {
+      rc = iunet_convT_bwd(dt, dim, WS + L.z[ksrc], (long long)cn * vi, dup, 2ll * c * v, F(L.wslab), F(L.bslab[l]), G + u.w, G + u.b, WS + L.dz[ksrc],
+                           (long long)cn * vi, K + u.dgr, WS + L.y[ksrc], (long long)cn * vi, F(L.mean[ksrc]), F(L.invstd[ksrc]), F(L.scale[ksrc]),
+                           F(L.shift[ksrc]), F(L.stats), N, di, hi, wi, cn, c, stream);
+      if (rc) return rc;
+      bw_ready[ksrc] = iunet_convT_wgrad_blocks(dim, N, di, hi, wi, cn, c);
+      continue;
+    }
     rc = iunet_convT_wgrad(dt, dim, WS + L.z[ksrc], (long long)cn * vi, dup, 2ll * c * v, F(L.wslab), F(L.bslab[l]), G + u.w, G + u.b, N, di, hi, wi, cn,
                            c, stream);
     if (rc) return rc;
-    rc = iunet_convT_dgrad(dt, dim, dup, 2ll * c * v, WS + L.dz[ksrc], (long long)cn * vi, K + u.dgr, N, di, hi, wi, cn, c, stream);
+    if (n->convT_bw) {
+      rc = iunet_convT_dgrad_bnstats(dt, dim, dup, 2ll * c * v, WS + L.dz[ksrc], (long long)cn * vi, K + u.dgr, WS + L.y[ksrc], (long long)cn * vi,
+                                     F(L.mean[ksrc]), F(L.invstd[ksrc]), F(L.scale[ksrc]), F(L.shift[ksrc]), F(L.stats), N, di, hi, wi, cn, c, stream);
+      bw_ready[ksrc] = iunet_convT_bwd_parts(dim, N, di, hi, wi, cn, c);
+    } else
+      rc = iunet_convT_dgrad(dt, dim, dup, 2ll * c * v, WS + L.dz[ksrc], (long long)cn * vi, K + u.dgr, N, di, hi, wi, cn, c, stream);
     if (rc) return rc;
   }
   if (hook) hook(hook_ctx, 0);
diff --git a/interactive-unet_amd/interactive_unet/_native.py b/interactive-unet_amd/interactive_unet/_native.py
--- a/interactive-unet_amd/interactive_unet/_native.py
+++ b/interactive-unet_amd/interactive_unet/_native.py
@@ -221,6 +221,12 @@
     'iunet_pack_convT_dgrad': [c_int, c_void_p, c_void_p, c_int, c_int, c_int, c_void_p],
     'iunet_convT_dgrad': [c_int, c_int, c_void_p, c_ll, c_void_p, c_ll, c_void_p, c_int, c_int, c_int, c_int, c_int,
                           c_int, c_void_p],
+    'iunet_convT_bwd_parts': [c_int] * 7,
+    'iunet_convT_dgrad_bnstats': [c_int, c_int, c_void_p, c_ll, c_void_p, c_ll, c_void_p, c_void_p, c_ll, c_void_p, c_void_p, c_void_p,
+                                  c_void_p, c_void_p, c_int, c_int, c_int, c_int, c_int, c_int, c_void_p],
+    'iunet_convT_bwd_ok': [c_int] * 3,
+    'iunet_convT_bwd': [c_int, c_int, c_void_p, c_ll, c_void_p, c_ll, c_void_p, c_void_p, c_void_p, c_void_p, c_void_p, c_ll, c_void_p, c_void_p,
+                        c_ll, c_void_p, c_void_p, c_void_p, c_void_p, c_void_p, c_int, c_int, c_int, c_int, c_int, c_int, c_void_p],
     'iunet_convT_wgrad_blocks': [c_int] * 7,
     'iunet_convT_wgrad': [c_int, c_int, c_void_p, c_ll, c_void_p, c_ll, c_void_p, c_void_p, c_void_p, c_void_p,
                           c_int, c_int, c_int, c_int, c_int, c_int, c_void_p],
diff --git a/interactive-unet_amd/interactive_unet/train_engine.py b/interactive-unet_amd/interactive_unet/train_engine.py
--- a/interactive-unet_amd/interactive_unet/train_engine.py
+++ b/interactive-unet_amd/interactive_unet/train_engine.py
@@ -53,6 +53,8 @@
         self.head_bn = self.head_act and not os.environ.get('IUNET_NO_HEAD_BN_FUSION')
         self.gn_head = (self.gn and not os.environ.get('IUNET_NO_HEAD_ACT') and not os.environ.get('IUNET_NO_HEAD_BN_FUSION')
                         and bool(nv.lib().iunet_head_bn_bwd_ok(self.ch[0], self.ncls)))
+        self.convT_bw = not self.gn and not os.environ.get('IUNET_NO_CONVT_FUSION')
+        self.convT_one = self.convT_bw and not os.environ.get('IUNET_NO_CONVT_ONE_PASS')
         self._bw_ready = {}
         self._flatten()
         if self.pg is not None:
@@ -220,6 +222,7 @@
                 nb = lib.iunet_convT_wgrad_blocks(self.dim, N, *dims[l + 1], ch[l + 1], ch[l])
                 max_wslab = max(max_wslab, nb * ch[l + 1] * ch[l] * self.npos)
                 ws[f'bslab{l}'] = f32(nb * ch[l])
+                max_stats = max(max_stats, max(lib.iunet_convT_bwd_parts(self.dim, N, *dims[l + 1], ch[l + 1], ch[l]), nb) * ch[l + 1] * 2)
             if l > 0:
                 ws[f'pin{l}'] = act(ch[l - 1], v)
                 ws[f'dpin{l}'] = act(ch[l - 1], v)
@@ -500,12 +503,27 @@
             src_name = f'enc{l + 1}.conv2' if l == L - 2 else f'dec{l + 1}.conv2'
             src, dsrc = ws['z.' + src_name], ws['dz.' + src_name]
             dup = self._P(ws[f'dcat{l}'], ch[l] * v)
+            _, wd = self.pk[f'dec{l}.up']
+            if self.convT_one and nv.lib().iunet_convT_bwd_ok(self.dim, ch[l + 1], ch[l]) == 1:
+                nv.call('iunet_convT_bwd', self.dt, self.dim, self._P(src), ch[l + 1] * vi, dup, 2 * ch[l] * v, nv.ptr(ws['wslab']),
+                        nv.ptr(ws[f'bslab{l}']), nv.ptr(self.g(f'dec{l}.up.weight')), nv.ptr(self.g(f'dec{l}.up.bias')), self._P(dsrc),
+                        ch[l + 1] * vi, nv.ptr(wd), self._P(ws['y.' + src_name]), ch[l + 1] * vi, nv.ptr(ws['mean.' + src_name]),
+                        nv.ptr(ws['invstd.' + src_name]), nv.ptr(ws['scale.' + src_name]), nv.ptr(ws['shift.' + src_name]), nv.ptr(ws['stats']),
+                        N, di[0], di[1], di[2], ch[l + 1], ch[l], s)
+                self._bw_ready[src_name] = nv.lib().iunet_convT_wgrad_blocks(self.dim, N, di[0], di[1], di[2], ch[l + 1], ch[l])
+                continue
             nv.call('iunet_convT_wgrad', self.dt, self.dim, self._P(src), ch[l + 1] * vi, dup, 2 * ch[l] * v,
                     nv.ptr(ws['wslab']), nv.ptr(ws[f'bslab{l}']), nv.ptr(self.g(f'dec{l}.up.weight')),
                     nv.ptr(self.g(f'dec{l}.up.bias')), N, di[0], di[1], di[2], ch[l + 1], ch[l], s)
-            _, wd = self.pk[f'dec{l}.up']
-            nv.call('iunet_convT_dgrad', self.dt, self.dim, dup, 2 * ch[l] * v, self._P(dsrc), ch[l + 1] * vi,
-                    nv.ptr(wd), N, di[0], di[1], di[2], ch[l + 1], ch[l], s)
+            if self.convT_bw:
+                nv.call('iunet_convT_dgrad_bnstats', self.dt, self.dim, dup, 2 * ch[l] * v, self._P(dsrc), ch[l + 1] * vi, nv.ptr(wd),
+                        self._P(ws['y.' + src_name]), ch[l + 1] * vi, nv.ptr(ws['mean.' + src_name]), nv.ptr(ws['invstd.' + src_name]),
+                        nv.ptr(ws['scale.' + src_name]), nv.ptr(ws['shift.' + src_name]), nv.ptr(ws['stats']), N, di[0], di[1], di[2],
+                        ch[l + 1], ch[l], s)
+                self._bw_ready[src_name] = nv.lib().iunet_convT_bwd_parts(self.dim, N, di[0], di[1], di[2], ch[l + 1], ch[l])
+            else:
+                nv.call('iunet_convT_dgrad', self.dt, self.dim, dup, 2 * ch[l] * v, self._P(dsrc), ch[l + 1] * vi,
+                        nv.ptr(wd), N, di[0], di[1], di[2], ch[l + 1], ch[l], s)
         if self.pg is not None:
             self.buckets.start_tail()
         for l in range(L - 1, -1, -1):
```

Result: no change. 740.6 million, median of 4 (+0.5%).
